# hrubaanna/mysticeti

Hardware: AMD Instinct MI355X
Metric: verified StatementBlock sigs/sec (1/2/4/8 MI355X) vs host-core ed25519-consensus (higher is better)
Workload: dtype u32

## Files before the change

include/mysti_verify.h:

```cpp
#ifndef MYSTI_VERIFY_H
#define MYSTI_VERIFY_H

#include <stddef.h>
#include <stdint.h>

#ifdef __cplusplus
extern "C" {
#endif

typedef struct mv_ctx mv_ctx;
typedef int32_t mv_status;

#define MV_OK 0
#define MV_E_INVALID_ARG (-1)
#define MV_E_HIP (-2)
#define MV_E_NO_DEVICE (-3)
#define MV_E_NO_COMMITTEE (-4)
#define MV_E_ALLOC (-5)
#define MV_E_INDEX_FULL (-6)

#define MV_SIG_OK 0
#define MV_SIG_INVALID 1
#define MV_SIG_MALFORMED_KEY 2

// ... 72 lines not shown

mv_status mv_ed25519_sign(mv_ctx* ctx, const uint8_t* seed, const uint8_t* msg, uint32_t n, uint8_t* pk,
                          uint8_t* sig);

mv_status mv_verify_blocks(mv_ctx* ctx, const uint8_t* buf, const uint64_t* off, const uint64_t* len, uint32_t n,
                           uint8_t* status, uint8_t* msg_digest, uint8_t* block_digest);

mv_status mv_queue_stats(mv_ctx* ctx, uint64_t* calls, uint64_t* passes);

mv_status mv_online_stats(mv_ctx* ctx, uint64_t* requests, uint64_t* launches);

mv_status mv_shard_plan(const uint64_t* weights, uint64_t n, uint32_t parts, uint64_t* cut );

int64_t mv_block_preimage(const uint8_t* bincode, uint64_t len, uint8_t* out, uint64_t cap);

mv_status mv_crc32(mv_ctx* ctx, const uint8_t* buf, const uint64_t* off, const uint64_t* len, uint32_t n,
                   uint32_t* out );

mv_status mv_wal_verify(mv_ctx* ctx, const uint8_t* wal, uint64_t size, uint64_t end_pos, uint32_t map_bits,
                        uint64_t* pos, uint32_t* tag, uint32_t* len, uint8_t* status, uint64_t cap,
                        uint64_t* count);

mv_status mv_wal_replay(mv_ctx* ctx, const uint8_t* wal, uint64_t size, uint64_t end_pos, uint32_t map_bits,
                        uint64_t* pos, uint32_t* tag, uint32_t* len, uint8_t* status, uint64_t cap, uint64_t* count,
                        uint64_t* blk_rows , uint8_t* blk_status ,
                        uint64_t cap_blocks, uint64_t* n_blocks, uint64_t* summary ,
                        uint64_t* last_seen );

uint64_t mv_wal_layout(const uint64_t* payload_len, uint64_t n, uint32_t map_bits, uint64_t start,
                       uint64_t* pos );

int64_t mv_frame_blocks(const uint8_t* buf, uint64_t len, uint64_t* off, uint64_t* blen, uint64_t cap,
                        uint64_t* consumed);

int64_t mv_frame_messages(const uint8_t* buf, uint64_t len, uint32_t* msgs , uint64_t cap_msgs,
                          uint64_t* blk_off, uint64_t* blk_len, uint64_t cap_blocks, uint64_t* n_blocks,
                          uint64_t* consumed);
mv_status mv_verify_frames(mv_ctx* ctx, const uint8_t* buf, const uint64_t* soff, const uint64_t* slen, uint32_t ns,
                           uint64_t* consumed , uint32_t* drop_msg , uint32_t* msgs ,
                           uint64_t cap_msgs, uint64_t* n_msgs, uint64_t* blk_off, uint64_t* blk_len,
                           uint8_t* blk_status , uint64_t cap_blocks, uint64_t* n_blocks);

mv_status mv_index_reserve(mv_ctx* ctx, uint64_t entries);
mv_status mv_index_clear(mv_ctx* ctx);
mv_status mv_index_stats(mv_ctx* ctx, uint64_t* out );
mv_status mv_index_insert(mv_ctx* ctx, const uint64_t* refs , uint64_t n, uint32_t state,
                          uint8_t* prior );
mv_status mv_index_insert_stored(mv_ctx* ctx, const uint64_t* refs , uint64_t n,
                                 uint8_t* prior );
mv_status mv_index_lookup(mv_ctx* ctx, const uint64_t* refs , uint64_t n, uint8_t* state );
mv_status mv_index_wanted(mv_ctx* ctx, uint64_t* refs , uint64_t cap, uint64_t* n);
mv_status mv_accept_blocks(mv_ctx* ctx, const uint8_t* buf, const uint64_t* off, const uint64_t* len,
                           const uint64_t* grp , uint32_t n, uint8_t* blk_status ,
                           uint8_t* blk_state , uint64_t* missing , uint64_t cap_missing,
                           uint64_t* n_missing);
mv_status mv_connect_blocks(mv_ctx* ctx, const uint8_t* buf, const uint64_t* off, const uint64_t* len,
                            const uint64_t* grp , uint32_t n, uint8_t* blk_status ,
                            uint8_t* blk_state , uint64_t* missing , uint64_t cap_missing,
                            uint64_t* n_missing, uint64_t* connected , uint64_t cap_connected,
                            uint64_t* n_connected);
mv_status mv_pending_reserve(mv_ctx* ctx, uint64_t blocks, uint64_t includes);
mv_status mv_pending_stats(mv_ctx* ctx, uint64_t* out );

mv_status mv_dag_reserve(mv_ctx* ctx, uint64_t blocks, uint64_t includes);
mv_status mv_dag_prune(mv_ctx* ctx, uint64_t round);
mv_status mv_dag_stats(mv_ctx* ctx, uint64_t* out );

#define MV_LEADER_UNDECIDED 0
#define MV_LEADER_COMMIT 1
#define MV_LEADER_SKIP 2
#define MV_LEADER_CONFLICT 3
#define MV_LEADER_OVERFLOW 4
#define MV_DECIDE_MAX_LEADER_BLOCKS 8
mv_status mv_decide_leaders(mv_ctx* ctx, const uint64_t* leaders , uint32_t n,
                            uint64_t* out , uint64_t* stakes );

#define MV_COMMIT_KIND_NONE 0
#define MV_COMMIT_KIND_DIRECT 1
#define MV_COMMIT_KIND_INDIRECT 2
#define MV_COMMIT_INCOMPLETE 1
#define MV_COMMIT_BLOCKED 2
mv_status mv_commit_leaders(mv_ctx* ctx, const uint64_t* leaders , uint32_t n,
                            uint64_t* out , uint64_t* info , uint64_t* n_sequence);

mv_status mv_wal_recover(mv_ctx* ctx, const uint8_t* wal, uint64_t size, uint64_t end_pos, uint32_t map_bits,
                         uint64_t* pos, uint32_t* tag, uint32_t* len, uint8_t* status, uint64_t cap, uint64_t* count,
                         uint64_t* blk_rows , uint8_t* blk_status ,
                         uint64_t cap_blocks, uint64_t* n_blocks, uint64_t* summary ,
                         uint64_t* last_seen , uint64_t floor_round, uint64_t* seeded );

#define MV_SEAL_OK 0
#define MV_SEAL_PARSE_ERROR 1
#define MV_SEAL_UNKNOWN_AUTHOR 2
#define MV_SEAL_UNLINKED 3
#define MV_SEAL_LINK 1u
mv_status mv_seal_blocks(mv_ctx* ctx, uint8_t* buf, const uint64_t* off, const uint64_t* len, uint32_t n,
                         const uint8_t* seeds , uint32_t n_auth, uint32_t flags,
                         uint8_t* status , uint8_t* msg_digest ,
                         uint8_t* block_digest );

mv_status mv_dev_ed25519_verify(mv_ctx* ctx, int device, const uint8_t* d_msg, const uint8_t* d_sig,
                                const uint8_t* d_pk, uint32_t n, uint8_t* d_status, void* stream);
mv_status mv_dev_ed25519_verify_batch(mv_ctx* ctx, int device, const uint8_t* d_msg, const uint8_t* d_sig,
                                      const uint8_t* d_pk, const uint32_t* d_key_idx, uint32_t n,
                                      uint8_t* d_status, uint32_t* d_batch_ok, void* stream);
mv_status mv_dev_ed25519_sign(mv_ctx* ctx, int device, const uint8_t* d_seed, const uint8_t* d_msg, uint32_t n,
                              uint8_t* d_pk, uint8_t* d_sig, void* stream);
mv_status mv_dev_verify_blocks(mv_ctx* ctx, int device, const uint8_t* d_buf, uint64_t buf_bytes,
                               const uint64_t* d_off, const uint64_t* d_len, uint32_t n, uint8_t* d_status,
                               uint8_t* d_msg_digest, uint8_t* d_block_digest, void* stream);

mv_status mv_dev_wal_verify(mv_ctx* ctx, int device, const uint8_t* d_wal, uint64_t size, uint64_t end_pos,
                            uint32_t map_bits, uint64_t* d_pos, uint32_t* d_tag, uint32_t* d_len, uint8_t* d_status,
                            uint64_t cap, uint64_t* count, void* stream);
mv_status mv_dev_wal_replay(mv_ctx* ctx, int device, const uint8_t* d_wal, uint64_t size, uint64_t end_pos,
                            uint32_t map_bits, uint64_t* d_pos, uint32_t* d_tag, uint32_t* d_len, uint8_t* d_status,
                            uint64_t cap, uint64_t* count, uint64_t* d_blk_rows, uint8_t* d_blk_status,
                            uint64_t cap_blocks, uint64_t* n_blocks, uint64_t* d_summary, uint64_t* d_last_seen,
                            void* stream);
mv_status mv_dev_verify_frames(mv_ctx* ctx, int device, const uint8_t* d_buf, uint64_t buf_bytes,
                               const uint64_t* d_soff, const uint64_t* d_slen, uint32_t ns, uint64_t* d_consumed,
                               uint32_t* d_drop_msg, uint32_t* d_msgs, uint64_t cap_msgs, uint64_t* n_msgs,
                               uint64_t* d_blk_off, uint64_t* d_blk_len, uint8_t* d_blk_status, uint64_t cap_blocks,
                               uint64_t* n_blocks, void* stream);
mv_status mv_dev_accept_blocks(mv_ctx* ctx, int device, const uint8_t* d_buf, uint64_t buf_bytes,
                               const uint64_t* d_off, const uint64_t* d_len, const uint64_t* d_grp, uint32_t n,
                               uint8_t* d_blk_status, uint8_t* d_blk_state, uint64_t* d_missing, uint64_t cap_missing,
                               uint64_t* n_missing, void* stream);
mv_status mv_dev_index_insert(mv_ctx* ctx, int device, const uint64_t* d_words, uint64_t stride_words, uint64_t n,
                              uint32_t state, void* stream);
mv_status mv_dev_dag_seed_rows(mv_ctx* ctx, int device, const uint8_t* d_wal, uint64_t size,
                               const uint64_t* d_blk_rows , const uint8_t* d_blk_status ,
                               uint64_t n_rows, uint64_t floor_round, uint64_t* seeded , void* stream);
mv_status mv_dev_connect_blocks(mv_ctx* ctx, int device, const uint8_t* d_buf, uint64_t buf_bytes,
                                const uint64_t* d_off, const uint64_t* d_len, const uint64_t* d_grp, uint32_t n,
                                uint8_t* d_blk_status, uint8_t* d_blk_state, uint64_t* d_missing, uint64_t cap_missing,
                                uint64_t* n_missing, uint64_t* d_connected, uint64_t cap_connected,
                                uint64_t* n_connected, void* stream);
mv_status mv_dev_decide_leaders(mv_ctx* ctx, int device, const uint64_t* d_leaders, uint32_t n, uint64_t* d_out,
                                uint64_t* d_stakes , void* stream);
mv_status mv_dev_commit_leaders(mv_ctx* ctx, int device, const uint64_t* d_leaders, uint32_t n, uint64_t* d_out,
                                uint64_t* d_info, uint64_t* n_sequence, void* stream);
mv_status mv_dev_seal_blocks(mv_ctx* ctx, int device, uint8_t* d_buf, uint64_t buf_bytes, const uint64_t* d_off,
                             const uint64_t* d_len, uint32_t n, const uint8_t* d_seeds, uint32_t n_auth,
                             uint32_t flags, uint8_t* d_status, uint8_t* d_msg_digest, uint8_t* d_block_digest,
                             void* stream);
mv_status mv_dev_crc32(mv_ctx* ctx, int device, const uint8_t* d_buf, const uint64_t* d_off, const uint64_t* d_len,
                       uint32_t n, uint32_t* d_out, void* stream);

mv_status mv_batch_stats(mv_ctx* ctx, uint64_t* batches, uint64_t* fallbacks);
mv_status mv_batch_counters(mv_ctx* ctx, uint64_t* out );
mv_status mv_batch_routes(mv_ctx* ctx, uint64_t* out );
mv_status mv_set_batch_groups(mv_ctx* ctx, uint32_t groups);
#define MV_NSTAGES 12
mv_status mv_set_stage_timing(mv_ctx* ctx, int enable);
mv_status mv_stage_times(mv_ctx* ctx, double* ms , uint64_t* calls ,
                         int reset);
mv_status mv_set_option(mv_ctx* ctx, const char* name, int64_t value);
mv_status mv_get_option(mv_ctx* ctx, const char* name, int64_t* value);
mv_status mv_selftest(mv_ctx* ctx, int op, const uint32_t* in, uint32_t n, uint32_t* out);
mv_status mv_selftest_batch_prep(mv_ctx* ctx, const uint8_t* msg, const uint8_t* sig, const uint8_t* pk,
                                 const uint32_t* key_idx, uint32_t n, uint32_t groups, const uint8_t* key,
                                 uint32_t launch_sigs, uint32_t* scal, uint32_t* pts, uint64_t* bsum,
                                 uint8_t* status, uint32_t* info);
mv_status mv_selftest_batch_msm(mv_ctx* ctx, uint32_t n, uint32_t groups, const uint32_t* scal, const uint32_t* pts,
                                const uint64_t* bsum, const uint32_t* key_idx, uint32_t n_keys, uint32_t* win,
                                uint32_t* asum, uint32_t* flags, uint32_t* info);
mv_status mv_selftest_comb_table(mv_ctx* ctx, int key, uint32_t* out);

#ifdef __cplusplus
}
#endif
#endif
```

mysticeti_amd/__init__.py:

```python
from __future__ import annotations

import contextlib
import ctypes
import os
from typing import Iterable, List, Optional, Sequence, Tuple

import numpy as np

_HERE = os.path.dirname(os.path.abspath(__file__))
LIB_PATH = os.environ.get("MV_LIB") or os.path.join(_HERE, "libmysti_verify.so")

MV_OK = 0
SIG_OK, SIG_INVALID, SIG_MALFORMED_KEY = 0, 1, 2
BLOCK_STATUS = [
    "OK", "PARSE_ERROR", "DIGEST_MISMATCH", "EPOCH_MISMATCH", "UNKNOWN_AUTHOR", "GENESIS", "SIG_INVALID",
    "INCLUDE_UNKNOWN_AUTHORITY", "INCLUDE_ROUND", "VOTE_RANGE", "THRESHOLD_CLOCK", "VOTE_RANGE_TOO_LONG",
    "VOTE_RANGE_END_TOO_LARGE",
]
(BLOCK_OK, BLOCK_PARSE_ERROR, BLOCK_DIGEST_MISMATCH, BLOCK_EPOCH_MISMATCH, BLOCK_UNKNOWN_AUTHOR,
 BLOCK_GENESIS, BLOCK_SIG_INVALID, BLOCK_INCLUDE_UNKNOWN_AUTHORITY, BLOCK_INCLUDE_ROUND,
 BLOCK_VOTE_RANGE, BLOCK_THRESHOLD_CLOCK, BLOCK_VOTE_RANGE_TOO_LONG, BLOCK_VOTE_RANGE_END_TOO_LARGE) = range(13)

EXPORTS = [
    "mv_create", "mv_destroy", "mv_last_error", "mv_version", "mv_set_committee", "mv_blake2b256",
    "mv_ed25519_verify", "mv_ed25519_sign", "mv_verify_blocks", "mv_dev_ed25519_verify",
    "mv_dev_ed25519_sign", "mv_selftest", "mv_selftest_batch_prep", "mv_selftest_batch_msm", "mv_selftest_comb_table", "mv_block_preimage", "mv_dev_ed25519_verify_batch", "mv_batch_stats",
    "mv_set_stage_timing", "mv_stage_times", "mv_dev_verify_blocks", "mv_batch_counters", "mv_batch_routes", "mv_set_batch_groups",
    "mv_queue_stats", "mv_shard_plan", "mv_crc32", "mv_wal_verify", "mv_wal_layout", "mv_dev_wal_verify",
    "mv_frame_blocks", "mv_frame_messages", "mv_verify_frames", "mv_dev_verify_frames",
    "mv_index_reserve", "mv_index_clear", "mv_index_stats", "mv_index_insert", "mv_index_lookup", "mv_index_wanted",
    "mv_accept_blocks", "mv_dev_accept_blocks", "mv_dev_index_insert",
    "mv_index_insert_stored", "mv_connect_blocks", "mv_dev_connect_blocks", "mv_pending_reserve", "mv_pending_stats",
    "mv_dag_reserve", "mv_dag_prune", "mv_dag_stats", "mv_decide_leaders", "mv_dev_decide_leaders",
    "mv_commit_leaders", "mv_dev_commit_leaders", "mv_wal_recover", "mv_dev_dag_seed_rows",
    "mv_seal_blocks", "mv_dev_seal_blocks",
    "mv_wal_replay", "mv_dev_wal_replay", "mv_dev_crc32", "mv_host_alloc", "mv_host_free", "mv_online_stats", "mv_set_option", "mv_get_option",
]
SEAL_STATUS = ["OK", "PARSE_ERROR", "UNKNOWN_AUTHOR", "UNLINKED"]
SEAL_OK, SEAL_PARSE_ERROR, SEAL_UNKNOWN_AUTHOR, SEAL_UNLINKED = range(4)
SEAL_LINK = 1
WAL_OK, WAL_CRC_MISMATCH, WAL_NONZERO_CRC_LEN0, WAL_BAD_LENGTH = range(4)
WAL_UNKNOWN_TAG, WAL_BLOCK_DECODE, WAL_UNKNOWN_AUTHORITY = 4, 5, 6
WAL_NONE = 0xFFFFFFFFFFFFFFFF
WAL_ROW_WORDS = 10
MSG_STATUS = ["OK", "DECODE_ERROR", "BLOCK_REJECTED", "TOO_MANY_REQUESTED", "NOT_REACHED", "BAD_SIZE"]
MSG_OK, MSG_DECODE_ERROR, MSG_BLOCK_REJECTED, MSG_TOO_MANY_REQUESTED, MSG_NOT_REACHED, MSG_BAD_SIZE = range(6)
MSG_NONE = 0xFFFFFFFF
REF_ABSENT, REF_WANTED, REF_HAVE, REF_STORED = 0, 1, 2, 3
ACC_STATE = ["REJECTED", "NEW", "KNOWN", "DUP", "DROPPED", "SUSPENDED"]
ACC_REJECTED, ACC_NEW, ACC_KNOWN, ACC_DUP, ACC_DROPPED, ACC_SUSPENDED = range(6)
CONNECT_EARLIER = 0xFFFFFFFFFFFFFFFF
E_INDEX_FULL = -6
E_INVALID_ARG, E_NO_COMMITTEE = -1, -4
LEADER_STATUS = ["UNDECIDED", "COMMIT", "SKIP", "CONFLICT", "OVERFLOW"]
LEADER_UNDECIDED, LEADER_COMMIT, LEADER_SKIP, LEADER_CONFLICT, LEADER_OVERFLOW = range(5)
DECIDE_MAX_LEADER_BLOCKS = 8
COMMIT_KIND_NONE, COMMIT_KIND_DIRECT, COMMIT_KIND_INDIRECT = range(3)
COMMIT_INCOMPLETE, COMMIT_BLOCKED = 1, 2
COMMIT_NO_ANCHOR = 0xFFFFFFFFFFFFFFFF
WAL_MAP_BITS, WAL_MAP_BITS_TEST = 24, 16
STAGES = ["prep", "sort", "bucket", "reduce", "final", "fallback", "parse", "hash", "verify", "verdict", "wal_walk",
          "wal_crc"]
FLAG_NO_BATCH, FLAG_NO_COMB, FLAG_HOST_PARSE, FLAG_NO_ONLINE = 1, 2, 4, 8
BATCH_MIN = 4096
SELFTEST_WIDE_OP = 64
BATCH_MAX_GROUPS = 16
COMB_ROWS, COMB_ENTRIES = 32, 129
BATCH_PREP_UNWRITTEN = 0xA5A5A5A5


class MvError(RuntimeError):

    def __init__(self, msg, code=None):
        super().__init__(msg)
        self.code = code


class _Config(ctypes.Structure):
    _fields_ = [("device_mask", ctypes.c_uint32), ("max_batch", ctypes.c_uint32), ("flags", ctypes.c_uint32),
                ("shards_per_device", ctypes.c_uint32)]


_lib = None


def load_library(path: str = LIB_PATH):
    global _lib
    if _lib is not None:
        return _lib
    if not os.path.exists(path):
        raise MvError(f"{path} missing: build it with `python -m mysticeti_amd.build` (no CPU fallback exists)")
    lib = ctypes.CDLL(path)
    vp, u32, u64 = ctypes.c_void_p, ctypes.c_uint32, ctypes.c_uint64
    lib.mv_create.argtypes = [ctypes.POINTER(_Config), ctypes.POINTER(vp)]
    lib.mv_destroy.argtypes = [vp]
    lib.mv_destroy.restype = None
    lib.mv_last_error.argtypes = [vp]
    lib.mv_last_error.restype = ctypes.c_char_p
    lib.mv_version.restype = ctypes.c_char_p
    lib.mv_set_committee.argtypes = [vp, vp, vp, u32, u64, vp]
    lib.mv_blake2b256.argtypes = [vp, vp, vp, vp, u32, vp]
    lib.mv_ed25519_verify.argtypes = [vp, vp, vp, vp, vp, u32, vp]
    lib.mv_ed25519_sign.argtypes = [vp, vp, vp, u32, vp, vp]
    lib.mv_verify_blocks.argtypes = [vp, vp, vp, vp, u32, vp, vp, vp]
    lib.mv_dev_ed25519_verify.argtypes = [vp, ctypes.c_int, vp, vp, vp, u32, vp, vp]
    lib.mv_dev_ed25519_verify_batch.argtypes = [vp, ctypes.c_int, vp, vp, vp, vp, u32, vp, vp, vp]
    lib.mv_batch_stats.argtypes = [vp, vp, vp]
    lib.mv_batch_counters.argtypes = [vp, vp]
    lib.mv_batch_routes.argtypes = [vp, vp]
    lib.mv_set_batch_groups.argtypes = [vp, u32]
    lib.mv_queue_stats.argtypes = [vp, vp, vp]
    lib.mv_online_stats.argtypes = [vp, vp, vp]
    lib.mv_shard_plan.argtypes = [vp, u64, u32, vp]
    lib.mv_set_stage_timing.argtypes = [vp, ctypes.c_int]
    lib.mv_stage_times.argtypes = [vp, vp, vp, ctypes.c_int]
    lib.mv_dev_verify_blocks.argtypes = [vp, ctypes.c_int, vp, u64, vp, vp, u32, vp, vp, vp, vp]
    lib.mv_dev_ed25519_sign.argtypes = [vp, ctypes.c_int, vp, vp, u32, vp, vp, vp]
    lib.mv_seal_blocks.argtypes = [vp, vp, vp, vp, u32, vp, u32, u32, vp, vp, vp]
    lib.mv_dev_seal_blocks.argtypes = [vp, ctypes.c_int, vp, u64, vp, vp, u32, vp, u32, u32, vp, vp, vp, vp]
    lib.mv_selftest.argtypes = [vp, ctypes.c_int, vp, u32, vp]
    lib.mv_selftest_batch_prep.argtypes = [vp, vp, vp, vp, vp, u32, u32, vp, u32, vp, vp, vp, vp, vp]
    lib.mv_selftest_batch_msm.argtypes = [vp, u32, u32, vp, vp, vp, vp, u32, vp, vp, vp, vp]
    lib.mv_selftest_comb_table.argtypes = [vp, ctypes.c_int, vp]
    lib.mv_block_preimage.argtypes = [vp, u64, vp, u64]
    lib.mv_block_preimage.restype = ctypes.c_int64
    lib.mv_crc32.argtypes = [vp, vp, vp, vp, u32, vp]
    lib.mv_wal_verify.argtypes = [vp, vp, u64, u64, u32, vp, vp, vp, vp, u64, vp]
    lib.mv_wal_layout.argtypes = [vp, u64, u32, u64, vp]
    lib.mv_wal_layout.restype = u64
    lib.mv_frame_blocks.argtypes = [vp, u64, vp, vp, u64, vp]
    lib.mv_frame_blocks.restype = ctypes.c_int64
    lib.mv_frame_messages.argtypes = [vp, u64, vp, u64, vp, vp, u64, vp, vp]
    lib.mv_frame_messages.restype = ctypes.c_int64
    lib.mv_verify_frames.argtypes = [vp, vp, vp, vp, u32, vp, vp, vp, u64, vp, vp, vp, vp, u64, vp]
    lib.mv_dev_verify_frames.argtypes = [vp, ctypes.c_int, vp, u64, vp, vp, u32, vp, vp, vp, u64, vp, vp, vp, vp, u64,
                                         vp, vp]
    lib.mv_dev_wal_verify.argtypes = [vp, ctypes.c_int, vp, u64, u64, u32, vp, vp, vp, vp, u64, vp, vp]
    lib.mv_wal_replay.argtypes = [vp, vp, u64, u64, u32, vp, vp, vp, vp, u64, vp, vp, vp, u64, vp, vp, vp]
    lib.mv_dev_wal_replay.argtypes = [vp, ctypes.c_int, vp, u64, u64, u32, vp, vp, vp, vp, u64, vp, vp, vp, u64, vp, vp,
                                      vp, vp]
    lib.mv_wal_recover.argtypes = [vp, vp, u64, u64, u32, vp, vp, vp, vp, u64, vp, vp, vp, u64, vp, vp, vp, u64, vp]
    lib.mv_dev_dag_seed_rows.argtypes = [vp, ctypes.c_int, vp, u64, vp, vp, u64, u64, vp, vp]
    lib.mv_dev_crc32.argtypes = [vp, ctypes.c_int, vp, vp, vp, u32, vp, vp]
    lib.mv_index_reserve.argtypes = [vp, u64]
    lib.mv_index_clear.argtypes = [vp]
    lib.mv_index_stats.argtypes = [vp, vp]
    lib.mv_index_insert.argtypes = [vp, vp, u64, u32, vp]
    lib.mv_index_lookup.argtypes = [vp, vp, u64, vp]
    lib.mv_index_wanted.argtypes = [vp, vp, u64, vp]
    lib.mv_accept_blocks.argtypes = [vp, vp, vp, vp, vp, u32, vp, vp, vp, u64, vp]
    lib.mv_dev_accept_blocks.argtypes = [vp, ctypes.c_int, vp, u64, vp, vp, vp, u32, vp, vp, vp, u64, vp, vp]
    lib.mv_dev_index_insert.argtypes = [vp, ctypes.c_int, vp, u64, u64, u32, vp]
    lib.mv_index_insert_stored.argtypes = [vp, vp, u64, vp]
    lib.mv_connect_blocks.argtypes = [vp, vp, vp, vp, vp, u32, vp, vp, vp, u64, vp, vp, u64, vp]
    lib.mv_dev_connect_blocks.argtypes = [vp, ctypes.c_int, vp, u64, vp, vp, vp, u32, vp, vp, vp, u64, vp, vp, u64, vp, vp]
    lib.mv_pending_reserve.argtypes = [vp, u64, u64]
    lib.mv_pending_stats.argtypes = [vp, vp]
    lib.mv_dag_reserve.argtypes = [vp, u64, u64]
    lib.mv_dag_prune.argtypes = [vp, u64]
    lib.mv_dag_stats.argtypes = [vp, vp]
    lib.mv_decide_leaders.argtypes = [vp, vp, u32, vp, vp]
    lib.mv_dev_decide_leaders.argtypes = [vp, ctypes.c_int, vp, u32, vp, vp, vp]
    lib.mv_commit_leaders.argtypes = [vp, vp, u32, vp, vp, vp]
    lib.mv_dev_commit_leaders.argtypes = [vp, ctypes.c_int, vp, u32, vp, vp, vp, vp]
    lib.mv_host_alloc.argtypes = [vp, u64, ctypes.POINTER(vp)]
    lib.mv_host_free.argtypes = [vp, vp]
    lib.mv_host_free.restype = None
    lib.mv_set_option.argtypes = [vp, ctypes.c_char_p, ctypes.c_int64]
    lib.mv_get_option.argtypes = [vp, ctypes.c_char_p, ctypes.POINTER(ctypes.c_int64)]
    for name in EXPORTS:
        getattr(lib, name).restype = getattr(lib, name).restype or ctypes.c_int32
    _lib = lib
    return lib


def _p(a: Optional[np.ndarray]):
    return None if a is None else ctypes.c_void_p(a.ctypes.data)


def _u8(a, shape_tail: int) -> np.ndarray:
    a = np.ascontiguousarray(np.asarray(a, dtype=np.uint8))
    return a.reshape(-1, shape_tail)


class Engine:

    def __init__(self, devices: Sequence[int] = (0,), max_batch: int = 0, batch: bool = True, comb: bool = True,
                 host_parse: bool = False, shards_per_device: int = 1, online: bool = True):
        self.lib = load_library()
        mask = 0
        for d in devices:
            mask |= 1 << int(d)
        flags = (0 if batch else FLAG_NO_BATCH) | (0 if comb else FLAG_NO_COMB) | (FLAG_HOST_PARSE if host_parse else 0) \
            | (0 if online else FLAG_NO_ONLINE)
        cfg = _Config(mask, max_batch, flags, shards_per_device)
        h = ctypes.c_void_p()
        rc = self.lib.mv_create(ctypes.byref(cfg), ctypes.byref(h))
        if rc != MV_OK:
            raise MvError(f"mv_create failed ({rc}): no usable gfx950 device")
        self.ctx = h
        self.devices = list(devices)
        self.committee_size = 0

    def close(self):
        if getattr(self, "ctx", None):
            for ptr in getattr(self, "_pinned", {}).values():
                self.lib.mv_host_free(self.ctx, ptr)
            self._pinned = {}
            self.lib.mv_destroy(self.ctx)
            self.ctx = None

    def host_empty(self, shape, dtype=np.uint8) -> np.ndarray:
        nbytes = int(np.prod(shape)) * np.dtype(dtype).itemsize
        ptr = ctypes.c_void_p()
        self._check(self.lib.mv_host_alloc(self.ctx, max(nbytes, 1), ctypes.byref(ptr)), "mv_host_alloc")
# ... 807 lines not shown
```

mysticeti_amd/csrc/batch.hip:

```cpp
#include <hip/hip_runtime.h>
#include <stdint.h>
#include <stdlib.h>

#include <algorithm>

#include "fe25519.h"
#include "ge25519.h"
#include "blake2b_quad.h"
#include "hash_dev.h"
#include "kernels.h"
#include "scalar25519.h"
#include "tables.h"
#include "comb.h"
#include "quad25519.h"
#include "pt_r16.h"

namespace mv {

constexpr int BV_C = 16;
constexpr int BV_NB = 1 << (BV_C - 1);
constexpr int BV_NW = 16;
constexpr int BV_NWR = 8;
constexpr uint32_t BV_NKG = BV_NW * BV_NB;
constexpr int BV_FINE_BITS = 8;
constexpr int BV_NPG = BV_NKG >> BV_FINE_BITS;
constexpr int BV_FAN = 8;
constexpr int BV_MAXG = mvk::BATCH_MAX_GROUPS;
constexpr int P3_QUADS = 9;
constexpr int SC_QUADS = 3;
constexpr int BSUM_WORDS = 12;

MV_DEV int bv_digit(uint32_t word, int half, uint32_t& carry) {
  const uint32_t v = (half ? (word >> 16) : (word & 0xffffu)) + carry;
  carry = v >= (1u << 15) ? 1u : 0u;
  return (int)v - (int)(carry << 16);
}

template <class Fn>
MV_DEV void bv_for_digits(const uint32_t z[4], const uint32_t zk[8], Fn fn) {
  uint32_t carry = 0;
#pragma unroll
  for (int w = 0; w < 7; w++) {
    const int d = bv_digit(z[w >> 1], w & 1, carry);
    if (d) fn(w, d, 0);
  }
  {
    const int d = (int)((z[3] >> 16) + carry);
    if (d) fn(7, d, 0);
  }
  carry = 0;
#pragma unroll
  for (int w = 0; w < 15; w++) {
    const int d = bv_digit(zk[w >> 1], w & 1, carry);
    if (d) fn(w, d, 1);
  }
  {
    const int d = (int)((zk[7] >> 16) + carry);
    if (d) fn(15, d, 1);
  }
}

MV_DEV uint32_t bv_key(int w, int d) { return (uint32_t)w * BV_NB + (uint32_t)(d < 0 ? -d : d) - 1u; }

MV_DEV void precomp_from_affine(precomp& pc, const p3& P) {
  fe d2;
  fe_const(d2, K_D2);
  fe_addn(pc.ypx, P.Y, P.X);
  fe_sub(pc.ymx, P.Y, P.X);
  fe_mul(pc.xy2d, P.T, d2);
}

MV_DEV void pt_store(uint4* pts, size_t idx, const precomp& pc) {
  uint4 q[7];
  precomp_to_quads(q, pc);
  uint4* p = pts + idx * PT_QUADS;
#pragma unroll
  for (int i = 0; i < 7; i++) p[i] = q[i];
  if (PT_QUADS == 8) p[7] = make_uint4(0, 0, 0, 0);
}
MV_DEV void pt_load(precomp& pc, const uint4* pts, uint32_t idx) {
  const uint4* p = pts + (size_t)idx * PT_QUADS;
  uint4 q[7];
#pragma unroll
  for (int i = 0; i < 7; i++) q[i] = p[i];
  quads_to_precomp(pc, q);
}
MV_DEV void p3_store(uint4* a, size_t idx, const p3& P) {
  uint4 q[9];
  p3_to_quads(q, P);
  uint4* p = a + idx * P3_QUADS;
#pragma unroll
  for (int i = 0; i < 9; i++) p[i] = q[i];
}
MV_DEV void p3_load(p3& P, const uint4* a, size_t idx) {
  const uint4* p = a + idx * P3_QUADS;
  uint4 q[9];
#pragma unroll
  for (int i = 0; i < 9; i++) q[i] = p[i];
  quads_to_p3(P, q);
}
MV_DEV void p3_acc(p3& P, const p3& Q) {
  cached c;
  p1p1 t;
  p3_to_cached(c, Q);
  p3_add_cached(t, P, c);
  p1p1_to_p3(P, t);
}
MV_DEV void p3_dbl_n(p3& P, int n) {
  if (n <= 0) return;
  p2 q;
  p1p1 t;
  q.X = P.X; q.Y = P.Y; q.Z = P.Z;
  for (int i = 1; i < n; i++) {
    p2_dbl(t, q);
    p1p1_to_p2(q, t);
  }
  p2_dbl(t, q);
  p1p1_to_p3(P, t);
}

struct BvKey {
  uint32_t w[10];
};

struct CommitteeA {
  const uint4* tab;
  const uint8_t* ok;
  uint32_t stride;
  uint32_t aggregate;
};

#ifndef MV_PREP_OCC
#define MV_PREP_OCC 3
#endif
__global__ void __launch_bounds__(256, MV_PREP_OCC)
    k_bv_prep(const uint8_t* __restrict__ msg, const uint8_t* __restrict__ sig, const uint8_t* __restrict__ pk,
              const uint32_t* __restrict__ key_idx, uint32_t n, BvKey key, CommitteeA ca, uint4* __restrict__ pts,
              uint4* __restrict__ scal, unsigned long long* __restrict__ bsum, uint8_t* __restrict__ status,
              uint32_t blk0, uint32_t group_sigs) {
  __shared__ unsigned long long sbsum[BSUM_WORDS];
  __shared__ uint32_t va[8][256], vs[8][256], vz[4][256];
#ifdef MV_PREP_X2
  __shared__ uint32_t vr[8][256];
#endif
  const uint32_t t = threadIdx.x;
  if (threadIdx.x < BSUM_WORDS) sbsum[threadIdx.x] = 0;
  __syncthreads();
  const uint32_t blk = blockIdx.x + blk0;
  const uint32_t gid = blk * blockDim.x + threadIdx.x;
  const bool live = gid < n;
  const uint32_t idx = live ? gid : n - 1;

  uint32_t aw[8], rw[8], sw[8], mw[8];
  const uint32_t kid = key_idx ? key_idx[idx] : idx;
  load8(aw, pk + 32 * (size_t)kid);
  load8(rw, sig + 64 * (size_t)idx);
  load8(sw, sig + 64 * (size_t)idx + 32);
  load8(mw, msg + 32 * (size_t)idx);
  const bool s_ok = sc_is_canonical(sw);
#pragma unroll
  for (int i = 0; i < 8; i++) {
    va[i][t] = aw[i];
    vs[i][t] = sw[i];
  }
  uint32_t z[4], zk[8];
  {
    uint32_t k[8];
    {
      uint32_t kin[24], h[16];
#pragma unroll
      for (int i = 0; i < 8; i++) {
        kin[i] = rw[i];
        kin[8 + i] = aw[i];
        kin[16 + i] = mw[i];
      }
      sha512_short(h, kin, 96);
      sc_reduce512(k, h);
    }
    uint64_t m[16], h[8];
#pragma unroll
    for (int i = 0; i < 5; i++) m[i] = (uint64_t)key.w[2 * i] | ((uint64_t)key.w[2 * i + 1] << 32);
    m[5] = gid;
#pragma unroll
    for (int i = 6; i < 16; i++) m[i] = 0;
    b2q::lane_init256(h);
    b2q::lane_compress(h, m, 48, true);
    z[0] = (uint32_t)h[0];
    z[1] = (uint32_t)(h[0] >> 32);
    z[2] = (uint32_t)h[1];
    z[3] = (uint32_t)(h[1] >> 32) & 0x7fffffffu;
    uint32_t z8[8], zero[8];
#pragma unroll
    for (int i = 0; i < 8; i++) {
      z8[i] = i < 4 ? z[i] : 0u;
      zero[i] = 0;
    }
    sc_muladd(zk, z8, k, zero);
  }
  uint4* sc = scal + (size_t)idx * SC_QUADS;
#pragma unroll
  for (int i = 0; i < 4; i++) vz[i][t] = z[i];
  if (live) {
    sc[0] = make_uint4(z[0], z[1], z[2], z[3]);
    sc[1] = make_uint4(zk[0], zk[1], zk[2], zk[3]);
    sc[2] = make_uint4(zk[4], zk[5], zk[6], zk[7]);
  }

  bool okA, okR;
  {
    precomp pc;
    if (ca.tab) {
      p3 P;
      decompress1_lean(P, okR, rw);
      precomp_from_affine(pc, P);
      if (live) pt_store(pts, gid, pc);
      okA = ca.ok[kid] != 0;
      if (!ca.aggregate) {
        const uint4* e = ca.tab + (size_t)kid * ca.stride + 8;
        uint4 q[7];
#pragma unroll
        for (int k = 0; k < 7; k++) q[k] = e[k];
        quads_to_precomp(pc, q);
        precomp_cneg(pc, true);
        fe_canon(pc.xy2d, pc.xy2d);
        if (live) pt_store(pts, (size_t)n + gid, pc);
      }
    } else {
#ifdef MV_PREP_X2
    p3 P, Q;
#pragma unroll
    for (int i = 0; i < 8; i++) vr[i][t] = rw[i];
    decompress2_lean(Q, okA, P, okR, [&](int which, uint32_t (&e)[8]) {
      asm volatile("" ::: "memory");
#pragma unroll
      for (int i = 0; i < 8; i++) e[i] = which ? vr[i][t] : va[i][t];
    });
    precomp_from_affine(pc, P);
    if (live) pt_store(pts, gid, pc);
    precomp_from_affine(pc, Q);
    if (live) pt_store(pts, (size_t)n + gid, pc);
#else
    p3 P;
    decompress1_lean(P, okR, rw);
    precomp_from_affine(pc, P);
    if (live) pt_store(pts, gid, pc);
    asm volatile("" ::: "memory");
#pragma unroll
    for (int i = 0; i < 8; i++) aw[i] = va[i][t];
    decompress1_lean(P, okA, aw);
    precomp_from_affine(pc, P);
    if (live) pt_store(pts, (size_t)n + gid, pc);
#endif
    }
  }
  const bool ok = live && okA && okR && s_ok;
  if (live) {
    if (!ok) {
      const uint4 zq = make_uint4(0, 0, 0, 0);
      sc[0] = zq;
      sc[1] = zq;
      sc[2] = zq;
    }
    status[gid] = !okA ? 2 : (ok ? 0 : 1);
  }
  asm volatile("" ::: "memory");
#pragma unroll
  for (int i = 0; i < 4; i++) z[i] = ok ? vz[i][t] : 0u;
#pragma unroll
  for (int i = 0; i < 8; i++) sw[i] = vs[i][t];
  {
    uint64_t acc = 0;
    uint32_t c2 = 0;
#pragma unroll
    for (int c = 0; c < 11; c++) {
#pragma unroll
      for (int i = 0; i < 4; i++)
        if (c - i >= 0 && c - i < 8) mac(acc, c2, z[i], sw[c - i]);
      atomicAdd(&sbsum[c], (unsigned long long)(uint32_t)acc);
      acc = (acc >> 32) | ((uint64_t)c2 << 32);
      c2 = 0;
    }
    atomicAdd(&sbsum[11], (unsigned long long)(uint32_t)acc);
  }
  __syncthreads();
  if (threadIdx.x < BSUM_WORDS)
    atomicAdd(&bsum[(size_t)(blk * 256u / group_sigs) * BSUM_WORDS + threadIdx.x], sbsum[threadIdx.x]);
}

template <int NT = 256>
MV_DEV uint32_t block_excl_scan256(uint32_t v, uint32_t* sm, uint32_t& total) {
  const int t = threadIdx.x;
  sm[t] = v;
  __syncthreads();
  for (int o = 1; o < NT; o <<= 1) {
    uint32_t x = t >= o ? sm[t - o] : 0u;
    __syncthreads();
    sm[t] += x;
    __syncthreads();
  }
  total = sm[NT - 1];
  const uint32_t incl = sm[t];
  __syncthreads();
  return incl - v;
}

constexpr int PART_CHUNK = 1024;

struct BvGroups {
  uint32_t count;
  uint32_t cpg;
};

MV_DEV void load_scalars(uint32_t z[4], uint32_t zk[8], const uint4* scal, uint32_t i) {
  const uint4* sc = scal + (size_t)i * SC_QUADS;
  const uint4 q0 = sc[0], q1 = sc[1], q2 = sc[2];
  z[0] = q0.x; z[1] = q0.y; z[2] = q0.z; z[3] = q0.w;
  zk[0] = q1.x; zk[1] = q1.y; zk[2] = q1.z; zk[3] = q1.w;
  zk[4] = q2.x; zk[5] = q2.y; zk[6] = q2.z; zk[7] = q2.w;
}
__global__ void __launch_bounds__(PART_CHUNK) k_part_count(const uint4* __restrict__ scal, uint32_t n, uint32_t skipA,
                                                           uint32_t* __restrict__ pcount) {
  __shared__ uint32_t hist[BV_NPG];
  for (int i = threadIdx.x; i < BV_NPG; i += PART_CHUNK) hist[i] = 0;
  __syncthreads();
  const uint32_t gid = blockIdx.x * PART_CHUNK + threadIdx.x;
  if (gid < n) {
    uint32_t z[4], zk[8];
    load_scalars(z, zk, scal, gid);
    if (skipA) {
#pragma unroll
      for (int i = 0; i < 8; i++) zk[i] = 0;
    }
    bv_for_digits(z, zk, [&](int w, int d, int) { atomicAdd(&hist[bv_key(w, d) >> BV_FINE_BITS], 1u); });
  }
  __syncthreads();
  for (int i = threadIdx.x; i < BV_NPG; i += PART_CHUNK) pcount[(size_t)blockIdx.x * BV_NPG + i] = hist[i];
}
constexpr int SCAN_SUB = 16;
__global__ void __launch_bounds__(64 * SCAN_SUB) k_part_scan(const uint32_t* __restrict__ pcount, uint32_t nchunk,
                                                             BvGroups G, uint32_t* __restrict__ poff,
                                                             uint32_t* __restrict__ ptot) {
  __shared__ uint32_t gsum[SCAN_SUB][64];
  constexpr uint32_t BPG = BV_NPG / 64;
  const uint32_t pl = threadIdx.x & 63, q = threadIdx.x >> 6;
  const uint32_t g = blockIdx.x / BPG;
  const uint32_t p = (blockIdx.x % BPG) * 64 + pl;
  const uint32_t cg0 = g * G.cpg, cg1 = min(nchunk, cg0 + G.cpg);
  const uint32_t per = (cg1 - cg0 + SCAN_SUB - 1) / SCAN_SUB;
  const uint32_t c0 = min(cg1, cg0 + q * per), c1 = min(cg1, c0 + per);
  uint32_t sum = 0;
  for (uint32_t c = c0; c < c1; c++) sum += pcount[(size_t)c * BV_NPG + p];
  gsum[q][pl] = sum;
  __syncthreads();
  uint32_t run = 0;
  for (uint32_t k = 0; k < q; k++) run += gsum[k][pl];
  for (uint32_t c = c0; c < c1; c++) {
    const uint32_t v = pcount[(size_t)c * BV_NPG + p];
    poff[(size_t)c * BV_NPG + p] = run;
    run += v;
  }
  if (q == SCAN_SUB - 1) ptot[g * BV_NPG + p] = run;
}
__global__ void __launch_bounds__(256) k_part_top(const uint32_t* __restrict__ ptot, uint32_t total,
                                                  uint32_t* __restrict__ pstart) {
  __shared__ uint32_t sm[256];
  const uint32_t per = total / 256;
  const uint32_t* src = ptot + (size_t)per * threadIdx.x;
  uint32_t sum = 0;
  for (uint32_t i = 0; i < per; i++) sum += src[i];
  uint32_t all;
  uint32_t run = block_excl_scan256(sum, sm, all);
  for (uint32_t i = 0; i < per; i++) {
    const uint32_t v = src[i];
    pstart[(size_t)per * threadIdx.x + i] = run;
    run += v;
  }
  if (threadIdx.x == 0) pstart[total] = all;
}
template <class E>
struct PartEntry;
template <>
struct PartEntry<uint32_t> {
  static constexpr bool narrow = true;
  static constexpr uint32_t REF_BITS = 32 - BV_FINE_BITS;
  static MV_DEV uint32_t make(uint32_t gkey, uint32_t ref) { return gkey << REF_BITS | ref; }
  static MV_DEV uint32_t bin(uint32_t e) { return e >> REF_BITS; }
  static MV_DEV uint32_t ref(uint32_t e) { return e & ((1u << REF_BITS) - 1); }
};
template <>
struct PartEntry<unsigned long long> {
  static constexpr bool narrow = false;
  static MV_DEV unsigned long long make(uint32_t gkey, uint32_t ref) { return (unsigned long long)gkey << 32 | ref; }
  static MV_DEV uint32_t bin(unsigned long long e) { return (uint32_t)(e >> 32) & ((1u << BV_FINE_BITS) - 1); }
  static MV_DEV uint32_t ref(unsigned long long e) { return (uint32_t)e; }
};
constexpr uint32_t BV_NARROW_MAX_N = 1u << (PartEntry<uint32_t>::REF_BITS - 2);

constexpr uint32_t BV_PPW = BV_NB >> BV_FINE_BITS;
template <class E>
__global__ void __launch_bounds__(PART_CHUNK) k_part_scatter_lds(const uint4* __restrict__ scal, uint32_t n,
                                                                 const uint32_t* __restrict__ pcount,
                                                                 const uint32_t* __restrict__ poff,
                                                                 const uint32_t* __restrict__ pstart, BvGroups G,
                                                                 uint32_t skipA, uint32_t nall, uint32_t base,
                                                                 E* __restrict__ tmp) {
  using PE = PartEntry<E>;
  __shared__ E buf[2 * PART_CHUNK];
  __shared__ uint8_t bpl[PE::narrow ? 2 * PART_CHUNK : 1];
  static_assert(BV_PPW <= 256, "a slot's partition fits a byte");
  __shared__ uint32_t lofs[BV_PPW + 1], gpos[BV_PPW], rank[BV_PPW];
  const uint32_t gid = blockIdx.x * PART_CHUNK + threadIdx.x;
  const bool live = gid < n;
  const uint32_t g = blockIdx.x / G.cpg;
  int dR[8], dA[16];
#pragma unroll
  for (int w = 0; w < 8; w++) dR[w] = 0;
#pragma unroll
  for (int w = 0; w < 16; w++) dA[w] = 0;
  if (live) {
    uint32_t z[4], zk[8];
    load_scalars(z, zk, scal, gid);
    if (skipA) {
// ... 508 lines not shown
  r4::store(outT, gid, U);
}

__global__ void __launch_bounds__(128) k_bv_final(const uint4* __restrict__ winV, uint32_t nw,
                                                  const uint4* __restrict__ asum,
                                                  const unsigned long long* __restrict__ bsum, uint32_t ngroups,
                                                  const uint4* __restrict__ combB, uint32_t* __restrict__ flags,
                                                  uint32_t rows) {
  __shared__ uint4 sbp[BV_MAXG][P3_QUADS];
  __shared__ uint4 shp[P3_QUADS];
  __shared__ uint32_t sflag[BV_MAXG];
  const uint32_t lane = threadIdx.x & 63;
  if (threadIdx.x >= 64) {
    if (lane < ngroups) {
      uint32_t x[16];
      unsigned long long carry = 0;
#pragma unroll
      for (int c = 0; c < BSUM_WORDS; c++) {
        const unsigned long long v = bsum[(size_t)lane * BSUM_WORDS + c];
        const unsigned long long lo = (v & 0xffffffffull) + (carry & 0xffffffffull);
        x[c] = (uint32_t)lo;
        carry = (v >> 32) + (carry >> 32) + (lo >> 32);
      }
      x[12] = (uint32_t)carry;
      x[13] = (uint32_t)(carry >> 32);
      x[14] = x[15] = 0;
      uint32_t r[8], sd[8];
      sc_reduce512(r, x);
      sc_recode256(sd, r);
      p3 P;
      ct_sum(P, combB, sd, 0, CT_ROWS);
      p3_neg(P, P);
      uint4 q[9];
      p3_to_quads(q, P);
#pragma unroll
      for (int i = 0; i < 9; i++) sbp[lane][i] = q[i];
    }
  }
  const uint32_t g = lane >> 2;
  fe v;
  if (threadIdx.x < 64 && rows && ngroups == 1) {
    const r16::Consts K = r16::consts();
    fe d2;
    fe_const(d2, K_D2);
    fer d2r;
    fer_from_fe(d2r, d2);
    fer pv = r4::load(winV, nw - 1);
#pragma unroll 1
    for (int w = (int)nw - 2; w >= 0; w--) {
      const fer wv = r4::load(winV, w);
#pragma unroll 1
      for (int i = 0; i < BV_C; i++) r4::dbl(pv, K);
      r4::addp(pv, wv, d2r, K);
    }
    if (asum) r4::addp(pv, r4::load(asum, 0), d2r, K);
    r4::store(reinterpret_cast<uint32_t*>(shp), pv);
    __builtin_amdgcn_fence(__ATOMIC_RELEASE, "wavefront");
    __builtin_amdgcn_wave_barrier();
    __builtin_amdgcn_fence(__ATOMIC_ACQUIRE, "wavefront");
    if (g == 0) qp_load(v, shp, 0);
  } else if (threadIdx.x < 64 && g < ngroups) {
    const size_t row0 = (size_t)g * nw;
    qp_load(v, winV, row0 + nw - 1);
    for (int w = (int)nw - 2; w >= 0; w--) {
      fe wv;
      qp_load(wv, winV, row0 + w);
      qp_dbl_n(v, BV_C);
      qp_add(v, wv);
    }
    if (asum) {
      fe av;
      qp_load(av, asum, g);
      qp_add(v, av);
    }
  }
  __syncthreads();
  if (threadIdx.x < 64 && g < ngroups) {
    fe bv;
    qp_load(bv, &sbp[0][0], g);
    qp_add(v, bv);
    qp_dbl_n(v, 3);
    fe Y, Z;
    fe_qget<1>(Y, v);
    fe_qget<2>(Z, v);
    const bool x0 = fe_is_zero(v);
    const bool yz = fe_eq(Y, Z);
    if ((lane & 3) == 0) sflag[g] = x0 && yz ? 1u : 0u;
  }
  __syncthreads();
  if (threadIdx.x == 0) {
    uint32_t all = 1;
    for (uint32_t gg = 0; gg < ngroups; gg++) {
      flags[1 + gg] = sflag[gg];
      all &= sflag[gg];
    }
    flags[0] = all;
  }
}

}

namespace mvk {

namespace {
constexpr size_t align256(size_t x) { return (x + 255) & ~(size_t)255; }
struct BatchLayout {
  size_t pts, scal, pcount, poff, ptot, pstart, tmp, offs, ents, carry, bktT, rV0, rT0, rV1, rT1, bsum, kpart, keyp,
      asum, flag, total;
  BatchLayout(uint32_t n, uint32_t groups) {
    using namespace mv;
    size_t o = 0;
    auto take = [&](size_t bytes) { size_t r = o; o += align256(bytes); return r; };
    pts = take((size_t)2 * n * PT_QUADS * 16);
    scal = take((size_t)n * SC_QUADS * 16);
    const size_t nchunk = (n + PART_CHUNK - 1) / PART_CHUNK;
    pcount = take(nchunk * BV_NPG * 4);
    poff = take(nchunk * BV_NPG * 4);
    ptot = take((size_t)groups * BV_NPG * 4);
    pstart = take(((size_t)groups * BV_NPG + 1) * 4);
    tmp = take((size_t)(BV_NWR + BV_NW) * n * 8);
    offs = take(((size_t)groups * BV_NKG + 1) * 4);
    ents = take((size_t)(BV_NWR + BV_NW) * n * 4);
    carry = take((size_t)groups * BV_NKG / 2 * P3_QUADS * 16);
    bktT = take((size_t)groups * BV_NKG * P3_QUADS * 16);
    const size_t lv = (size_t)groups * (BV_NKG / BV_FAN) * P3_QUADS * 16;
    rV0 = take(lv); rT0 = take(lv); rV1 = take(lv); rT1 = take(lv);
    bsum = take((size_t)BV_MAXG * BSUM_WORDS * 8);
    kpart = take(nchunk * BV_MAXKEYS * 8 * 8);
    keyp = take((size_t)BV_MAXG * BV_MAXKEYS * P3_QUADS * 16);
    asum = take((size_t)BV_MAXG * P3_QUADS * 16);
    flag = take((1 + BV_MAXG) * 4);
    total = o;
  }
};
mv::BvGroups batch_groups(uint32_t n, uint32_t want) {
  const uint32_t nchunk = (n + mv::PART_CHUNK - 1) / mv::PART_CHUNK;
  uint32_t g = want < 1 ? 1 : (want > (uint32_t)mv::BV_MAXG ? (uint32_t)mv::BV_MAXG : want);
  if (g > nchunk) g = nchunk;
  const uint32_t cpg = (nchunk + g - 1) / g;
  return mv::BvGroups{(nchunk + cpg - 1) / cpg, cpg};
}
bool agg_disabled(const Knobs& kn) { return kn.no_key_agg != 0; }

uint32_t reduce_quad_max(const Knobs& kn) { return (uint32_t)kn.reduce_quad; }
}

size_t batch_scratch_bytes(uint32_t n, uint32_t groups) { return BatchLayout(n, groups).total; }

uint32_t batch_group_size(uint32_t n, uint32_t groups) {
  return batch_groups(n, groups).cpg * mv::PART_CHUNK;
}

namespace {
struct PrepStage {
  mv::CommitteeA ca;
  bool agg;
};
hipError_t launch_prep_stage(const Knobs& kn, const uint8_t* msg, const uint8_t* sig, const uint8_t* pk,
                             const uint32_t* key_idx, uint32_t n, const mv::BvGroups& G, const uint32_t key[10],
                             uint4* pts, uint4* scal, unsigned long long* bsum, uint8_t* status, hipStream_t s,
                             const void* comb_a, const uint8_t* key_ok, uint32_t n_keys, const ChunkGate* gate,
                             const hipEvent_t* chain, PrepStage* out) {
  using namespace mv;
  hipError_t e;
  BvKey k;
  for (int i = 0; i < 10; i++) k.w[i] = key[i];
  const bool com = key_idx && key_ok && comb_a;
  const bool agg = com && n_keys > 0 && n_keys <= (uint32_t)BV_MAXKEYS && !agg_disabled(kn);
  const CommitteeA ca{com ? static_cast<const uint4*>(comb_a) : nullptr, key_ok,
                      (uint32_t)(comb_table_bytes(1) / sizeof(uint4)), agg ? 1u : 0u};
  out->ca = ca;
  out->agg = agg;
  e = hipMemsetAsync(bsum, 0, (size_t)BV_MAXG * BSUM_WORDS * 8, s);
  if (e != hipSuccess) return e;
  const uint32_t group_sigs = G.cpg * PART_CHUNK;
  if (gate && gate->n) {
    const uint32_t* end = gate->end;
    if (end[gate->n - 1] != n) return hipErrorInvalidValue;
    for (uint32_t c = 0, lo = 0; c < gate->n; lo = end[c++]) {
      const uint32_t hi = end[c];
      if (hi <= lo || lo % 256 || (hi % 256 && hi != n)) return hipErrorInvalidValue;
      if ((e = hipStreamWaitEvent(s, gate->ready[c], 0)) != hipSuccess) return e;
      hipLaunchKernelGGL(k_bv_prep, dim3((hi - lo + 255) / 256), dim3(256), 0, s, msg, sig, pk, key_idx, n, k, ca,
                         pts, scal, bsum, status, lo / 256, group_sigs);
    }
  } else {
    if (chain && chain[0] && (e = hipStreamWaitEvent(s, chain[0], 0)) != hipSuccess) return e;
    hipLaunchKernelGGL(k_bv_prep, dim3((n + 255) / 256), dim3(256), 0, s, msg, sig, pk, key_idx, n, k, ca, pts, scal,
                       bsum, status, 0u, group_sigs);
    if (chain && (e = hipEventRecord(chain[1], s)) != hipSuccess) return e;
  }
  return hipSuccess;
}
}

hipError_t launch_batch_prep(const Knobs& kn, const uint8_t* msg, const uint8_t* sig, const uint8_t* pk,
                             const uint32_t* key_idx, uint32_t n, uint32_t groups, const uint32_t key[10], void* pts,
                             void* scal, void* bsum, uint8_t* status, hipStream_t s, const void* comb_a,
                             const uint8_t* key_ok, uint32_t n_keys, const ChunkGate* gate, BatchPrepInfo* info) {
  if (n == 0) return hipSuccess;
  const mv::BvGroups G = batch_groups(n, groups);
  PrepStage ps;
  hipError_t e = launch_prep_stage(kn, msg, sig, pk, key_idx, n, G, key, static_cast<uint4*>(pts),
                                   static_cast<uint4*>(scal), static_cast<unsigned long long*>(bsum), status, s, comb_a,
                                   key_ok, n_keys, gate, nullptr, &ps);
  if (e != hipSuccess) return e;
  if (info) *info = BatchPrepInfo{G.count, G.cpg * mv::PART_CHUNK, ps.ca.tab && ps.ca.aggregate ? 0u : 1u};
  return hipGetLastError();
}

namespace {
struct MsmStage {
  const uint4* winV;
  const uint4* asum;
  uint32_t nw;
};
hipError_t launch_msm_stage(const Knobs& kn, const uint32_t* key_idx, uint32_t n, const mv::BvGroups& G, bool agg,
                            uint32_t n_keys, const void* comb_a, const void* comb_b, void* bscratch, hipStream_t s,
                            hipEvent_t* ev, MsmStage* out) {
  using namespace mv;
  auto mark = [&](int i) { if (ev) (void)hipEventRecord(ev[i], s); };
  const BatchLayout L(n, G.count);
  char* base = static_cast<char*>(bscratch);
  const uint4* pts = (const uint4*)(base + L.pts);
  const uint4* scal = (const uint4*)(base + L.scal);
  uint32_t* pcount = (uint32_t*)(base + L.pcount);
  uint32_t* poff = (uint32_t*)(base + L.poff);
  uint32_t* ptot = (uint32_t*)(base + L.ptot);
  uint32_t* pstart = (uint32_t*)(base + L.pstart);
  void* tmp = base + L.tmp;
  const bool sort_narrow = !kn.sort_wide && n <= BV_NARROW_MAX_N;
  uint32_t* offs = (uint32_t*)(base + L.offs);
  uint32_t* ents = (uint32_t*)(base + L.ents);
  uint4* carry = (uint4*)(base + L.carry);
  uint4* bktT = (uint4*)(base + L.bktT);
  uint4* rv[2] = {(uint4*)(base + L.rV0), (uint4*)(base + L.rV1)};
  uint4* rt[2] = {(uint4*)(base + L.rT0), (uint4*)(base + L.rT1)};
  unsigned long long* bsum = (unsigned long long*)(base + L.bsum);
  unsigned long long* kpart = (unsigned long long*)(base + L.kpart);
  uint4* keyp = (uint4*)(base + L.keyp);
  uint4* asum = (uint4*)(base + L.asum);
  uint32_t* flag = (uint32_t*)(base + L.flag);
  const uint32_t nchunk = (n + PART_CHUNK - 1) / PART_CHUNK;
  const uint32_t nparts = G.count * BV_NPG;
  const uint32_t nw = agg ? BV_NWR : BV_NW;
  const uint32_t nk = G.count * BV_NKG;
  {
    mark(1);
    hipLaunchKernelGGL(k_part_count, dim3(nchunk), dim3(PART_CHUNK), 0, s, scal, n, agg ? 1u : 0u, pcount);
    hipLaunchKernelGGL(k_part_scan, dim3(G.count * (BV_NPG / 64)), dim3(64 * SCAN_SUB), 0, s, pcount, nchunk, G, poff,
                       ptot);
    hipLaunchKernelGGL(k_part_top, dim3(1), dim3(256), 0, s, ptot, nparts, pstart);
    if (sort_narrow) {
      hipLaunchKernelGGL(k_part_scatter_lds<uint32_t>, dim3(nchunk), dim3(PART_CHUNK), 0, s, scal, n, pcount, poff,
                         pstart, G, agg ? 1u : 0u, n, 0u, (uint32_t*)tmp);
      hipLaunchKernelGGL(k_fine_sort_lds<uint32_t>, dim3(nparts), dim3(FINE_NT), 0, s, (const uint32_t*)tmp, pstart,
                         G.count, ents, offs);
    } else {
      hipLaunchKernelGGL(k_part_scatter_lds<unsigned long long>, dim3(nchunk), dim3(PART_CHUNK), 0, s, scal, n, pcount,
                         poff, pstart, G, agg ? 1u : 0u, n, 0u, (unsigned long long*)tmp);
      hipLaunchKernelGGL(k_fine_sort_lds<unsigned long long>, dim3(nparts), dim3(FINE_NT), 0, s,
                         (const unsigned long long*)tmp, pstart, G.count, ents, offs);
    }
    mark(2);
    const uint64_t est = (uint64_t)n * (nw + BV_NWR);
    const uint64_t want = kn.bucket_bal > 1 ? est / (uint64_t)kn.bucket_bal
                                            : std::max<uint64_t>(est / 64, std::min<uint64_t>(est / 8, 196608));
    const uint32_t cap = nk / 2;
    const uint32_t nl = (uint32_t)std::min<uint64_t>(cap, std::max<uint64_t>(256, (want + 255) / 256 * 256));
    hipLaunchKernelGGL(k_bv_bucket_bal, dim3(nl / 256), dim3(256), 0, s, pts, offs, ents, nk, nl, carry, bktT);
    hipLaunchKernelGGL(k_bv_bucket_fix, dim3(G.count * nw * BV_NB / 256), dim3(256), 0, s, offs, nk, G.count, nw, nl,
                       carry, bktT);
  }
  if (agg) {
    hipLaunchKernelGGL(k_bv_keyacc, dim3(nchunk), dim3(PART_CHUNK), 0, s, scal, key_idx, n, n_keys, kpart);
    hipLaunchKernelGGL(k_bv_keycol, dim3(G.count * n_keys), dim3(256), 0, s, kpart, nchunk, G.cpg, n_keys,
                       static_cast<const uint4*>(comb_a), keyp);
    hipLaunchKernelGGL(k_bv_keysum, dim3(G.count), dim3(256), 0, s, keyp, n_keys, asum);
  }
  mark(3);
  const uint4* inV = nullptr;
  const uint4* inT = bktT;
  const uint32_t rows = G.count * nw;
  uint32_t cnt = BV_NB;
  int shift = 0;
  int pp = 0;
  while (cnt > 1) {
    const int fan = cnt >= (uint32_t)BV_FAN ? BV_FAN : (int)cnt;
    const uint32_t out = (cnt + fan - 1) / fan;
    const uint32_t lanes = out * rows;
    if (lanes <= (uint32_t)kn.reduce_rows)
      hipLaunchKernelGGL(k_bv_reduce_r, dim3((64 * lanes + 255) / 256), dim3(256), 0, s, inV, inT, cnt, fan, shift,
                         rows, nw, inT == bktT ? 1u : 0u, rv[pp], rt[pp]);
    else if (lanes <= reduce_quad_max(kn))
      hipLaunchKernelGGL(k_bv_reduce_q, dim3((4 * lanes + 255) / 256), dim3(256), 0, s, inV, inT, cnt, fan, shift,
                         rows, nw, inT == bktT ? 1u : 0u, rv[pp], rt[pp]);
    else
      hipLaunchKernelGGL(k_bv_reduce, dim3((lanes + 63) / 64), dim3(64), 0, s, inV, inT, cnt, fan, shift, rows, nw,
                         inT == bktT ? 1u : 0u, rv[pp], rt[pp]);
    inV = rv[pp];
    inT = rt[pp];
    pp ^= 1;
    shift += fan == 8 ? 3 : (fan == 4 ? 2 : 1);
    cnt = out;
  }
  mark(4);
  hipLaunchKernelGGL(k_bv_final, dim3(1), dim3(128), 0, s, inV, nw, agg ? (const uint4*)asum : nullptr, bsum,
                     G.count, static_cast<const uint4*>(comb_b), flag, kn.final_rows ? 1u : 0u);
  mark(5);
  *out = MsmStage{inV, agg ? (const uint4*)asum : nullptr, nw};
  return hipGetLastError();
}
}

hipError_t launch_verify_batch(const Knobs& kn, const uint8_t* msg, const uint8_t* sig, const uint8_t* pk, const uint32_t* key_idx,
                               uint32_t n, uint32_t groups, const uint32_t key[10], const void* btab,
                               void* bscratch, void* vscratch, uint8_t* status, hipStream_t s,
                               uint32_t** flag_out, hipEvent_t* ev, const void* comb_a, const uint8_t* key_ok,
                               uint32_t n_keys, const void* comb_b, const ChunkGate* gate, const hipEvent_t* chain) {
  using namespace mv;
  auto mark = [&](int i) { if (ev) (void)hipEventRecord(ev[i], s); };
  if (n == 0) return hipSuccess;
  const BvGroups G = batch_groups(n, groups);
  const BatchLayout L(n, G.count);
  char* base = static_cast<char*>(bscratch);
  uint4* pts = (uint4*)(base + L.pts);
  uint4* scal = (uint4*)(base + L.scal);
  unsigned long long* bsum = (unsigned long long*)(base + L.bsum);
  uint32_t* flag = (uint32_t*)(base + L.flag);
  if (flag_out) *flag_out = flag;
  hipError_t e;
  mark(0);
  PrepStage ps;
  e = launch_prep_stage(kn, msg, sig, pk, key_idx, n, G, key, pts, scal, bsum, status, s, comb_a, key_ok, n_keys, gate,
                        chain, &ps);
  if (e != hipSuccess) return e;
  const CommitteeA& ca = ps.ca;
  MsmStage ms;
  e = launch_msm_stage(kn, key_idx, n, G, ps.agg, n_keys, comb_a, comb_b, bscratch, s, ev, &ms);
  if (e != hipSuccess) return e;
  e = launch_verify(msg, sig, pk, key_idx, n, btab, vscratch, status, s, flag + 1, G.cpg * PART_CHUNK, pts,
                    ca.tab && ca.aggregate ? comb_a : nullptr);
  mark(6);
  return e;
}

hipError_t launch_batch_msm(const Knobs& kn, uint32_t n, uint32_t groups, const void* h_scal, const void* h_pts,
                            const void* h_bsum, const uint32_t* key_idx, uint32_t n_keys, const void* comb_a,
                            const void* comb_b, void* bscratch, size_t scratch_bytes, hipStream_t s,
                            BatchMsmInfo* info) {
  using namespace mv;
  if (n == 0) return hipSuccess;
  const BvGroups G = batch_groups(n, groups);
  const BatchLayout L(n, G.count);
  const bool agg = key_idx != nullptr;
  if (scratch_bytes < L.total || (agg && (!comb_a || n_keys == 0 || n_keys > (uint32_t)BV_MAXKEYS || agg_disabled(kn))))
    return hipErrorInvalidValue;
  char* base = static_cast<char*>(bscratch);
  hipError_t e;
  if ((e = hipMemcpyAsync(base + L.scal, h_scal, (size_t)n * SC_QUADS * 16, hipMemcpyHostToDevice, s)) != hipSuccess)
    return e;
  if ((e = hipMemcpyAsync(base + L.pts, h_pts, (size_t)(agg ? 1 : 2) * n * PT_QUADS * 16, hipMemcpyHostToDevice, s)) !=
      hipSuccess)
    return e;
  if ((e = hipMemcpyAsync(base + L.bsum, h_bsum, (size_t)BV_MAXG * BSUM_WORDS * 8, hipMemcpyHostToDevice, s)) !=
      hipSuccess)
    return e;
  MsmStage ms;
  e = launch_msm_stage(kn, key_idx, n, G, agg, n_keys, comb_a, comb_b, bscratch, s, nullptr, &ms);
  if (e != hipSuccess) return e;
  *info = BatchMsmInfo{G.count, G.cpg * PART_CHUNK, ms.nw, ms.winV, ms.asum, (const uint32_t*)(base + L.flag)};
  return hipSuccess;
}

}
```

mysticeti_amd/csrc/engine.cpp:

```cpp
#include <hip/hip_runtime.h>
#include <stdio.h>
#include <stdlib.h>
#include <string.h>
#include <dirent.h>
#include <unistd.h>

#include <algorithm>
#include <chrono>
#include <atomic>
#include <condition_variable>
#include <mutex>
#include <string>
#include <thread>
#include <vector>

#include "engine_internal.h"

using namespace mvi;

namespace mvi {

constexpr int kGuardBatches = 64;
constexpr int kSingleRun = 32;
constexpr uint32_t kDenseRejects = 4;
// ... 2 lines not shown
struct Retired {
  int device;
  void* p;
  bool host;
  hipEvent_t guard;
};
std::mutex g_retired_mu;
std::vector<Retired> g_retired;
std::atomic<int> g_retired_n{0};

void free_retired(const std::vector<Retired>& blocks) {
  for (const Retired& r : blocks) (void)(r.host ? hipHostFree(r.p) : hipFree(r.p));
  mvr::g_live -= (int64_t)blocks.size();
}

void reap_retired(int device) {
  std::vector<Retired> mine;
  {
    std::lock_guard<std::mutex> lk(g_retired_mu);
    auto it = std::stable_partition(g_retired.begin(), g_retired.end(),
                                    [device](const Retired& r) { return r.device != device; });
    mine.assign(it, g_retired.end());
    g_retired.erase(it, g_retired.end());
    g_retired_n.store((int)g_retired.size());
  }
  free_retired(mine);
}

void reap_ready(int device) {
  if (g_retired_n.load(std::memory_order_relaxed) == 0) return;
  std::vector<Retired> done;
  {
    std::lock_guard<std::mutex> lk(g_retired_mu);
    auto it = std::stable_partition(g_retired.begin(), g_retired.end(), [device](const Retired& r) {
      if (r.device != device) return true;
      if (!r.guard) return false;
      const hipError_t q = hipEventQuery(r.guard);
      if (q != hipSuccess) (void)hipGetLastError();
      return q != hipSuccess;
    });
    done.assign(it, g_retired.end());
    g_retired.erase(it, g_retired.end());
    g_retired_n.store((int)g_retired.size());
  }
  free_retired(done);
}

}

void mvr::retire(void* p, bool host, hipEvent_t guard) {
  int d = 0;
  (void)hipGetDevice(&d);
  std::lock_guard<std::mutex> lk(g_retired_mu);
  g_retired.push_back(Retired{d, p, host, guard});
  g_retired_n.store((int)g_retired.size());
  g_live++;
}

namespace mvi {

void poll_flags(mv_ctx* ctx, Device& dev) {
  for (int k = 0; k < Device::kFlagRing; k++) {
    const uint32_t ng = dev.batch.flag_groups[k];
    if (!ng) continue;
    if (hipEventQuery(dev.batch.flag_ev[k]) != hipSuccess) {
      (void)hipGetLastError();
      continue;
    }
    dev.batch.flag_groups[k] = 0;
    const uint32_t* f = dev.batch.flags(k);
    if (ng == kSingleMark) {
      if (f[0] >= kDenseRejects) {
        ctx->single_left.store(kSingleRun);
      } else {
        ctx->single_left.store(0);
        ctx->guard_left = kGuardBatches;
      }
      continue;
    }
    ctx->batches++;
    ctx->groups_run += ng;
    uint32_t bad = 0;
    for (uint32_t g = 0; g < ng; g++) bad += f[1 + g] ? 0u : 1u;
    ctx->groups_failed += bad;
    if (!f[0]) {
      ctx->fallbacks++;
      ctx->guard_left = kGuardBatches;
      if (ng >= 2 && 2 * bad >= ng && ctx->groups_fixed == 0) {
        ctx->dense_failures++;
        ctx->single_left.store(kSingleRun);
      }
    }
  }
}

uint32_t pick_groups(mv_ctx* ctx) {
  if (ctx->groups_fixed) return ctx->groups_fixed;
  if (ctx->guard_left.fetch_sub(1) > 0) return ctx->guard_groups;
  ctx->guard_left.store(0);
  return ctx->base_groups;
}

mv_status enqueue_batch(mv_ctx* ctx, Device& dev, const uint8_t* d_msg, const uint8_t* d_sig, const uint8_t* d_pk,
                        const uint32_t* d_key_idx, uint32_t n, uint8_t* d_status, hipStream_t s,
                        uint32_t* flag_dst, const mvk::ChunkGate* gate, bool caller_stream) {
  poll_flags(ctx, dev);
  auto& ring = dev.batch.ring;
  int slot;
  HIPCHK(ctx, ring.claim(&slot));
  if (!dev.batch.h_flags.p) {
    constexpr size_t kFlagBytes = sizeof(uint32_t) * Device::kFlagRing * Device::kFlagWords;
    HIPCHK(ctx, dev.batch.h_flags.ensure(kFlagBytes));
    memset(dev.batch.h_flags.p, 0, kFlagBytes);
  }
  const int fe = dev.batch.flag_next;
  dev.batch.flag_next = (fe + 1) % Device::kFlagRing;
  HIPCHK(ctx, dev.batch.flag_ev[fe].ensure());
  if (dev.batch.flag_groups[fe]) {
    HIPCHK(ctx, hipEventSynchronize(dev.batch.flag_ev[fe]));
    poll_flags(ctx, dev);
  }
  const bool com_a = d_key_idx && dev.committee_loaded && d_pk == dev.tab.committee_pk.as<uint8_t>() &&
                     !(ctx->flags & MV_FLAG_NO_COMB);
  if (ctx->groups_fixed == 0 && ctx->single_left.load() > 0) {
    ctx->single_left--;
    ring.hand_back(slot);
    if (gate && gate->n)
      for (uint32_t c = 0; c < gate->n; c++) HIPCHK(ctx, hipStreamWaitEvent(s, gate->ready[c], 0));
    mv_status st = com_a ? enqueue_committee_verify(ctx, dev, d_msg, d_sig, d_key_idx, n, d_status, s)
                         : enqueue_verify(ctx, dev, d_msg, d_sig, d_pk, d_key_idx, n, d_status, s);
    if (st != MV_OK) return st;
    HIPCHK(ctx, dev.batch.rejects.ensure(sizeof(uint32_t) * Device::kFlagRing));
    uint32_t* cnt = dev.batch.rejects.as<uint32_t>() + fe;
    HIPCHK(ctx, mvk::launch_count_rejects(d_status, n, cnt, s));
    if (flag_dst) HIPCHK(ctx, hipMemsetAsync(flag_dst, 0, 4, s));
    HIPCHK(ctx, hipMemcpyAsync(dev.batch.flags(fe), cnt, sizeof(uint32_t), hipMemcpyDeviceToHost, s));
    HIPCHK(ctx, hipEventRecord(dev.batch.flag_ev[fe], s));
    dev.batch.flag_groups[fe] = kSingleMark;
    ctx->single_batches++;
    return MV_OK;
  }
  HIPCHK(ctx, ring.order_behind(slot, s));
  auto& sl = ring.slot[slot];
  const uint32_t groups = pick_groups(ctx);
  HIPCHK(ctx, sl.scr.b.ensure(mvk::batch_scratch_bytes(n, mvk::BATCH_MAX_GROUPS), sl.done));
  HIPCHK(ctx, sl.scr.v.ensure(mvk::verify_scratch_bytes(n), sl.done));
  uint32_t key[10];
  memcpy(key, ctx->secret, 32);
  const uint64_t call = ctx->calls.fetch_add(1);
  key[8] = (uint32_t)call;
  key[9] = (uint32_t)(call >> 32);
  uint32_t* flag = nullptr;
  mvr::EventSet evs;
  mv_status st = make_events(ctx, mvk::BATCH_STAGES, evs);
  if (st != MV_OK) return st;
  hipEvent_t chain[2] = {};
  const bool chained = ctx->kn.prep_chain && !(gate && gate->n) && (!caller_stream || ctx->kn.prep_chain >= 2);
  if (chained) {
    HIPCHK(ctx, dev.batch.prep_chain.ensure());
    chain[0] = dev.batch.prep_chained ? (hipEvent_t)dev.batch.prep_chain : nullptr;
    chain[1] = dev.batch.prep_chain;
  }
  HIPCHK(ctx, mvk::launch_verify_batch(ctx->kn, d_msg, d_sig, d_pk, d_key_idx, n, groups, key, dev.tab.btab.p, sl.scr.b.p,
                                       sl.scr.v.p, d_status, s, &flag, evs.empty() ? nullptr : evs.data(),
                                       com_a ? dev.tab.combA.p : nullptr, com_a ? dev.tab.keyok.as<uint8_t>() : nullptr,
                                       com_a ? (uint32_t)ctx->committee.size() : 0u, dev.tab.combB.p, gate,
                                       chained ? chain : nullptr));
  if (chained) dev.batch.prep_chained = true;
  keep_events(ctx, dev.id, 0, evs);
  if (flag_dst) HIPCHK(ctx, hipMemcpyAsync(flag_dst, flag, 4, hipMemcpyDeviceToDevice, s));
  const uint32_t ng = (n + mvk::batch_group_size(n, groups) - 1) / mvk::batch_group_size(n, groups);
  HIPCHK(ctx, hipMemcpyAsync(dev.batch.flags(fe), flag, sizeof(uint32_t) * (1 + ng), hipMemcpyDeviceToHost, s));
  HIPCHK(ctx, ring.mark_used(slot, s));
  HIPCHK(ctx, hipEventRecord(dev.batch.flag_ev[fe], s));
  dev.batch.flag_groups[fe] = ng;
  return MV_OK;
}

mv_status enqueue_verify(mv_ctx* ctx, Device& dev, const uint8_t* d_msg, const uint8_t* d_sig, const uint8_t* d_pk,
                         const uint32_t* d_key_idx, uint32_t n, uint8_t* d_status, hipStream_t s) {
  if (n == 0) return MV_OK;
  auto& ring = dev.single.ring;
  int slot;
  HIPCHK(ctx, ring.take(s, &slot));
  auto& sl = ring.slot[slot];
  HIPCHK(ctx, sl.scr.ensure(mvk::verify_scratch_bytes(n), sl.done));
  HIPCHK(ctx, mvk::launch_verify(d_msg, d_sig, d_pk, d_key_idx, n, dev.tab.btab.p, sl.scr.p, d_status, s));
  HIPCHK(ctx, ring.mark_used(slot, s));
  return MV_OK;
}

mv_status enqueue_committee_verify(mv_ctx* ctx, Device& dev, const uint8_t* d_msg, const uint8_t* d_sig,
                                   const uint32_t* d_kidx, uint32_t n, uint8_t* d_status, hipStream_t s,
                                   const mvk::BlockVerdictOut* bv, const mvk::BlockHashIn* hin,
                                   const mvk::BlockIngestIn* ing) {
  if (!(ctx->flags & MV_FLAG_NO_COMB)) {
    HIPCHK(ctx, mvk::launch_verify_comb(ctx->kn, d_msg, d_sig, dev.tab.committee_pk.as<uint8_t>(), d_kidx, n, dev.tab.combB.p,
                                        dev.tab.combA.p, dev.tab.keyok.as<uint8_t>(), d_status, s, bv, hin, ing));
  } else {
    return enqueue_verify(ctx, dev, d_msg, d_sig, dev.tab.committee_pk.as<uint8_t>(), d_kidx, n, d_status, s);
  }
  return MV_OK;
}

bool committee_ready(mv_ctx* ctx) {
  if (!ctx->has_committee) return false;
  for (auto& dev : ctx->devs)
    if (!dev.committee_loaded) return false;
  return true;
}

bool host_pinned(const void* p) {
  if (!p) return false;
  hipPointerAttribute_t a;
  if (hipPointerGetAttributes(&a, p) != hipSuccess) {
    (void)hipGetLastError();
    return false;
  }
  return a.type == hipMemoryTypeHost;
}

bool pinned_range_holds(const void* p, uint64_t bytes) {
  if (!host_pinned(p)) return false;
  void* start = nullptr;
  size_t size = 0;
  hipDeviceptr_t q = const_cast<void*>(p);
  if (hipPointerGetAttribute(&start, HIP_POINTER_ATTRIBUTE_RANGE_START_ADDR, q) != hipSuccess ||
      hipPointerGetAttribute(&size, HIP_POINTER_ATTRIBUTE_RANGE_SIZE, q) != hipSuccess || !start || !size) {
    (void)hipGetLastError();
    return false;
  }
  const uintptr_t a = reinterpret_cast<uintptr_t>(start), b = reinterpret_cast<uintptr_t>(p);
  return b >= a && b - a <= size && bytes <= size - (b - a);
}

mv_status verify_host_streamed(mv_ctx* ctx, Device& dev, const uint8_t* msg, const uint8_t* sig, const uint8_t* pk,
                               const uint32_t* key_idx, uint64_t lo, uint64_t hi, int slot) {
  const int chunk_log2 = (int)std::min<int64_t>(24, std::max<int64_t>(8, ctx->kn.stream_chunk_log2));
  const uint64_t m = hi - lo;
  const std::vector<double> fracs(ctx->kn.stream_fracs, ctx->kn.stream_fracs + ctx->kn.n_stream_fracs);
  std::vector<uint32_t> sizes;
  {
    double tot = 0.0;
    for (double f : fracs) tot += f;
    uint64_t done = 0;
    for (size_t k = 0; k < fracs.size() && done < m; k++) {
      uint64_t want = k + 1 == fracs.size() ? m - done : (((uint64_t)(m * fracs[k] / tot)) + 1023) & ~1023ull;
      if (want < MV_BATCH_MIN) want = MV_BATCH_MIN;
      if (want > m - done) want = m - done;
      if (m - done - want > 0 && m - done - want < MV_BATCH_MIN) want = m - done;
      if (want > ctx->max_batch) want = ctx->max_batch;
      done += want;
      sizes.push_back((uint32_t)want);
    }
    while (done < m) {
      const uint64_t want = std::min<uint64_t>(m - done, ctx->max_batch);
      sizes.push_back((uint32_t)want);
      done += want;
    }
  }
  uint32_t cap = 0;
  for (uint32_t z : sizes) cap = std::max(cap, z);
  uint32_t chunk = 1u << chunk_log2;
  while ((cap + chunk - 1) / chunk > (uint32_t)Device::kMaxChunks / 2) chunk <<= 1;
  auto schedule = [&](int first, uint32_t k) {
    std::vector<uint32_t> cut;
    uint32_t o = 0, c = first ? std::min<uint32_t>(chunk, 1u << 14) : chunk;
    while (o < k) {
      cut.push_back(o);
      o += c;
      if (c < chunk) c *= 2;
    }
    cut.push_back(k);
    return cut;
  };
  const size_t kb = pk ? 32 : 4;
  for (int b = 0; b < Device::kPinBufs; b++) {
    HIPCHK(ctx, dev.pin.pin_free[b].ensure());
    HIPCHK(ctx, dev.pin.chunk_ev[b].ensure(Device::kMaxChunks, hipEventDisableTiming));
    HIPCHK(ctx, dev.pin.pin_msg[b].ensure(32 * (size_t)cap, dev.pin.pin_free[b]));
    HIPCHK(ctx, dev.pin.pin_sig[b].ensure(64 * (size_t)cap, dev.pin.pin_free[b]));
    HIPCHK(ctx, dev.pin.pin_pk[b].ensure(kb * cap, dev.pin.pin_free[b]));
    HIPCHK(ctx, dev.pin.pin_st[b].ensure(cap, dev.pin.pin_free[b]));
  }
  for (int k = 0; k < 2; k++) HIPCHK(ctx, dev.pin.sig_done[slot][k].ensure());
  HIPCHK(ctx, dev.pin.sig_stage[slot].ensure(m));
  uint8_t* hst = dev.pin.sig_stage[slot].as<uint8_t>();
  bool used[2] = {false, false};
  hipStream_t xs = dev.stream;
  uint64_t i = lo;
  for (size_t t = 0; t < sizes.size(); i += sizes[t], t++) {
    const int rot = dev.pin.pin_next++;
    const int b = rot % Device::kPinBufs, ci = rot & 1;
    hipStream_t cs = dev.pin.pstream[ci];
    used[ci] = true;
    const uint32_t k = sizes[t];
    HIPCHK(ctx, hipStreamWaitEvent(xs, dev.pin.pin_free[b], 0));
    const uint8_t* src_pk = pk ? pk + 32 * i : (const uint8_t*)(key_idx + i);
    const std::vector<uint32_t> cut = schedule(t == 0, k);
    std::vector<uint32_t> marks;
    for (uint32_t c = 0; c + 1 < cut.size() && cut[c] < k; c++) {
      const uint32_t o = cut[c];
      const size_t r = std::min(cut[c + 1], k) - o;
      marks.push_back(o + (uint32_t)r);
      HIPCHK(ctx, hipMemcpyAsync(dev.pin.pin_msg[b].as<uint8_t>() + 32 * (size_t)o, msg + 32 * (i + o), 32 * r,
                                 hipMemcpyHostToDevice, xs));
      HIPCHK(ctx, hipMemcpyAsync(dev.pin.pin_sig[b].as<uint8_t>() + 64 * (size_t)o, sig + 64 * (i + o), 64 * r,
                                 hipMemcpyHostToDevice, xs));
      HIPCHK(ctx, hipMemcpyAsync(dev.pin.pin_pk[b].as<uint8_t>() + kb * o, src_pk + kb * o, kb * r,
                                 hipMemcpyHostToDevice, xs));
      HIPCHK(ctx, hipEventRecord(dev.pin.chunk_ev[b][c], xs));
    }
    const mvk::ChunkGate gate{dev.pin.chunk_ev[b].data(), (uint32_t)marks.size(), marks.data()};
    mv_status rc = enqueue_batch(ctx, dev, dev.pin.pin_msg[b].as<uint8_t>(), dev.pin.pin_sig[b].as<uint8_t>(),
                                 pk ? dev.pin.pin_pk[b].as<uint8_t>() : dev.tab.committee_pk.as<uint8_t>(),
                                 pk ? nullptr : dev.pin.pin_pk[b].as<uint32_t>(), k, dev.pin.pin_st[b].as<uint8_t>(), cs,
                                 nullptr, &gate);
    hipError_t e = rc == MV_OK ? hipMemcpyAsync(hst + (i - lo), dev.pin.pin_st[b].p, k, hipMemcpyDeviceToHost, cs)
                               : hipSuccess;
    if (e == hipSuccess && rc == MV_OK) e = hipEventRecord(dev.pin.pin_free[b], cs);
    if (rc != MV_OK || e != hipSuccess) {
      (void)hipStreamSynchronize(xs);
// ... 516 lines not shown
    HIPCHK(ctx, hipSetDevice(dev.id));
    for (uint64_t i = lo; i < hi; i += ctx->max_batch) {
      uint32_t m = (uint32_t)std::min<uint64_t>(ctx->max_batch, hi - i);
      HIPCHK(ctx, dev.hc.msg.ensure(32 * (size_t)m));
      HIPCHK(ctx, dev.hc.sig.ensure(64 * (size_t)m));
      HIPCHK(ctx, dev.hc.status.ensure(m));
      HIPCHK(ctx, hipMemcpyAsync(dev.hc.msg.p, msg + 32 * i, 32 * (size_t)m, hipMemcpyHostToDevice, dev.stream));
      HIPCHK(ctx, hipMemcpyAsync(dev.hc.sig.p, sig + 64 * i, 64 * (size_t)m, hipMemcpyHostToDevice, dev.stream));
      const uint8_t* dpk;
      const uint32_t* dki = nullptr;
      if (pk) {
        HIPCHK(ctx, dev.hc.pk.ensure(32 * (size_t)m));
        HIPCHK(ctx, hipMemcpyAsync(dev.hc.pk.p, pk + 32 * i, 32 * (size_t)m, hipMemcpyHostToDevice, dev.stream));
        dpk = dev.hc.pk.as<uint8_t>();
      } else {
        HIPCHK(ctx, dev.hc.keyidx.ensure(4 * (size_t)m));
        HIPCHK(ctx, hipMemcpyAsync(dev.hc.keyidx.p, key_idx + i, 4 * (size_t)m, hipMemcpyHostToDevice, dev.stream));
        dpk = dev.tab.committee_pk.as<uint8_t>();
        dki = dev.hc.keyidx.as<uint32_t>();
      }
      if (!(ctx->flags & MV_FLAG_NO_BATCH) && m >= MV_BATCH_MIN) {
        mv_status st = enqueue_batch(ctx, dev, dev.hc.msg.as<uint8_t>(), dev.hc.sig.as<uint8_t>(), dpk, dki, m,
                                     dev.hc.status.as<uint8_t>(), dev.stream, nullptr);
        if (st != MV_OK) return st;
      } else if (dki) {
        mv_status st = enqueue_committee_verify(ctx, dev, dev.hc.msg.as<uint8_t>(), dev.hc.sig.as<uint8_t>(), dki, m,
                                                dev.hc.status.as<uint8_t>(), dev.stream);
        if (st != MV_OK) return st;
      } else {
        mv_status st = enqueue_verify(ctx, dev, dev.hc.msg.as<uint8_t>(), dev.hc.sig.as<uint8_t>(), dpk, nullptr, m,
                                      dev.hc.status.as<uint8_t>(), dev.stream);
        if (st != MV_OK) return st;
      }
      HIPCHK(ctx, hipMemcpyAsync(status + i, dev.hc.status.p, m, hipMemcpyDeviceToHost, dev.stream));
      HIPCHK(ctx, hipStreamSynchronize(dev.stream));
      poll_flags(ctx, dev);
    }
    return MV_OK;
  });
}

mv_status mv_ed25519_sign(mv_ctx* ctx, const uint8_t* seed, const uint8_t* msg, uint32_t n, uint8_t* pk,
                          uint8_t* sig) {
  if (!ctx || (n && (!seed || !msg || !pk || !sig))) return set_err(ctx, MV_E_INVALID_ARG, "bad sign args");
  std::lock_guard<std::mutex> lk(ctx->mu);
  return for_each_shard(ctx, n, [&](Device& dev, uint64_t lo, uint64_t hi) -> mv_status {
    HIPCHK(ctx, hipSetDevice(dev.id));
    for (uint64_t i = lo; i < hi; i += ctx->max_batch) {
      uint32_t m = (uint32_t)std::min<uint64_t>(ctx->max_batch, hi - i);
      HIPCHK(ctx, dev.hc.msg.ensure(32 * (size_t)m));
      HIPCHK(ctx, dev.hc.bytes.ensure(32 * (size_t)m));
      HIPCHK(ctx, dev.hc.pk.ensure(32 * (size_t)m));
      HIPCHK(ctx, dev.hc.sig.ensure(64 * (size_t)m));
      HIPCHK(ctx, hipMemcpyAsync(dev.hc.bytes.p, seed + 32 * i, 32 * (size_t)m, hipMemcpyHostToDevice, dev.stream));
      HIPCHK(ctx, hipMemcpyAsync(dev.hc.msg.p, msg + 32 * i, 32 * (size_t)m, hipMemcpyHostToDevice, dev.stream));
      HIPCHK(ctx, mvk::launch_sign(dev.hc.bytes.as<uint8_t>(), dev.hc.msg.as<uint8_t>(), m, dev.tab.btab.p,
                                   dev.hc.pk.as<uint8_t>(), dev.hc.sig.as<uint8_t>(), dev.stream));
      HIPCHK(ctx, hipMemcpyAsync(pk + 32 * i, dev.hc.pk.p, 32 * (size_t)m, hipMemcpyDeviceToHost, dev.stream));
      HIPCHK(ctx, hipMemcpyAsync(sig + 64 * i, dev.hc.sig.p, 64 * (size_t)m, hipMemcpyDeviceToHost, dev.stream));
      HIPCHK(ctx, hipStreamSynchronize(dev.stream));
    }
    return MV_OK;
  });
}

mv_status mv_online_stats(mv_ctx* ctx, uint64_t* requests, uint64_t* launches) {
  if (!ctx) return MV_E_INVALID_ARG;
  uint64_t r = 0, l = 0;
  for (auto& dev : ctx->devs)
    if (dev.online) {
      r += dev.online->requests.load();
      l += dev.online->launches.load();
    }
  if (requests) *requests = r;
  if (launches) *launches = l;
  return MV_OK;
}

mv_status mv_queue_stats(mv_ctx* ctx, uint64_t* calls, uint64_t* passes) {
  if (!ctx) return MV_E_INVALID_ARG;
  if (calls) *calls = ctx->q_calls.load();
  if (passes) *passes = ctx->q_passes.load();
  return MV_OK;
}

mv_status mv_dev_ed25519_verify(mv_ctx* ctx, int device, const uint8_t* d_msg, const uint8_t* d_sig,
                                const uint8_t* d_pk, uint32_t n, uint8_t* d_status, void* stream) {
  if (!ctx || (n && (!d_msg || !d_sig || !d_pk || !d_status))) return set_err(ctx, MV_E_INVALID_ARG, "bad args");
  if ((((uintptr_t)d_msg) | ((uintptr_t)d_sig) | ((uintptr_t)d_pk)) & 15)
    return set_err(ctx, MV_E_INVALID_ARG, "device inputs must be 16-byte aligned");
  std::lock_guard<std::mutex> lk(ctx->mu);
  Device* dev = find_dev(ctx, device);
  if (!dev) return set_err(ctx, MV_E_NO_DEVICE, "device not in context");
  HIPCHK(ctx, hipSetDevice(dev->id));
  reap_idle(ctx, *dev);
  hipStream_t s = stream ? (hipStream_t)stream : dev->stream;
  return enqueue_verify(ctx, *dev, d_msg, d_sig, d_pk, nullptr, n, d_status, s);
}

mv_status mv_dev_ed25519_verify_batch(mv_ctx* ctx, int device, const uint8_t* d_msg, const uint8_t* d_sig,
                                      const uint8_t* d_pk, const uint32_t* d_key_idx, uint32_t n,
                                      uint8_t* d_status, uint32_t* d_batch_ok, void* stream) {
  if (!ctx || (n && (!d_msg || !d_sig || !d_pk || !d_status))) return set_err(ctx, MV_E_INVALID_ARG, "bad args");
  if ((((uintptr_t)d_msg) | ((uintptr_t)d_sig) | ((uintptr_t)d_pk)) & 15)
    return set_err(ctx, MV_E_INVALID_ARG, "device inputs must be 16-byte aligned");
  std::lock_guard<std::mutex> lk(ctx->mu);
  Device* dev = find_dev(ctx, device);
  if (!dev) return set_err(ctx, MV_E_NO_DEVICE, "device not in context");
  if (n == 0) return MV_OK;
  HIPCHK(ctx, hipSetDevice(dev->id));
  reap_idle(ctx, *dev);
  hipStream_t s = stream ? (hipStream_t)stream : dev->stream;
  return enqueue_batch(ctx, *dev, d_msg, d_sig, d_pk, d_key_idx, n, d_status, s, d_batch_ok, nullptr, true);
}

mv_status mv_batch_counters(mv_ctx* ctx, uint64_t* out) {
  if (!ctx || !out) return MV_E_INVALID_ARG;
  mv_status st = mv_batch_stats(ctx, out, out + 1);
  out[2] = ctx->groups_run.load();
  out[3] = ctx->groups_failed.load();
  return st;
}

mv_status mv_batch_routes(mv_ctx* ctx, uint64_t* out) {
  if (!ctx || !out) return MV_E_INVALID_ARG;
  mv_status st = mv_batch_stats(ctx, out, nullptr);
  out[1] = ctx->single_batches.load();
  out[2] = ctx->dense_failures.load();
  return st;
}

mv_status mv_set_batch_groups(mv_ctx* ctx, uint32_t groups) {
  if (!ctx || groups > (uint32_t)mvk::BATCH_MAX_GROUPS) return set_err(ctx, MV_E_INVALID_ARG, "groups > 16");
  std::lock_guard<std::mutex> lk(ctx->mu);
  ctx->groups_fixed = groups;
  ctx->guard_left = 0;
  ctx->single_left = 0;
  return MV_OK;
}

mv_status mv_set_stage_timing(mv_ctx* ctx, int enable) {
  if (!ctx) return MV_E_INVALID_ARG;
  std::lock_guard<std::mutex> lk(ctx->mu);
  ctx->stage_timing = enable != 0;
  return MV_OK;
}

mv_status mv_stage_times(mv_ctx* ctx, double* ms, uint64_t* calls, int reset) {
  if (!ctx) return MV_E_INVALID_ARG;
  std::lock_guard<std::mutex> lk(ctx->tmu);
  for (auto& pe : ctx->pending) {
    HIPCHK(ctx, hipSetDevice(pe.device));
    mvr::EventSet& ev = pe.events;
    HIPCHK(ctx, hipEventSynchronize(ev.back()));
    for (size_t i = 0; i + 1 < ev.size(); i++) {
      float t = 0;
      HIPCHK(ctx, hipEventElapsedTime(&t, ev[i], ev[i + 1]));
      ctx->stage_ms[pe.first_stage + i] += t;
      ctx->stage_calls[pe.first_stage + i]++;
    }
    ev.release();
  }
  ctx->pending.clear();
  for (int i = 0; i < MV_NSTAGES; i++) {
    if (ms) ms[i] = ctx->stage_ms[i];
    if (calls) calls[i] = ctx->stage_calls[i];
  }
  if (reset) {
    for (double& x : ctx->stage_ms) x = 0;
    for (uint64_t& x : ctx->stage_calls) x = 0;
  }
  return MV_OK;
}

mv_status mv_batch_stats(mv_ctx* ctx, uint64_t* batches, uint64_t* fallbacks) {
  if (!ctx) return MV_E_INVALID_ARG;
  {
    std::lock_guard<std::mutex> lk(ctx->mu);
    for (auto& dev : ctx->devs) {
      (void)hipSetDevice(dev.id);
      poll_flags(ctx, dev);
    }
  }
  if (batches) *batches = ctx->batches.load();
  if (fallbacks) *fallbacks = ctx->fallbacks.load();
  return MV_OK;
}

mv_status mv_dev_ed25519_sign(mv_ctx* ctx, int device, const uint8_t* d_seed, const uint8_t* d_msg, uint32_t n,
                              uint8_t* d_pk, uint8_t* d_sig, void* stream) {
  if (!ctx || (n && (!d_seed || !d_msg || !d_pk || !d_sig))) return set_err(ctx, MV_E_INVALID_ARG, "bad args");
  if ((((uintptr_t)d_seed) | ((uintptr_t)d_msg) | ((uintptr_t)d_pk) | ((uintptr_t)d_sig)) & 15)
    return set_err(ctx, MV_E_INVALID_ARG, "device buffers must be 16-byte aligned");
  std::lock_guard<std::mutex> lk(ctx->mu);
  Device* dev = find_dev(ctx, device);
  if (!dev) return set_err(ctx, MV_E_NO_DEVICE, "device not in context");
  HIPCHK(ctx, hipSetDevice(dev->id));
  hipStream_t s = stream ? (hipStream_t)stream : dev->stream;
  HIPCHK(ctx, mvk::launch_sign(d_seed, d_msg, n, dev->tab.btab.p, d_pk, d_sig, s));
  return MV_OK;
}

mv_status mv_selftest(mv_ctx* ctx, int op, const uint32_t* in, uint32_t n, uint32_t* out) {
  if (!ctx || (n && (!in || !out))) return set_err(ctx, MV_E_INVALID_ARG, "bad selftest args");
  std::lock_guard<std::mutex> lk(ctx->mu);
  Device& dev = ctx->devs[0];
  HIPCHK(ctx, hipSetDevice(dev.id));
  const bool wide = op >= mvk::SELFTEST_WIDE_OP;
  const size_t row = wide ? 256 : 64;
  HIPCHK(ctx, dev.hc.bytes.ensure(row * n + 64));
  HIPCHK(ctx, dev.hc.out2.ensure(row * n + 64));
  HIPCHK(ctx, hipMemcpyAsync(dev.hc.bytes.p, in, row * n, hipMemcpyHostToDevice, dev.stream));
  if (wide)
    HIPCHK(ctx, mvk::launch_selftest_wide(op, dev.hc.bytes.as<uint32_t>(), n, dev.hc.out2.as<uint32_t>(), dev.stream));
  else
    HIPCHK(ctx, mvk::launch_selftest(op, dev.hc.bytes.as<uint32_t>(), n, dev.tab.btab.p, dev.hc.out2.as<uint32_t>(), dev.stream));
  HIPCHK(ctx, hipMemcpyAsync(out, dev.hc.out2.p, row * n, hipMemcpyDeviceToHost, dev.stream));
  HIPCHK(ctx, hipStreamSynchronize(dev.stream));
  return MV_OK;
}

mv_status mv_selftest_batch_prep(mv_ctx* ctx, const uint8_t* msg, const uint8_t* sig, const uint8_t* pk,
                                 const uint32_t* key_idx, uint32_t n, uint32_t groups, const uint8_t* key,
                                 uint32_t launch_sigs, uint32_t* scal, uint32_t* pts, uint64_t* bsum,
                                 uint8_t* status, uint32_t* info) {
  if (!ctx || !key || !bsum || !info || (n && (!msg || !sig || !scal || !pts || !status || (!pk == !key_idx))))
    return set_err(ctx, MV_E_INVALID_ARG, "bad batch prep args: exactly one of pk / key_idx");
  if (launch_sigs % 256) return set_err(ctx, MV_E_INVALID_ARG, "launch_sigs must be a multiple of 256");
  std::lock_guard<std::mutex> lk(ctx->mu);
  Device& dev = ctx->devs[0];
  if (key_idx) {
    if (!ctx->has_committee || !dev.committee_loaded)
      return set_err(ctx, MV_E_NO_COMMITTEE, "key_idx given but no committee set");
    for (uint32_t i = 0; i < n; i++)
      if (key_idx[i] >= ctx->committee.size()) return set_err(ctx, MV_E_INVALID_ARG, "key_idx out of range");
  }
  info[0] = info[1] = info[2] = 0;
  memset(bsum, 0, sizeof(uint64_t) * 12 * mvk::BATCH_MAX_GROUPS);
  if (n == 0) return MV_OK;
  HIPCHK(ctx, hipSetDevice(dev.id));
  constexpr size_t kPtRow = 128, kScRow = 48;
  const size_t bsum_bytes = sizeof(uint64_t) * 12 * mvk::BATCH_MAX_GROUPS;
  mvr::DevBuf d_msg, d_sig, d_pk, d_pts, d_scal, d_bsum, d_status;
  mvr::Event ready;
  HIPCHK(ctx, d_msg.ensure(32 * (size_t)n));
  HIPCHK(ctx, d_sig.ensure(64 * (size_t)n));
  HIPCHK(ctx, d_pk.ensure((pk ? 32 : 4) * (size_t)n));
  HIPCHK(ctx, d_pts.ensure(2 * kPtRow * (size_t)n));
  HIPCHK(ctx, d_scal.ensure(kScRow * (size_t)n));
  HIPCHK(ctx, d_bsum.ensure(bsum_bytes));
  HIPCHK(ctx, d_status.ensure(n));
  HIPCHK(ctx, ready.ensure());
  hipStream_t s = dev.stream;
  HIPCHK(ctx, hipMemcpyAsync(d_msg.p, msg, 32 * (size_t)n, hipMemcpyHostToDevice, s));
  HIPCHK(ctx, hipMemcpyAsync(d_sig.p, sig, 64 * (size_t)n, hipMemcpyHostToDevice, s));
  HIPCHK(ctx, hipMemcpyAsync(d_pk.p, pk ? (const void*)pk : key_idx, (pk ? 32 : 4) * (size_t)n, hipMemcpyHostToDevice, s));
  HIPCHK(ctx, hipMemsetAsync(d_pts.p, 0xff, 2 * kPtRow * (size_t)n, s));
  HIPCHK(ctx, hipMemsetAsync(d_scal.p, 0xff, kScRow * (size_t)n, s));
  HIPCHK(ctx, hipMemsetAsync(d_status.p, 0xff, n, s));
  HIPCHK(ctx, hipMemsetAsync(d_bsum.p, 0xff, bsum_bytes, s));
  uint32_t kw[10];
  memcpy(kw, key, 40);
  std::vector<uint32_t> ends;
  std::vector<hipEvent_t> evs;
  if (launch_sigs)
    for (uint64_t o = launch_sigs;; o += launch_sigs) {
      ends.push_back((uint32_t)std::min<uint64_t>(o, n));
      evs.push_back(ready);
      if (o >= n) break;
    }
  HIPCHK(ctx, hipEventRecord(ready, s));
  const mvk::ChunkGate gate{evs.data(), (uint32_t)ends.size(), ends.data()};
  const bool com_a = key_idx && !(ctx->flags & MV_FLAG_NO_COMB);
  mvk::BatchPrepInfo pi{};
  HIPCHK(ctx, mvk::launch_batch_prep(ctx->kn, d_msg.as<uint8_t>(), d_sig.as<uint8_t>(),
                                     pk ? d_pk.as<uint8_t>() : dev.tab.committee_pk.as<uint8_t>(),
                                     pk ? nullptr : d_pk.as<uint32_t>(), n, groups, kw, d_pts.p, d_scal.p, d_bsum.p,
                                     d_status.as<uint8_t>(), s, com_a ? dev.tab.combA.p : nullptr,
                                     com_a ? dev.tab.keyok.as<uint8_t>() : nullptr,
                                     com_a ? (uint32_t)ctx->committee.size() : 0u, launch_sigs ? &gate : nullptr, &pi));
  HIPCHK(ctx, hipMemcpyAsync(scal, d_scal.p, kScRow * (size_t)n, hipMemcpyDeviceToHost, s));
  HIPCHK(ctx, hipMemcpyAsync(pts, d_pts.p, (pi.a_rows ? 2 : 1) * kPtRow * (size_t)n, hipMemcpyDeviceToHost, s));
  HIPCHK(ctx, hipMemcpyAsync(bsum, d_bsum.p, bsum_bytes, hipMemcpyDeviceToHost, s));
  HIPCHK(ctx, hipMemcpyAsync(status, d_status.p, n, hipMemcpyDeviceToHost, s));
  HIPCHK(ctx, hipStreamSynchronize(s));
  info[0] = pi.groups;
  info[1] = pi.group_sigs;
  info[2] = pi.a_rows;
  return MV_OK;
}

mv_status mv_selftest_batch_msm(mv_ctx* ctx, uint32_t n, uint32_t groups, const uint32_t* scal, const uint32_t* pts,
                                const uint64_t* bsum, const uint32_t* key_idx, uint32_t n_keys, uint32_t* win,
                                uint32_t* asum, uint32_t* flags, uint32_t* info) {
  if (!ctx || !bsum || !win || !asum || !flags || !info || (n && (!scal || !pts)))
    return set_err(ctx, MV_E_INVALID_ARG, "bad batch msm args");
  std::lock_guard<std::mutex> lk(ctx->mu);
  Device& dev = ctx->devs[0];
  if (key_idx) {
    if (!ctx->has_committee || !dev.committee_loaded || (ctx->flags & MV_FLAG_NO_COMB))
      return set_err(ctx, MV_E_NO_COMMITTEE, "key_idx given but no committee with comb tables set");
    if (n_keys == 0 || n_keys > ctx->committee.size() || n_keys > 512 || ctx->kn.no_key_agg)
      return set_err(ctx, MV_E_INVALID_ARG, "per-key form: 1..512 keys of the committee, MV_NO_KEY_AGG off");
    for (uint32_t i = 0; i < n; i++)
      if (key_idx[i] >= n_keys) return set_err(ctx, MV_E_INVALID_ARG, "key_idx out of range");
  }
// ... 49 lines not shown
```

mysticeti_amd/csrc/engine_internal.h:

```cpp
#pragma once
#include <hip/hip_runtime.h>

#include <atomic>
#include <condition_variable>
#include <deque>
#include <memory>
#include <mutex>
#include <shared_mutex>
#include <string>
#include <thread>
#include <vector>

#include "../../include/mysti_verify.h"
#include "block_codec.h"
#include "dev_resources.h"
#include "kernels.h"

namespace mvi {

constexpr int kBlockStage0 = mvk::BATCH_STAGES;

constexpr int kBlockStages = 4;
constexpr int kWalStage0 = kBlockStage0 + kBlockStages;
static_assert(kWalStage0 + 2 == MV_NSTAGES, "stage count");

using mvr::DevBuf;
using mvr::HostBuf;

struct OnlineSvc;

struct Device {
  int id = 0;
  int cus = 0;
  bool committee_loaded = false;
  mvr::Stream stream;

  struct Tables {
    DevBuf btab, combB;
    DevBuf committee_pk, stakes, combA, keyok;
  } tab;

  struct HostCall {
    DevBuf msg, sig, pk, keyidx, status, bytes, off, len, out2;
    HostBuf h_in, h_out;
  } hc;

#ifndef MV_SLOTS
#define MV_SLOTS 3
#endif
  static constexpr int kSlots = MV_SLOTS;
  static constexpr int kFlagWords = 1 + mvk::BATCH_MAX_GROUPS;
  static constexpr int kFlagRing = 16;
  struct BatchPath {
    struct Scratch {
      DevBuf b, v;
    };
    mvr::ScratchRing<Scratch, kSlots> ring;
    DevBuf rejects;
    HostBuf h_flags;
    uint32_t flag_groups[kFlagRing] = {};
    mvr::Event flag_ev[kFlagRing];
    int flag_next = 0;
    mvr::Event prep_chain;
    bool prep_chained = false;
    const uint32_t* flags(int e) const { return h_flags.as<uint32_t>() + e * kFlagWords; }
    uint32_t* flags(int e) { return h_flags.as<uint32_t>() + e * kFlagWords; }
  } batch;

  struct SinglePath {
    mvr::ScratchRing<DevBuf, kSlots> ring;
  } single;

#ifndef MV_BLK_SLOTS
#define MV_BLK_SLOTS 3
#endif
  static constexpr int kBlkSlots = MV_BLK_SLOTS;
  struct BlkAux {
    mvr::Event ev[2];
    mvr::Stream stream;
  };
  struct BlockPath {
    mvr::ScratchRing<DevBuf, kBlkSlots> ring;
    BlkAux aux[kBlkSlots];
  } blk;

  static constexpr int kPinBufs = 3;
  static constexpr int kMaxChunks = 64;
  static constexpr int kSigCalls = 4;
  struct PinnedPath {
    DevBuf pin_msg[kPinBufs], pin_sig[kPinBufs], pin_pk[kPinBufs], pin_st[kPinBufs];
    HostBuf sig_stage[kSigCalls];
    mvr::Event sig_done[kSigCalls][2];
    bool sig_busy[kSigCalls] = {};
    mvr::Event pin_free[kPinBufs];
    mvr::EventSet chunk_ev[kPinBufs];
    int pin_next = 0;
    mvr::Stream pstream[2];
  } pin;

  static constexpr int kPassSets = 4;
  struct PassSet {
    HostBuf h_in, h_out;
    DevBuf bytes, out2, scr;
    BlkAux aux;
    mvr::Event done;
    hipStream_t stream = nullptr;
    const void* it = nullptr;
    uint64_t lo = 0;
    uint32_t m = 0;
    bool inflight = false;
  };
  struct PassSets {
    PassSet set[kPassSets];
    mvr::Stream qstream[kPassSets];
  } pass;

  struct Wal {
    DevBuf tab, rec, mcount, mflag, moff, ent, ff, img, pos, tag, len, st;
    DevBuf rctl, rscr, rows, rsum;
  } wal;

  struct Frames {
    DevBuf s, f, o, in, tab;
  } frm;

  struct Index {
    DevBuf tab, ctl;
    DevBuf item, keys, out, wg;
    DevBuf acc, accv, in, tab_in, miss;
    HostBuf h_ctl;
    uint64_t slots = 0;
    uint64_t used = 0;
    bool used_exact = true;
    mvr::Event ahead;
    bool ahead_set = false;
    uint64_t rebuilds = 0;
    uint32_t tag_bits = 64;
    struct Pending {
      DevBuf blk[2], inc[2];
      int cur = 0;
      uint64_t nb = 0, ni = 0, cap_b = 0, cap_i = 0, levels = 0;
      DevBuf cand_slot, cand_dst, lvl, hit, newbase, rows;
      DevBuf row_of;
    } pend;
    struct Dag {
      bool on = false;
      DevBuf rec, inc, map;
      uint64_t nb = 0, ni = 0, cap_b = 0, cap_i = 0, map_slots = 0;
      DevBuf src, newbase, lead, state, lists, sup, res, cmask, cm, marks, span;
    } dag;
  } index;

  struct Seal {
    DevBuf keys, heads, tab, md, bd, in, ol, st, seeds;
    HostBuf h;
  } seal;

  std::shared_ptr<OnlineSvc> online;
};

struct PendingEvents {
  int device;
  int first_stage;
  mvr::EventSet events;
};

}

struct mv_ctx {
  std::mutex mu;
  std::vector<mvi::Device> devs;
  std::string err;
  uint32_t max_batch = 1u << 20;
  uint32_t flags = 0;
  uint32_t secret[8] = {0};
  uint64_t index_secret[2] = {0};
  std::atomic<uint64_t> calls{0};
  std::atomic<uint64_t> batches{0}, fallbacks{0}, groups_run{0}, groups_failed{0};
  uint32_t groups_fixed = 0;
  uint32_t base_groups = 1;
  uint32_t guard_groups = 8;
  std::atomic<int> guard_left{0};
  std::atomic<int> single_left{0};
  std::atomic<uint64_t> single_batches{0}, dense_failures{0};
  bool stage_timing = false;
  std::mutex tmu;
  std::vector<mvi::PendingEvents> pending;
  double stage_ms[MV_NSTAGES] = {0};
  uint64_t stage_calls[MV_NSTAGES] = {0};
  std::atomic<bool> has_committee{false};
  std::condition_variable sig_cv;
  mvh::Committee committee;
  struct BlockReq;
  std::mutex q_mu;
  std::condition_variable q_cv;
  std::deque<BlockReq*> q;
  bool q_packing = false;
  bool q_set_busy[mvi::Device::kPassSets] = {};
  int q_sets = 0;
  std::condition_variable q_linger_cv;
  bool q_lingering = false;
  size_t q_last_calls = 0;
  std::atomic<uint64_t> q_calls{0}, q_passes{0};
  std::shared_mutex com_mu;
  std::atomic<uint64_t> online_rr{0};
  std::vector<size_t> online_devs;
  mvk::Knobs kn;
};

struct mv_ctx::BlockReq {
  const uint8_t* buf;
  const uint64_t *off, *len;
  uint32_t n;
  uint8_t *status, *md, *bd;
  mv_status rc = MV_OK;
  std::string err;
  bool taken = false;
  std::atomic<bool> done{false};
};

namespace mvi {

inline thread_local std::string* t_err = nullptr;

inline void record_err(mv_ctx* ctx, const std::string& msg) {
  if (t_err) *t_err = msg;
  else if (ctx) ctx->err = msg;
}

#define HIPCHK(ctx, expr)                                                                          \
  do {                                                                                             \
    hipError_t e_ = (expr);                                                                        \
    if (e_ != hipSuccess) {                                                                        \
      record_err((ctx), std::string(#expr) + ": " + hipGetErrorString(e_));                        \
      return MV_E_HIP;                                                                             \
    }                                                                                              \
  } while (0)

#define HIPCHK_RC(ctx, rc, expr)                                                  \
  do {                                                                            \
    hipError_t e_ = (expr);                                                       \
    if (e_ != hipSuccess && (rc) == MV_OK) {                                      \
      record_err((ctx), std::string(#expr) + ": " + hipGetErrorString(e_));       \
      (rc) = MV_E_HIP;                                                            \
    }                                                                             \
  } while (0)

inline mv_status set_err(mv_ctx* ctx, mv_status code, const std::string& msg) {
  record_err(ctx, msg);
  return code;
}

template <class Fn>
mv_status for_each_cut(mv_ctx* ctx, const std::vector<uint64_t>& cut, Fn fn) {
  const size_t nd = ctx->devs.size();
  std::vector<mv_status> rc(nd, MV_OK);
  std::vector<std::string> errs(nd);
  std::vector<std::thread> th;
  for (size_t d = 0; d < nd; d++) {
    const uint64_t lo = cut[d], hi = cut[d + 1];
    if (lo == hi) continue;
    th.emplace_back([&, d, lo, hi] {
      t_err = &errs[d];
      rc[d] = fn(ctx->devs[d], lo, hi);
      t_err = nullptr;
    });
  }
  for (auto& t : th) t.join();
  for (size_t d = 0; d < nd; d++)
    if (rc[d] != MV_OK) {
      ctx->err = errs[d];
      return rc[d];
    }
  return MV_OK;
}

template <class Fn>
mv_status for_each_shard(mv_ctx* ctx, uint64_t n, Fn fn) {
  const size_t nd = ctx->devs.size();
  if (nd == 1 || n < 2 * 256) return fn(ctx->devs[0], 0, n);
  std::vector<uint64_t> cut(nd + 1);
  for (size_t d = 0; d <= nd; d++) cut[d] = n * d / nd;
  return for_each_cut(ctx, cut, fn);
}

inline mv_status make_events(mv_ctx* ctx, int count, mvr::EventSet& evs) {
  evs.release();
  if (!ctx->stage_timing) return MV_OK;
  HIPCHK(ctx, evs.ensure(count + 1, hipEventDefault));
  return MV_OK;
}

inline void keep_events(mv_ctx* ctx, int device, int first_stage, mvr::EventSet& evs) {
  if (evs.empty()) return;
  std::lock_guard<std::mutex> lk(ctx->tmu);
  ctx->pending.push_back(PendingEvents{device, first_stage, std::move(evs)});
}

constexpr uint32_t kOnSlots = mvk::ONLINE_SLOTS, kOnMax = mvk::ONLINE_MAX_BLOCKS;
constexpr size_t kOnInCap = mvk::ONLINE_IN_CAP;
constexpr size_t kOnInStride = mvk::ONLINE_IN_STRIDE;
constexpr size_t kOnOutStride = mvk::ONLINE_OUT_STRIDE;

struct OnlineSvc {
  std::mutex mu;
  bool ready = false, launched = false;
  std::atomic<bool> failed{false};
  bool stuck = false;
  struct Resources {
    HostBuf ctl, req, in, out;
    DevBuf dctl, scr;
    mvr::Event exited;
    mvr::Stream stream;
    void abandon() {
      for (HostBuf* b : {&ctl, &req, &in, &out}) b->abandon();
      dctl.abandon();
      scr.abandon();
      exited.abandon();
      stream.abandon();
    }
  } res;
  mvk::OnlineCtl* ctl = nullptr;
  mvk::OnlineReq* req = nullptr;
  uint8_t* in = nullptr;
  uint8_t* out = nullptr;
  void *ctl_d = nullptr, *req_d = nullptr, *in_d = nullptr, *out_d = nullptr;
  std::unique_ptr<std::atomic<uint64_t>[]> freed;
  int max_spinners = 4;
  std::atomic<int> spinners{0}, sleepers{0};
  std::unique_ptr<std::atomic<uint32_t>[]> dwake;
  std::unique_ptr<std::atomic<uint64_t>[]> sleep_q;
  std::unique_ptr<std::atomic<uint32_t>[]> fseq, fwait;
  std::thread reaper;
  std::mutex rmu;
  std::condition_variable rcv;
  bool rstop = false;
  uint64_t next_q = 0;
  uint32_t grid = 0, launch_no = 0;
  std::atomic<uint64_t> requests{0}, launches{0};
  uint64_t idle_us = 10000;
  bool trace = false, debug = false;
  double ticks_per_us = 100.0;
  std::mutex tr_mu;
  double tr_sum[14] = {};
  uint64_t tr_n = 0;
};

inline Device* find_dev(mv_ctx* ctx, int device) {
  for (auto& d : ctx->devs)
    if (d.id == device) return &d;
  return nullptr;
}

void poll_flags(mv_ctx* ctx, Device& dev);
mv_status enqueue_batch(mv_ctx* ctx, Device& dev, const uint8_t* d_msg, const uint8_t* d_sig, const uint8_t* d_pk,
                        const uint32_t* d_key_idx, uint32_t n, uint8_t* d_status, hipStream_t s,
                        uint32_t* flag_dst, const mvk::ChunkGate* gate = nullptr, bool caller_stream = false);
mv_status enqueue_verify(mv_ctx* ctx, Device& dev, const uint8_t* d_msg, const uint8_t* d_sig, const uint8_t* d_pk,
                         const uint32_t* d_key_idx, uint32_t n, uint8_t* d_status, hipStream_t s);
mv_status enqueue_committee_verify(mv_ctx* ctx, Device& dev, const uint8_t* d_msg, const uint8_t* d_sig,
                                   const uint32_t* d_kidx, uint32_t n, uint8_t* d_status, hipStream_t s,
                                   const mvk::BlockVerdictOut* bv = nullptr, const mvk::BlockHashIn* hin = nullptr,
                                   const mvk::BlockIngestIn* ing = nullptr);
bool committee_ready(mv_ctx* ctx);
bool host_pinned(const void* p);
bool pinned_range_holds(const void* p, uint64_t bytes);
void reap_idle(mv_ctx* ctx, Device& dev);

mv_status enqueue_blocks(mv_ctx* ctx, Device& dev, const uint8_t* d_buf, uint64_t buf_bytes, const uint64_t* d_off,
                         const uint64_t* d_len, uint32_t n, uint8_t* d_status, uint8_t* d_md, uint8_t* d_bd,
                         hipStream_t s, DevBuf* own = nullptr, Device::BlkAux* own_aux = nullptr);
std::vector<uint64_t> balanced_cuts(const uint64_t* w, uint64_t n, uint32_t parts);

constexpr size_t ix_al(size_t x) { return (x + 255) & ~(size_t)255; }
using Index = Device::Index;
using Pending = Device::Index::Pending;
using Dag = Device::Index::Dag;
mvk::IndexTable table_of(mv_ctx* ctx, const Index& ix);
mv_status index_dev(mv_ctx* ctx, Device*& dev);
mv_status index_ctl(mv_ctx* ctx, Device& dev, hipStream_t s);
mv_status read_ctl(mv_ctx* ctx, Device& dev, hipStream_t s, const uint64_t** words);
mv_status order_behind_ahead(mv_ctx* ctx, Device& dev, hipStream_t s);
mv_status index_room_for_more(mv_ctx* ctx, Device& dev, uint64_t more, bool can_grow, hipStream_t s);
mv_status insert_rounds(mv_ctx* ctx, Device& dev, const mvk::IndexKeys& ks, uint64_t n, uint32_t state, hipStream_t s);
struct AcceptOut {
  uint64_t n_missing = 0;
  const uint8_t *status = nullptr, *state = nullptr;
  const uint64_t* missing = nullptr;
  mvk::AcceptArrays a{};
  uint64_t ncand = 0, ninc = 0;
};
mv_status accept_run(mv_ctx* ctx, Device& dev, const uint8_t* d_buf, uint64_t buf_bytes, const uint64_t* d_off,
                     const uint64_t* d_len, const uint64_t* d_grp, uint32_t n32, uint64_t cap_missing, bool can_grow,
                     hipStream_t s, AcceptOut& out, bool connect = false);
mv_status stage_blocks(mv_ctx* ctx, Device& dev, const uint8_t* buf, const uint64_t* off, const uint64_t* len,
                       const uint64_t* grp, uint32_t n, uint64_t cap_missing, hipStream_t s, AcceptOut& ao, bool connect);

mvk::PendStore pend_view(const Pending& pd, int k);
mv_status pending_room(mv_ctx* ctx, Device& dev, uint64_t more_b, uint64_t more_i, bool can_grow, hipStream_t s);

mvk::DagStore dag_view(const Dag& dg, const DevBuf& rec, const DevBuf& inc, uint64_t cap_b, uint64_t cap_i);
mvk::DagStore dag_view(const Dag& dg);
mv_status dag_room(mv_ctx* ctx, Device& dev, uint64_t more_b, uint64_t more_i, hipStream_t s, bool can_grow = true);
mv_status dag_seed_run(mv_ctx* ctx, Device& dev, const uint8_t* d_img, uint64_t size, const uint64_t* d_rows,
                       const uint8_t* d_status, uint64_t n, uint64_t floor_round, bool can_grow, hipStream_t s,
                       uint64_t* seeded);

bool online_eligible(mv_ctx* ctx, uint32_t n, uint64_t bytes, uint64_t longest);
mv_status online_verify(mv_ctx* ctx, Device& dev, const uint8_t* buf, const uint64_t* off, const uint64_t* len,
                        uint32_t n, uint8_t* status, uint8_t* md, uint8_t* bd);
bool online_stop(OnlineSvc& o);
void online_release(OnlineSvc& o);

}
```

mysticeti_amd/csrc/fe25519.h:

```cpp
#pragma once
#include <hip/hip_runtime.h>
#include <stdint.h>

#define MV_DEV __device__ __forceinline__

#include "carry32.h"

namespace mv {

constexpr uint32_t M29 = (1u << 29) - 1;
constexpr uint32_t R261 = 1216;

struct fe {
  uint32_t v[9];
};

MV_DEV void fe_normalize(fe& r) {
  uint32_t c;
#pragma unroll
  for (int i = 0; i < 8; i++) {
    c = r.v[i] >> 29;
    r.v[i] &= M29;
    r.v[i + 1] += c;
  }
// ... 139 lines not shown
}

MV_DEV void fe_mul2(fe& r0, const fe& a0, const fe& b0, fe& r1, const fe& a1, const fe& b1) {
  fe_mul(r0, a0, b0);
  fe_mul(r1, a1, b1);
}
MV_DEV void fe_sq2(fe& r0, const fe& a0, fe& r1, const fe& a1) {
  fe_sq(r0, a0);
  fe_sq(r1, a1);
}

MV_DEV void fe_canon(fe& r, const fe& a) {
  fe t = a;
  fe_normalize(t);
#pragma unroll
  for (int it = 0; it < 2; it++) {
    uint32_t q = t.v[8] >> 23;
    t.v[8] &= (1u << 23) - 1;
    t.v[0] += q * 19u;
    uint32_t c;
#pragma unroll
    for (int i = 0; i < 8; i++) {
      c = t.v[i] >> 29;
      t.v[i] &= M29;
      t.v[i + 1] += c;
    }
  }
  uint32_t u[9];
  uint32_t c = 19;
#pragma unroll
  for (int i = 0; i < 9; i++) {
    uint32_t s = t.v[i] + c;
    c = s >> 29;
    u[i] = s & M29;
  }
  const bool ge = (u[8] >> 23) != 0;
  u[8] &= (1u << 23) - 1;
#pragma unroll
  for (int i = 0; i < 9; i++) r.v[i] = ge ? u[i] : t.v[i];
}
MV_DEV bool fe_is_zero(const fe& a) {
  fe c;
  fe_canon(c, a);
  uint32_t o = 0;
#pragma unroll
  for (int i = 0; i < 9; i++) o |= c.v[i];
  return o == 0;
}
MV_DEV bool fe_eq(const fe& a, const fe& b) {
  fe d;
  fe_sub(d, a, b);
  return fe_is_zero(d);
}
MV_DEV bool fe_is_negative(const fe& a) {
  fe c;
  fe_canon(c, a);
  return c.v[0] & 1u;
}
MV_DEV void fe_cmov(fe& r, const fe& a, bool c) {
#pragma unroll
  for (int i = 0; i < 9; i++) r.v[i] = c ? a.v[i] : r.v[i];
}
MV_DEV void fe_from_words_full(fe& r, const uint32_t w[8]) {
#pragma unroll
  for (int i = 0; i < 9; i++) {
    const int b = 29 * i, wi = b >> 5, s = b & 31;
    uint32_t lo = w[wi];
    uint32_t hi = (wi + 1 < 8) ? w[wi + 1] : 0u;
    r.v[i] = __builtin_amdgcn_alignbit(hi, lo, s) & M29;
  }
}
MV_DEV void fe_from_words(fe& r, const uint32_t w[8]) {
  fe_from_words_full(r, w);
  r.v[8] &= (1u << 23) - 1;
}
MV_DEV void fe_to_words(uint32_t w[8], const fe& a) {
  fe c;
  fe_canon(c, a);
#pragma unroll
  for (int j = 0; j < 8; j++) {
    const int b = 32 * j, li = b / 29, s = b % 29;
    uint32_t x = c.v[li] >> s;
    if (li + 1 < 9) x |= c.v[li + 1] << (29 - s);
    if (s > 26 && li + 2 < 9) x |= c.v[li + 2] << (58 - s);
    w[j] = x;
  }
}

MV_DEV void fe_pow22501(fe& t19, fe& t3, const fe& x) {
  fe t0, t1, t2, t5, t7, t13, t15, a;
  fe_sq(t0, x);
  fe_sqn(t1, t0, 2);
  fe_mul(t2, x, t1);
  fe_mul(t3, t0, t2);
  fe_sq(a, t3);
  fe_mul(t5, t2, a);
  fe_sqn(a, t5, 5);
  fe_mul(t7, a, t5);
  fe_sqn(a, t7, 10);
  fe_mul(t1, a, t7);
  fe_sqn(a, t1, 20);
  fe_mul(a, a, t1);
  fe_sqn(a, a, 10);
  fe_mul(t13, a, t7);
  fe_sqn(a, t13, 50);
  fe_mul(t15, a, t13);
  fe_sqn(a, t15, 100);
  fe_mul(a, a, t15);
  fe_sqn(a, a, 50);
  fe_mul(t19, a, t13);
}
MV_DEV void fe_invert(fe& r, const fe& x) {
  fe t19, t3;
  fe_pow22501(t19, t3, x);
  fe_sqn(t19, t19, 5);
  fe_mul(r, t19, t3);
}
MV_DEV void fe_pow_p58(fe& r, const fe& x) {
  fe t19, t3;
  fe_pow22501(t19, t3, x);
  fe_sqn(t19, t19, 2);
  fe_mul(r, t19, x);
}
MV_DEV void fe_sq2n(fe& a, fe& b, int n) {
#pragma unroll 1
  for (int i = 0; i < n; i++) fe_sq2(a, a, b, b);
}
MV_DEV void fe_pow_p58_x2(fe& ra, fe& rb, const fe& xa, const fe& xb) {
  fe a0, b0, a2, b2, a3, b3, a5, b5, a7, b7, a13, b13, a15, b15, ta, tb;
  fe_sq2(a0, xa, b0, xb);
  ta = a0; tb = b0; fe_sq2n(ta, tb, 2);
  fe_mul2(a2, xa, ta, b2, xb, tb);
  fe_mul2(a3, a0, a2, b3, b0, b2);
  fe_sq2(ta, a3, tb, b3);
  fe_mul2(a5, a2, ta, b5, b2, tb);
  ta = a5; tb = b5; fe_sq2n(ta, tb, 5);
  fe_mul2(a7, ta, a5, b7, tb, b5);
  ta = a7; tb = b7; fe_sq2n(ta, tb, 10);
  fe_mul2(a2, ta, a7, b2, tb, b7);
  ta = a2; tb = b2; fe_sq2n(ta, tb, 20);
  fe_mul2(ta, ta, a2, tb, tb, b2);
  fe_sq2n(ta, tb, 10);
  fe_mul2(a13, ta, a7, b13, tb, b7);
  ta = a13; tb = b13; fe_sq2n(ta, tb, 50);
  fe_mul2(a15, ta, a13, b15, tb, b13);
  ta = a15; tb = b15; fe_sq2n(ta, tb, 100);
  fe_mul2(ta, ta, a15, tb, tb, b15);
  fe_sq2n(ta, tb, 50);
  fe_mul2(ta, ta, a13, tb, tb, b13);
  fe_sq2n(ta, tb, 2);
  fe_mul2(ra, ta, xa, rb, tb, xb);
}

MV_DEV void fe_pow_p58_x2_nox(fe& ra, fe& rb, const fe& xa, const fe& xb) {
  fe a0, b0, a2, b2, a3, b3, a5, b5, a7, b7, a13, b13, a15, b15, ta, tb;
  fe_sq2(a0, xa, b0, xb);
  ta = a0; tb = b0; fe_sq2n(ta, tb, 2);
  fe_mul2(a2, xa, ta, b2, xb, tb);
  fe_mul2(a3, a0, a2, b3, b0, b2);
  fe_sq2(ta, a3, tb, b3);
  fe_mul2(a5, a2, ta, b5, b2, tb);
  ta = a5; tb = b5; fe_sq2n(ta, tb, 5);
  fe_mul2(a7, ta, a5, b7, tb, b5);
  ta = a7; tb = b7; fe_sq2n(ta, tb, 10);
  fe_mul2(a2, ta, a7, b2, tb, b7);
  ta = a2; tb = b2; fe_sq2n(ta, tb, 20);
  fe_mul2(ta, ta, a2, tb, tb, b2);
  fe_sq2n(ta, tb, 10);
  fe_mul2(a13, ta, a7, b13, tb, b7);
  ta = a13; tb = b13; fe_sq2n(ta, tb, 50);
  fe_mul2(a15, ta, a13, b15, tb, b13);
  ta = a15; tb = b15; fe_sq2n(ta, tb, 100);
  fe_mul2(ta, ta, a15, tb, tb, b15);
  fe_sq2n(ta, tb, 50);
  fe_mul2(ta, ta, a13, tb, tb, b13);
  fe_sq2n(ta, tb, 2);
  ra = ta;
  rb = tb;
}

}
```

mysticeti_amd/csrc/ge25519.h:

```cpp
#pragma once
#include "fe25519.h"

namespace mv {

struct p3 { fe X, Y, Z, T; };
struct p2 { fe X, Y, Z; };
struct p1p1 { fe X, Y, Z, T; };
struct cached { fe YpX, YmX, Z, T2d; };
struct precomp { fe ypx, ymx, xy2d; };

__constant__ const uint32_t K_D[8] = {0x135978a3, 0x75eb4dca, 0x4141d8ab, 0x00700a4d,
                                      0x7779e898, 0x8cc74079, 0x2b6ffe73, 0x52036cee};
__constant__ const uint32_t K_D2[8] = {0x26b2f159, 0xebd69b94, 0x8283b156, 0x00e0149a,
                                       0xeef3d130, 0x198e80f2, 0x56dffce7, 0x2406d9dc};
__constant__ const uint32_t K_SQRTM1[8] = {0x4a0ea0b0, 0xc4ee1b27, 0xad2fe478, 0x2f431806,
                                           0x3dfbd7a7, 0x2b4d0099, 0x4fc1df0b, 0x2b832480};

MV_DEV void fe_const(fe& r, const uint32_t* c) {
  uint32_t w[8];
#pragma unroll
  for (int i = 0; i < 8; i++) w[i] = c[i];
  fe_from_words_full(r, w);
}

// ... 60 lines not shown
  fe_sub(r.T, ZZ2, TT);
}
template <MulOrder O = MulOrder::chained>
MV_DEV void p3_add_precomp(p1p1& r, const p3& p, const precomp& q) {
  fe PP, MM, TT, Z2, ypx, ymx;
  fe_add(ypx, p.Y, p.X);
  fe_sub(ymx, p.Y, p.X);
  fe_mul<O>(PP, ypx, q.ypx);
  fe_mul<O>(MM, ymx, q.ymx);
  fe_mul<O>(TT, p.T, q.xy2d);
  fe_add(Z2, p.Z, p.Z);
  fe_sub(r.X, PP, MM);
  fe_add(r.Y, PP, MM);
  fe_addn(r.Z, Z2, TT);
  fe_sub(r.T, Z2, TT);
}
MV_DEV void cached_cneg(cached& c, bool neg) {
#pragma unroll
  for (int i = 0; i < 9; i++) {
    uint32_t a = c.YpX.v[i], b = c.YmX.v[i];
    c.YpX.v[i] = neg ? b : a;
    c.YmX.v[i] = neg ? a : b;
  }
  fe n;
  fe_neg(n, c.T2d);
  fe_cmov(c.T2d, n, neg);
}
MV_DEV void precomp_cneg(precomp& c, bool neg) {
#pragma unroll
  for (int i = 0; i < 9; i++) {
    uint32_t a = c.ypx.v[i], b = c.ymx.v[i];
    c.ypx.v[i] = neg ? b : a;
    c.ymx.v[i] = neg ? a : b;
  }
  fe n;
  fe_neg(n, c.xy2d);
  fe_cmov(c.xy2d, n, neg);
}
MV_DEV void p3_neg(p3& r, const p3& p) {
  fe_neg(r.X, p.X);
  r.Y = p.Y;
  r.Z = p.Z;
  fe_neg(r.T, p.T);
}
MV_DEV bool p3_is_identity(const p3& p) { return fe_is_zero(p.X) && fe_eq(p.Y, p.Z); }

MV_DEV bool sqrt_ratio_finish(fe& r, const fe& u, const fe& v, const fe& r0) {
  fe i, check, t, ui;
  fe_const(i, K_SQRTM1);
  fe_sq(t, r0);
  fe_mul(check, v, t);
  fe_add(t, check, u);
  bool flipped = fe_is_zero(t);
  bool correct = fe_eq(check, u);
  fe_mul(ui, u, i);
  fe_add(t, check, ui);
  bool flipped_i = fe_is_zero(t);
  fe ri;
  fe_mul(ri, r0, i);
  r = r0;
  fe_cmov(r, ri, flipped || flipped_i);
  fe nr;
  fe_neg(nr, r);
  fe_cmov(r, nr, fe_is_negative(r));
  return correct || flipped;
}

MV_DEV void decompress_x2(p3& A, bool& okA, const uint32_t ea[8], p3& R, bool& okR, const uint32_t er[8]) {
  fe d, one;
  fe_const(d, K_D);
  fe_set(one, 1);
  fe ya, yr, ua, ur, va, vr, t;
  fe_from_words(ya, ea);
  fe_from_words(yr, er);
  fe_sq(t, ya);
  fe_sub(ua, t, one);
  fe_mul(va, t, d);
  fe_add(va, va, one);
  fe_sq(t, yr);
  fe_sub(ur, t, one);
  fe_mul(vr, t, d);
  fe_add(vr, vr, one);
  fe v3a, v3r, ea7, er7;
  fe_sq(t, va); fe_mul(v3a, t, va);
  fe_sq(t, vr); fe_mul(v3r, t, vr);
  fe_sq(t, v3a); fe_mul(ea7, t, va); fe_mul(ea7, ea7, ua);
  fe_sq(t, v3r); fe_mul(er7, t, vr); fe_mul(er7, er7, ur);
  fe pa, pr;
  fe_pow_p58_x2(pa, pr, ea7, er7);
  fe_mul(pa, pa, v3a); fe_mul(pa, pa, ua);
  fe_mul(pr, pr, v3r); fe_mul(pr, pr, ur);
  fe xa, xr;
  okA = sqrt_ratio_finish(xa, ua, va, pa);
  okR = sqrt_ratio_finish(xr, ur, vr, pr);
  fe n;
  fe_neg(n, xa);
  fe_cmov(xa, n, (ea[7] >> 31) != 0);
  fe_neg(n, xr);
  fe_cmov(xr, n, (er[7] >> 31) != 0);
  A.X = xa; A.Y = ya; fe_set(A.Z, 1); fe_mul(A.T, xa, ya);
  R.X = xr; R.Y = yr; fe_set(R.Z, 1); fe_mul(R.T, xr, yr);
}

MV_DEV void decompress1(p3& A, bool& okA, const uint32_t ea[8]) {
  fe d, one, ya, ua, va, t, v3a, ea7, pa, xa, n;
  fe_const(d, K_D);
  fe_set(one, 1);
  fe_from_words(ya, ea);
  fe_sq(t, ya);
  fe_sub(ua, t, one);
  fe_mul(va, t, d);
  fe_add(va, va, one);
  fe_sq(t, va); fe_mul(v3a, t, va);
  fe_sq(t, v3a); fe_mul(ea7, t, va); fe_mul(ea7, ea7, ua);
  fe_pow_p58(pa, ea7);
  fe_mul(pa, pa, v3a); fe_mul(pa, pa, ua);
  okA = sqrt_ratio_finish(xa, ua, va, pa);
  fe_neg(n, xa);
  fe_cmov(xa, n, (ea[7] >> 31) != 0);
  A.X = xa; A.Y = ya; fe_set(A.Z, 1); fe_mul(A.T, xa, ya);
}

MV_DEV void decompress1_lean(p3& A, bool& okA, const uint32_t ea[8]) {
  fe pa;
  {
    fe d, one, ya, ua, va, t, ea7;
    fe_const(d, K_D);
    fe_set(one, 1);
    fe_from_words(ya, ea);
    fe_sq(t, ya);
    fe_sub(ua, t, one);
    fe_mul(va, t, d);
    fe_add(va, va, one);
    fe_sq(t, va); fe_mul(ea7, t, va);
    fe_sq(t, ea7); fe_mul(ea7, t, va); fe_mul(ea7, ea7, ua);
    fe_pow_p58(pa, ea7);
  }
  fe d, one, ya, ua, va, t, v3a, xa, n;
  fe_const(d, K_D);
  fe_set(one, 1);
  fe_from_words(ya, ea);
  fe_sq(t, ya);
  fe_sub(ua, t, one);
  fe_mul(va, t, d);
  fe_add(va, va, one);
  fe_sq(t, va); fe_mul(v3a, t, va);
  fe_mul(pa, pa, v3a); fe_mul(pa, pa, ua);
  okA = sqrt_ratio_finish(xa, ua, va, pa);
  fe_neg(n, xa);
  fe_cmov(xa, n, (ea[7] >> 31) != 0);
  A.X = xa; A.Y = ya; fe_set(A.Z, 1); fe_mul(A.T, xa, ya);
}

template <class Get>
MV_DEV void decompress2_lean(p3& A, bool& okA, p3& R, bool& okR, Get get) {
  fe pa, pr;
  {
    fe xa, xr;
    {
      fe d, one, y, u, v, t;
      uint32_t ea[8], er[8];
      get(0, ea);
      get(1, er);
      fe_const(d, K_D);
      fe_set(one, 1);
      fe_from_words(y, ea);
      fe_sq(t, y);
      fe_sub(u, t, one);
      fe_mul(v, t, d);
      fe_add(v, v, one);
      fe_sq(t, v); fe_mul(xa, t, v);
      fe_sq(t, xa); fe_mul(xa, t, v); fe_mul(xa, xa, u);
      fe_from_words(y, er);
      fe_sq(t, y);
      fe_sub(u, t, one);
      fe_mul(v, t, d);
      fe_add(v, v, one);
      fe_sq(t, v); fe_mul(xr, t, v);
      fe_sq(t, xr); fe_mul(xr, t, v); fe_mul(xr, xr, u);
    }
    fe_pow_p58_x2_nox(pa, pr, xa, xr);
  }
  auto finish = [](p3& P, bool& ok, const uint32_t e[8], fe& p) {
    fe d, one, y, u, v, t, v3, x, n;
    fe_const(d, K_D);
    fe_set(one, 1);
    fe_from_words(y, e);
    fe_sq(t, y);
    fe_sub(u, t, one);
    fe_mul(v, t, d);
    fe_add(v, v, one);
    fe_sq(t, v); fe_mul(v3, t, v);
    fe_sq(t, v3); fe_mul(t, t, v); fe_mul(t, t, u);
    fe_mul(p, p, t);
    fe_mul(p, p, v3); fe_mul(p, p, u);
    ok = sqrt_ratio_finish(x, u, v, p);
    fe_neg(n, x);
    fe_cmov(x, n, (e[7] >> 31) != 0);
    P.X = x; P.Y = y; fe_set(P.Z, 1); fe_mul(P.T, x, y);
  };
  uint32_t e[8];
  get(0, e);
  finish(A, okA, e, pa);
  get(1, e);
  finish(R, okR, e, pr);
}

}
```

mysticeti_amd/csrc/kernels.h:

```cpp
#pragma once
#include <hip/hip_runtime.h>
#include <stddef.h>
#include <stdint.h>

namespace mvk {
struct Knobs {
  int64_t blk_pipe = 1;
  int64_t comb_split_bytes = 2048;
  int64_t hash_in_comb = 1;
  int64_t ingest_in_comb = 1;
  int64_t verdict_fused = 1;
  int64_t blk_chunk_bytes = 256ll << 20;
  int64_t pack_threads = 0;
  int64_t blk_trace = 0;
  int64_t blk_zerocopy = 1ll << 20;
  int64_t pass_spin = 0;
  int64_t pass_sets = 2;
  int64_t q_linger_us = 50;
  int64_t q_spin_us = 0;
  int64_t online = 1;
  int64_t online_long = 1;
  int64_t online_prio = 1;
  int64_t online_wgs = 0;
  int64_t online_idle_us = 10000;
  int64_t online_trace = 0;
  int64_t online_debug = 0;
  int64_t online_inject = 0;
  int64_t online_spinners = 0;
  int64_t stream_chunk_log2 = 17;
  int64_t guard_groups = 8;
  int64_t base_groups = 1;
  double stream_fracs[8] = {0.7, 0.3};
  int n_stream_fracs = 2;
  int64_t no_key_agg = 0;
  int64_t reduce_quad = 16384;
  int64_t b2_lane = 1;
  int64_t comb_quad = -1;
  int64_t reduce_rows = 1024;
  int64_t final_rows = 1;
  int64_t bucket_bal = 1;
  int64_t sort_wide = 0;
  int64_t prep_chain = 1;
  int64_t blk_walk = 1;
  int64_t index_tag_bits = 64;
};

size_t verify_scratch_bytes(uint32_t n);
size_t btable_bytes();
hipError_t launch_btable_init(void* d_btab, hipStream_t s);
hipError_t launch_verify(const uint8_t* msg, const uint8_t* sig, const uint8_t* pk, const uint32_t* key_idx, uint32_t n,
                         const void* btab, void* scratch, uint8_t* status, hipStream_t s, const uint32_t* skip = nullptr,
                         uint32_t skip_group = 0, const void* prep_pts = nullptr, const void* prep_comb = nullptr);
hipError_t launch_count_rejects(const uint8_t* status, uint32_t n, uint32_t* count, hipStream_t s);
hipError_t launch_sign(const uint8_t* seed, const uint8_t* msg, uint32_t n, const void* btab, uint8_t* pk,
                       uint8_t* sig, hipStream_t s);
hipError_t launch_blake2b(const Knobs& kn, const uint8_t* buf, const uint64_t* off, const uint64_t* len, uint32_t n, uint8_t* out,
                          hipStream_t s);
hipError_t launch_block_hash(const Knobs& kn, const uint8_t* buf, const uint64_t* off, const uint64_t* len, uint32_t n,
                             uint8_t* msg_out, uint8_t* dig_out, hipStream_t s);
hipError_t launch_blake2b_quad(const Knobs& kn, const uint8_t* buf, const uint64_t* off, const uint64_t* len, uint32_t n, uint8_t* out,
                               hipStream_t s);
hipError_t launch_block_hash_quad(const Knobs& kn, const uint8_t* buf, const uint64_t* off, const uint64_t* len, uint32_t n,
                                  uint8_t* msg_out, uint8_t* dig_out, hipStream_t s);
hipError_t launch_blake2b_lane(const uint8_t* buf, const uint64_t* off, const uint64_t* len, uint32_t n, uint8_t* out,
                               hipStream_t s);
hipError_t launch_block_hash_lane(const uint8_t* buf, const uint64_t* off, const uint64_t* len, uint32_t n,
                                  uint8_t* msg_out, uint8_t* dig_out, hipStream_t s);
hipError_t launch_selftest(int op, const uint32_t* in, uint32_t n, const void* btab, uint32_t* out, hipStream_t s);
constexpr int SELFTEST_WIDE_OP = 64;
constexpr int SELFTEST_SCALAR_OP = 112;
hipError_t launch_selftest_wide(int op, const uint32_t* in, uint32_t n, uint32_t* out, hipStream_t s);
struct ChunkGate {
  const hipEvent_t* ready;
  uint32_t n;
  const uint32_t* end;
};
constexpr int BATCH_STAGES = 6;
constexpr int BATCH_MAX_GROUPS = 16;
size_t batch_scratch_bytes(uint32_t n, uint32_t groups);
uint32_t batch_group_size(uint32_t n, uint32_t groups);
hipError_t launch_verify_batch(const Knobs& kn, const uint8_t* msg, const uint8_t* sig, const uint8_t* pk, const uint32_t* key_idx,
                               uint32_t n, uint32_t groups, const uint32_t key[10], const void* btab,
                               void* bscratch, void* vscratch, uint8_t* status, hipStream_t s,
                               uint32_t** flag_out, hipEvent_t* ev = nullptr, const void* comb_a = nullptr,
                               const uint8_t* key_ok = nullptr, uint32_t n_keys = 0, const void* comb_b = nullptr,
                               const struct ChunkGate* gate = nullptr, const hipEvent_t* chain = nullptr);
struct BatchPrepInfo {
  uint32_t groups, group_sigs, a_rows;
};
hipError_t launch_batch_prep(const Knobs& kn, const uint8_t* msg, const uint8_t* sig, const uint8_t* pk,
                             const uint32_t* key_idx, uint32_t n, uint32_t groups, const uint32_t key[10], void* pts,
                             void* scal, void* bsum, uint8_t* status, hipStream_t s, const void* comb_a,
                             const uint8_t* key_ok, uint32_t n_keys, const struct ChunkGate* gate,
                             BatchPrepInfo* info);
struct BatchMsmInfo {
  uint32_t groups, group_sigs, nw;
  const uint4* win;
  const uint4* asum;
  const uint32_t* flag;
};
hipError_t launch_batch_msm(const Knobs& kn, uint32_t n, uint32_t groups, const void* h_scal, const void* h_pts,
                            const void* h_bsum, const uint32_t* key_idx, uint32_t n_keys, const void* comb_a,
                            const void* comb_b, void* bscratch, size_t scratch_bytes, hipStream_t s,
                            BatchMsmInfo* info);
size_t comb_table_bytes(uint32_t nbases);
hipError_t launch_comb_init(const uint8_t* enc, uint32_t nb, int negate, void* tab, uint8_t* ok, hipStream_t s);
struct BlockVerdictOut {
  const uint32_t* facts;
  const uint8_t* claimed;
  uint8_t* msg_digest;
  uint8_t* digest;
  uint8_t* status;
};
struct BlockHashIn {
  const uint8_t* stage;
  const uint64_t* pre_off;
  const uint64_t* pre_len;
  uint8_t* msg_digest;
  uint8_t* digest;
};
struct BlockIngestIn {
  const uint8_t* buf;
  const uint64_t* off;
  const uint64_t* len;
  const uint64_t* stakes;
  uint32_t n_auth;
  uint64_t epoch, quorum_thr;
  uint8_t* stage;
  uint64_t* pre_off;
  uint64_t* pre_len;
  uint8_t* sig;
  uint32_t* key_idx;
  uint32_t* facts;
  uint8_t* claimed;
};
#ifndef MV_ONLINE_SLOTS
#define MV_ONLINE_SLOTS 128
#endif
constexpr uint32_t ONLINE_SLOTS = MV_ONLINE_SLOTS;
constexpr uint32_t ONLINE_MAX_BLOCKS = 64;
constexpr uint32_t ONLINE_JOBS = 16 * ONLINE_SLOTS;
constexpr uint32_t ONLINE_MAX_WGS = 256;
constexpr uint32_t ONLINE_WG_LEFT = 0x80000000u;
constexpr uint64_t ONLINE_EXIT_STOP = 1, ONLINE_EXIT_IDLE = 2, ONLINE_EXIT_MAX = 3;
constexpr size_t ONLINE_IN_CAP = 128u << 10;
constexpr size_t online_al(size_t x) { return (x + 255) & ~(size_t)255; }
constexpr size_t ONLINE_IN_STRIDE = online_al(16 * ONLINE_MAX_BLOCKS + ONLINE_IN_CAP + 64);
constexpr size_t ONLINE_OUT_STRIDE = online_al(65 * ONLINE_MAX_BLOCKS);
constexpr size_t ONLINE_O_OUT = ONLINE_IN_STRIDE;
constexpr size_t ONLINE_O_STAGE = ONLINE_O_OUT + ONLINE_OUT_STRIDE;
constexpr size_t ONLINE_O_POFF = ONLINE_O_STAGE + online_al(ONLINE_IN_CAP + 4096);
constexpr size_t ONLINE_O_PLEN = ONLINE_O_POFF + online_al(8 * ONLINE_MAX_BLOCKS);
constexpr size_t ONLINE_O_SIG = ONLINE_O_PLEN + online_al(8 * ONLINE_MAX_BLOCKS);
constexpr size_t ONLINE_O_KIDX = ONLINE_O_SIG + online_al(64 * ONLINE_MAX_BLOCKS);
constexpr size_t ONLINE_O_FACTS = ONLINE_O_KIDX + online_al(4 * ONLINE_MAX_BLOCKS);
constexpr size_t ONLINE_O_CLAIMED = ONLINE_O_FACTS + online_al(4 * ONLINE_MAX_BLOCKS);
constexpr size_t ONLINE_O_SST = ONLINE_O_CLAIMED + online_al(32 * ONLINE_MAX_BLOCKS);
constexpr size_t ONLINE_SCR_STRIDE = ONLINE_O_SST + online_al(ONLINE_MAX_BLOCKS);
constexpr uint32_t INGEST_WINDOW_BYTES = 10240;
struct OnlineReq {
  uint64_t seq;
  uint32_t n;
  uint32_t copy_bytes;
};
struct OnlineCtl {
  uint64_t tail;
  uint64_t stop;
  uint64_t done[ONLINE_SLOTS];
  uint64_t trace[ONLINE_SLOTS][14];
  uint32_t wg[ONLINE_MAX_WGS];
  uint64_t exit_why, exit_ready, exit_head, exit_tail;
};
struct OnlineDev {
  unsigned long long ready;
  unsigned long long jobs_head;
  unsigned long long jobs_tail;
  uint32_t quit, epoch;
  uint32_t n[ONLINE_SLOTS];
  uint32_t jobs_done[ONLINE_SLOTS];
  unsigned long long moved[ONLINE_SLOTS];
  unsigned long long jobs[ONLINE_JOBS];
  uint64_t sink[2 * 1024];
};
struct OnlineArgs {
  OnlineCtl* ctl;
  const OnlineReq* reqs;
  OnlineDev* dev;
  const uint8_t* in_host;
  uint8_t* out_host;
  uint8_t* scr;
  const void* combB;
  const void* combA;
  const uint8_t* key_ok;
  const uint8_t* pk;
  const uint64_t* stakes;
  uint64_t epoch, quorum_thr;
  uint32_t n_auth;
  uint32_t launch;
  uint64_t idle_ticks, max_ticks;
};
hipError_t launch_online(const OnlineArgs& a, uint32_t grid, hipStream_t s);
hipError_t launch_verify_comb(const Knobs& kn, const uint8_t* msg, const uint8_t* sig, const uint8_t* pk, const uint32_t* key_idx,
                              uint32_t n, const void* combB, const void* combA, const uint8_t* key_ok,
                              uint8_t* status, hipStream_t s, const BlockVerdictOut* bv = nullptr,
                              const BlockHashIn* hin = nullptr, const BlockIngestIn* ing = nullptr);
bool comb_short_chain(const Knobs& kn, uint32_t n);
hipError_t launch_hash_comb_pre(const uint8_t* stage, const uint64_t* poff, const uint64_t* plen, uint32_t n,
                                uint8_t* md, uint8_t* bd, const uint8_t* sig, const void* combB, void* rbuf,
                                void* sbuf, uint8_t* qflags, hipStream_t s);
hipError_t launch_comb_post(const uint8_t* msg, const uint8_t* sig, const uint8_t* pk, const uint32_t* key_idx,
                            uint32_t n, const void* combA, const uint8_t* key_ok, const void* rbuf,
                            const void* sbuf, const uint8_t* qflags, uint8_t* status, hipStream_t s,
                            const BlockVerdictOut* bv = nullptr);
hipError_t launch_block_parse(const uint8_t* buf, const uint64_t* off, const uint64_t* len, uint32_t n,
                              const uint64_t* stakes, uint32_t n_auth, uint64_t epoch, uint64_t quorum_thr,
                              uint8_t* stage, uint64_t* pre_off, uint64_t* pre_len, uint8_t* sig, uint32_t* key_idx,
                              uint32_t* facts, uint8_t* claimed, hipStream_t s);
hipError_t launch_block_walk(const uint8_t* buf, const uint64_t* off, const uint64_t* len, uint32_t n,
                             const uint64_t* stakes, uint32_t n_auth, uint64_t epoch, uint64_t quorum_thr,
                             uint8_t* sig, uint32_t* key_idx, uint32_t* facts, uint8_t* claimed, uint8_t* md,
                             uint8_t* bd, hipStream_t s);
hipError_t launch_block_digest_gate(const uint8_t* claimed, const uint8_t* digest, const uint32_t* facts, uint32_t n,
                                    uint8_t* sig, hipStream_t s);
hipError_t launch_block_verdict(const uint32_t* facts, const uint8_t* claimed, uint8_t* msg_digest, uint8_t* digest,
                                const uint8_t* sig_status, uint32_t n, uint8_t* status, hipStream_t s);
size_t wal_table_words();
void wal_build_tables(uint32_t* out);
hipError_t launch_crc32(const uint8_t* buf, const uint64_t* off, const uint64_t* len, uint32_t n,
                        const uint32_t* tables, uint32_t* out, int cus, hipStream_t s);
constexpr uint8_t WAL_MAP_EMPTY = 0, WAL_MAP_NEXT = 1, WAL_MAP_END = 2, WAL_MAP_BAD = 3;
// ... 278 lines not shown
```

rust/mysti-verify-sys/src/lib.rs:

```rust
#![allow(non_camel_case_types)]
use std::os::raw::{c_char, c_void};

#[repr(C)]
pub struct mv_ctx {
    _p: [u8; 0],
}

#[repr(C)]
#[derive(Default, Clone, Copy)]
pub struct mv_config {
    pub device_mask: u32,
    pub max_batch: u32,
    pub flags: u32,
    pub shards_per_device: u32,
}

pub const MV_OK: i32 = 0;
pub const MV_E_INVALID_ARG: i32 = -1;
pub const MV_E_HIP: i32 = -2;
pub const MV_E_NO_DEVICE: i32 = -3;
pub const MV_E_NO_COMMITTEE: i32 = -4;
pub const MV_E_ALLOC: i32 = -5;
pub const MV_E_INDEX_FULL: i32 = -6;

pub const MV_REF_ABSENT: u8 = 0;
pub const MV_REF_WANTED: u8 = 1;
pub const MV_REF_HAVE: u8 = 2;
pub const MV_REF_STORED: u8 = 3;

pub const MV_ACC_REJECTED: u8 = 0;
pub const MV_ACC_NEW: u8 = 1;
pub const MV_ACC_KNOWN: u8 = 2;
pub const MV_ACC_DUP: u8 = 3;
pub const MV_ACC_DROPPED: u8 = 4;
pub const MV_ACC_SUSPENDED: u8 = 5;

pub const MV_LEADER_UNDECIDED: u64 = 0;
pub const MV_LEADER_COMMIT: u64 = 1;
pub const MV_LEADER_SKIP: u64 = 2;
pub const MV_LEADER_CONFLICT: u64 = 3;
pub const MV_LEADER_OVERFLOW: u64 = 4;
pub const MV_DECIDE_MAX_LEADER_BLOCKS: u64 = 8;
pub const MV_COMMIT_KIND_NONE: u64 = 0;
pub const MV_COMMIT_KIND_DIRECT: u64 = 1;
pub const MV_COMMIT_KIND_INDIRECT: u64 = 2;
pub const MV_COMMIT_INCOMPLETE: u64 = 1;
pub const MV_COMMIT_BLOCKED: u64 = 2;

pub const MV_SIG_OK: u8 = 0;
pub const MV_SIG_INVALID: u8 = 1;
pub const MV_SIG_MALFORMED_KEY: u8 = 2;

pub const MV_BLOCK_OK: u8 = 0;
pub const MV_BLOCK_PARSE_ERROR: u8 = 1;
pub const MV_BLOCK_DIGEST_MISMATCH: u8 = 2;
pub const MV_BLOCK_EPOCH_MISMATCH: u8 = 3;
pub const MV_BLOCK_UNKNOWN_AUTHOR: u8 = 4;
pub const MV_BLOCK_GENESIS: u8 = 5;
pub const MV_BLOCK_SIG_INVALID: u8 = 6;
pub const MV_BLOCK_INCLUDE_UNKNOWN_AUTHORITY: u8 = 7;
pub const MV_BLOCK_INCLUDE_ROUND: u8 = 8;
pub const MV_BLOCK_VOTE_RANGE: u8 = 9;
pub const MV_BLOCK_THRESHOLD_CLOCK: u8 = 10;
pub const MV_BLOCK_VOTE_RANGE_TOO_LONG: u8 = 11;
pub const MV_BLOCK_VOTE_RANGE_END_TOO_LARGE: u8 = 12;

pub const MV_SEAL_OK: u8 = 0;
pub const MV_SEAL_PARSE_ERROR: u8 = 1;
pub const MV_SEAL_UNKNOWN_AUTHOR: u8 = 2;
pub const MV_SEAL_UNLINKED: u8 = 3;
pub const MV_SEAL_LINK: u32 = 1;

pub const MV_WAL_OK: u8 = 0;
pub const MV_WAL_CRC_MISMATCH: u8 = 1;
pub const MV_WAL_NONZERO_CRC_LEN0: u8 = 2;
pub const MV_WAL_BAD_LENGTH: u8 = 3;
pub const MV_WAL_UNKNOWN_TAG: u8 = 4;
pub const MV_WAL_BLOCK_DECODE: u8 = 5;
pub const MV_WAL_UNKNOWN_AUTHORITY: u8 = 6;

pub const MV_MSG_OK: u32 = 0;
pub const MV_MSG_DECODE_ERROR: u32 = 1;
pub const MV_MSG_BLOCK_REJECTED: u32 = 2;
pub const MV_MSG_TOO_MANY_REQUESTED: u32 = 3;
pub const MV_MSG_NOT_REACHED: u32 = 4;
pub const MV_MSG_BAD_SIZE: u32 = 5;

pub const MV_FLAG_NO_BATCH: u32 = 1;
pub const MV_FLAG_NO_COMB: u32 = 2;
pub const MV_FLAG_HOST_PARSE: u32 = 4;
pub const MV_FLAG_NO_ONLINE: u32 = 8;
pub const MV_BATCH_MIN: u32 = 4096;
pub const MV_NSTAGES: usize = 12;

extern "C" {
    pub fn mv_create(cfg: *const mv_config, out: *mut *mut mv_ctx) -> i32;
    pub fn mv_destroy(ctx: *mut mv_ctx);
    pub fn mv_last_error(ctx: *const mv_ctx) -> *const c_char;
    pub fn mv_version() -> *const c_char;
    pub fn mv_set_committee(ctx: *mut mv_ctx, pks: *const u8, stakes: *const u64, n: u32, epoch: u64,
                            key_ok: *mut u8) -> i32;
    pub fn mv_blake2b256(ctx: *mut mv_ctx, buf: *const u8, off: *const u64, len: *const u64, n: u32,
                         out: *mut u8) -> i32;
    pub fn mv_ed25519_verify(ctx: *mut mv_ctx, msg: *const u8, sig: *const u8, pk: *const u8,
                             key_idx: *const u32, n: u32, status: *mut u8) -> i32;
    pub fn mv_host_alloc(ctx: *mut mv_ctx, bytes: u64, out: *mut *mut c_void) -> i32;
    pub fn mv_host_free(ctx: *mut mv_ctx, p: *mut c_void);
    pub fn mv_ed25519_sign(ctx: *mut mv_ctx, seed: *const u8, msg: *const u8, n: u32, pk: *mut u8,
                           sig: *mut u8) -> i32;
    pub fn mv_verify_blocks(ctx: *mut mv_ctx, buf: *const u8, off: *const u64, len: *const u64, n: u32,
                            status: *mut u8, msg_digest: *mut u8, block_digest: *mut u8) -> i32;
    pub fn mv_block_preimage(bincode: *const u8, len: u64, out: *mut u8, cap: u64) -> i64;
    pub fn mv_queue_stats(ctx: *mut mv_ctx, calls: *mut u64, passes: *mut u64) -> i32;
    pub fn mv_online_stats(ctx: *mut mv_ctx, requests: *mut u64, launches: *mut u64) -> i32;
    pub fn mv_shard_plan(weights: *const u64, n: u64, parts: u32, cut: *mut u64) -> i32;
    pub fn mv_crc32(ctx: *mut mv_ctx, buf: *const u8, off: *const u64, len: *const u64, n: u32,
                    out: *mut u32) -> i32;
    pub fn mv_wal_verify(ctx: *mut mv_ctx, wal: *const u8, size: u64, end_pos: u64, map_bits: u32,
                         pos: *mut u64, tag: *mut u32, len: *mut u32, status: *mut u8, cap: u64,
                         count: *mut u64) -> i32;
    pub fn mv_wal_replay(ctx: *mut mv_ctx, wal: *const u8, size: u64, end_pos: u64, map_bits: u32,
                         pos: *mut u64, tag: *mut u32, len: *mut u32, status: *mut u8, cap: u64,
                         count: *mut u64, blk_rows: *mut u64, blk_status: *mut u8, cap_blocks: u64,
                         n_blocks: *mut u64, summary: *mut u64, last_seen: *mut u64) -> i32;
    pub fn mv_wal_recover(ctx: *mut mv_ctx, wal: *const u8, size: u64, end_pos: u64, map_bits: u32,
                          pos: *mut u64, tag: *mut u32, len: *mut u32, status: *mut u8, cap: u64,
                          count: *mut u64, blk_rows: *mut u64, blk_status: *mut u8, cap_blocks: u64,
                          n_blocks: *mut u64, summary: *mut u64, last_seen: *mut u64, floor_round: u64,
                          seeded: *mut u64) -> i32;
    pub fn mv_wal_layout(payload_len: *const u64, n: u64, map_bits: u32, start: u64, pos: *mut u64) -> u64;
    pub fn mv_frame_blocks(buf: *const u8, len: u64, off: *mut u64, blen: *mut u64, cap: u64,
                           consumed: *mut u64) -> i64;
    pub fn mv_frame_messages(buf: *const u8, len: u64, msgs: *mut u32, cap_msgs: u64, blk_off: *mut u64,
                             blk_len: *mut u64, cap_blocks: u64, n_blocks: *mut u64,
                             consumed: *mut u64) -> i64;
    pub fn mv_verify_frames(ctx: *mut mv_ctx, buf: *const u8, soff: *const u64, slen: *const u64, ns: u32,
                            consumed: *mut u64, drop_msg: *mut u32, msgs: *mut u32, cap_msgs: u64,
                            n_msgs: *mut u64, blk_off: *mut u64, blk_len: *mut u64, blk_status: *mut u8,
                            cap_blocks: u64, n_blocks: *mut u64) -> i32;
    pub fn mv_index_reserve(ctx: *mut mv_ctx, entries: u64) -> i32;
    pub fn mv_index_clear(ctx: *mut mv_ctx) -> i32;
    pub fn mv_index_stats(ctx: *mut mv_ctx, out: *mut u64) -> i32;
    pub fn mv_index_insert(ctx: *mut mv_ctx, refs: *const u64, n: u64, state: u32, prior: *mut u8) -> i32;
    pub fn mv_index_insert_stored(ctx: *mut mv_ctx, refs: *const u64, n: u64, prior: *mut u8) -> i32;
    pub fn mv_index_lookup(ctx: *mut mv_ctx, refs: *const u64, n: u64, state: *mut u8) -> i32;
    pub fn mv_index_wanted(ctx: *mut mv_ctx, refs: *mut u64, cap: u64, n: *mut u64) -> i32;
    pub fn mv_accept_blocks(ctx: *mut mv_ctx, buf: *const u8, off: *const u64, len: *const u64,
                            grp: *const u64, n: u32, blk_status: *mut u8, blk_state: *mut u8,
                            missing: *mut u64, cap_missing: u64, n_missing: *mut u64) -> i32;
    pub fn mv_dev_accept_blocks(ctx: *mut mv_ctx, device: i32, d_buf: *const u8, buf_bytes: u64,
                                d_off: *const u64, d_len: *const u64, d_grp: *const u64, n: u32,
                                d_blk_status: *mut u8, d_blk_state: *mut u8, d_missing: *mut u64,
                                cap_missing: u64, n_missing: *mut u64, stream: *mut c_void) -> i32;
    pub fn mv_connect_blocks(ctx: *mut mv_ctx, buf: *const u8, off: *const u64, len: *const u64,
                             grp: *const u64, n: u32, blk_status: *mut u8, blk_state: *mut u8,
                             missing: *mut u64, cap_missing: u64, n_missing: *mut u64,
                             connected: *mut u64, cap_connected: u64, n_connected: *mut u64) -> i32;
    pub fn mv_dev_connect_blocks(ctx: *mut mv_ctx, device: i32, d_buf: *const u8, buf_bytes: u64,
                                 d_off: *const u64, d_len: *const u64, d_grp: *const u64, n: u32,
                                 d_blk_status: *mut u8, d_blk_state: *mut u8, d_missing: *mut u64,
                                 cap_missing: u64, n_missing: *mut u64, d_connected: *mut u64,
                                 cap_connected: u64, n_connected: *mut u64, stream: *mut c_void) -> i32;
    pub fn mv_pending_reserve(ctx: *mut mv_ctx, blocks: u64, includes: u64) -> i32;
    pub fn mv_pending_stats(ctx: *mut mv_ctx, out: *mut u64) -> i32;
    pub fn mv_dag_reserve(ctx: *mut mv_ctx, blocks: u64, includes: u64) -> i32;
    pub fn mv_dag_prune(ctx: *mut mv_ctx, round: u64) -> i32;
    pub fn mv_dag_stats(ctx: *mut mv_ctx, out: *mut u64) -> i32;
    pub fn mv_decide_leaders(ctx: *mut mv_ctx, leaders: *const u64, n: u32, out: *mut u64, stakes: *mut u64) -> i32;
    pub fn mv_dev_decide_leaders(ctx: *mut mv_ctx, device: i32, d_leaders: *const u64, n: u32, d_out: *mut u64,
                                 d_stakes: *mut u64, stream: *mut c_void) -> i32;
    pub fn mv_commit_leaders(ctx: *mut mv_ctx, leaders: *const u64, n: u32, out: *mut u64, info: *mut u64,
                             n_sequence: *mut u64) -> i32;
    pub fn mv_dev_commit_leaders(ctx: *mut mv_ctx, device: i32, d_leaders: *const u64, n: u32, d_out: *mut u64,
                                 d_info: *mut u64, n_sequence: *mut u64, stream: *mut c_void) -> i32;
    pub fn mv_dev_index_insert(ctx: *mut mv_ctx, device: i32, d_words: *const u64, stride_words: u64, n: u64,
                               state: u32, stream: *mut c_void) -> i32;
    pub fn mv_dev_dag_seed_rows(ctx: *mut mv_ctx, device: i32, d_wal: *const u8, size: u64, d_blk_rows: *const u64,
                                d_blk_status: *const u8, n_rows: u64, floor_round: u64, seeded: *mut u64,
                                stream: *mut c_void) -> i32;
    pub fn mv_seal_blocks(ctx: *mut mv_ctx, buf: *mut u8, off: *const u64, len: *const u64, n: u32,
                          seeds: *const u8, n_auth: u32, flags: u32, status: *mut u8, msg_digest: *mut u8,
                          block_digest: *mut u8) -> i32;
    pub fn mv_dev_seal_blocks(ctx: *mut mv_ctx, device: i32, d_buf: *mut u8, buf_bytes: u64, d_off: *const u64,
                              d_len: *const u64, n: u32, d_seeds: *const u8, n_auth: u32, flags: u32,
                              d_status: *mut u8, d_msg_digest: *mut u8, d_block_digest: *mut u8,
                              stream: *mut c_void) -> i32;
    pub fn mv_dev_verify_frames(ctx: *mut mv_ctx, device: i32, d_buf: *const u8, buf_bytes: u64,
                                d_soff: *const u64, d_slen: *const u64, ns: u32, d_consumed: *mut u64,
                                d_drop_msg: *mut u32, d_msgs: *mut u32, cap_msgs: u64, n_msgs: *mut u64,
                                d_blk_off: *mut u64, d_blk_len: *mut u64, d_blk_status: *mut u8,
                                cap_blocks: u64, n_blocks: *mut u64, stream: *mut c_void) -> i32;
    pub fn mv_dev_ed25519_verify(ctx: *mut mv_ctx, device: i32, d_msg: *const u8, d_sig: *const u8,
                                 d_pk: *const u8, n: u32, d_status: *mut u8, stream: *mut c_void) -> i32;
    pub fn mv_dev_ed25519_verify_batch(ctx: *mut mv_ctx, device: i32, d_msg: *const u8, d_sig: *const u8,
                                       d_pk: *const u8, d_key_idx: *const u32, n: u32, d_status: *mut u8,
                                       d_batch_ok: *mut u32, stream: *mut c_void) -> i32;
    pub fn mv_dev_ed25519_sign(ctx: *mut mv_ctx, device: i32, d_seed: *const u8, d_msg: *const u8, n: u32,
                               d_pk: *mut u8, d_sig: *mut u8, stream: *mut c_void) -> i32;
    pub fn mv_dev_verify_blocks(ctx: *mut mv_ctx, device: i32, d_buf: *const u8, buf_bytes: u64,
                                d_off: *const u64, d_len: *const u64, n: u32, d_status: *mut u8,
                                d_msg_digest: *mut u8, d_block_digest: *mut u8, stream: *mut c_void) -> i32;
    pub fn mv_dev_wal_verify(ctx: *mut mv_ctx, device: i32, d_wal: *const u8, size: u64, end_pos: u64,
                             map_bits: u32, d_pos: *mut u64, d_tag: *mut u32, d_len: *mut u32,
                             d_status: *mut u8, cap: u64, count: *mut u64, stream: *mut c_void) -> i32;
    pub fn mv_dev_wal_replay(ctx: *mut mv_ctx, device: i32, d_wal: *const u8, size: u64, end_pos: u64,
                             map_bits: u32, d_pos: *mut u64, d_tag: *mut u32, d_len: *mut u32,
                             d_status: *mut u8, cap: u64, count: *mut u64, d_blk_rows: *mut u64,
                             d_blk_status: *mut u8, cap_blocks: u64, n_blocks: *mut u64,
                             d_summary: *mut u64, d_last_seen: *mut u64, stream: *mut c_void) -> i32;
    pub fn mv_dev_crc32(ctx: *mut mv_ctx, device: i32, d_buf: *const u8, d_off: *const u64, d_len: *const u64,
                        n: u32, d_out: *mut u32, stream: *mut c_void) -> i32;
    pub fn mv_batch_stats(ctx: *mut mv_ctx, batches: *mut u64, fallbacks: *mut u64) -> i32;
    pub fn mv_batch_counters(ctx: *mut mv_ctx, out: *mut u64) -> i32;
    pub fn mv_batch_routes(ctx: *mut mv_ctx, out: *mut u64) -> i32;
    pub fn mv_set_batch_groups(ctx: *mut mv_ctx, groups: u32) -> i32;
    pub fn mv_set_stage_timing(ctx: *mut mv_ctx, enable: i32) -> i32;
    pub fn mv_stage_times(ctx: *mut mv_ctx, ms: *mut f64, calls: *mut u64, reset: i32) -> i32;
    pub fn mv_selftest(ctx: *mut mv_ctx, op: i32, input: *const u32, n: u32, out: *mut u32) -> i32;
    pub fn mv_selftest_batch_prep(ctx: *mut mv_ctx, msg: *const u8, sig: *const u8, pk: *const u8,
                                  key_idx: *const u32, n: u32, groups: u32, key: *const u8, launch_sigs: u32,
                                  scal: *mut u32, pts: *mut u32, bsum: *mut u64, status: *mut u8,
                                  info: *mut u32) -> i32;
    pub fn mv_selftest_batch_msm(ctx: *mut mv_ctx, n: u32, groups: u32, scal: *const u32, pts: *const u32,
                                 bsum: *const u64, key_idx: *const u32, n_keys: u32, win: *mut u32,
                                 asum: *mut u32, flags: *mut u32, info: *mut u32) -> i32;
    pub fn mv_selftest_comb_table(ctx: *mut mv_ctx, key: i32, out: *mut u32) -> i32;
    pub fn mv_set_option(ctx: *mut mv_ctx, name: *const c_char, value: i64) -> i32;
    pub fn mv_get_option(ctx: *mut mv_ctx, name: *const c_char, value: *mut i64) -> i32;
}
```

Before: 348.1 million.

## Split batch prep into scalar kernel and point-decompression kernel, sort before prep

```diff
diff --git a/include/mysti_verify.h b/include/mysti_verify.h
--- a/include/mysti_verify.h
+++ b/include/mysti_verify.h
@@ -248,7 +248,7 @@
 mv_status mv_batch_counters(mv_ctx* ctx, uint64_t* out );
 mv_status mv_batch_routes(mv_ctx* ctx, uint64_t* out );
 mv_status mv_set_batch_groups(mv_ctx* ctx, uint32_t groups);
-#define MV_NSTAGES 12
+#define MV_NSTAGES 13
 mv_status mv_set_stage_timing(mv_ctx* ctx, int enable);
 mv_status mv_stage_times(mv_ctx* ctx, double* ms , uint64_t* calls ,
                          int reset);
diff --git a/mysticeti_amd/__init__.py b/mysticeti_amd/__init__.py
--- a/mysticeti_amd/__init__.py
+++ b/mysticeti_amd/__init__.py
@@ -60,7 +60,7 @@
 COMMIT_NO_ANCHOR = 0xFFFFFFFFFFFFFFFF
 WAL_MAP_BITS, WAL_MAP_BITS_TEST = 24, 16
 STAGES = ["prep", "sort", "bucket", "reduce", "final", "fallback", "parse", "hash", "verify", "verdict", "wal_walk",
-          "wal_crc"]
+          "wal_crc", "scal"]
 FLAG_NO_BATCH, FLAG_NO_COMB, FLAG_HOST_PARSE, FLAG_NO_ONLINE = 1, 2, 4, 8
 BATCH_MIN = 4096
 SELFTEST_WIDE_OP = 64
diff --git a/mysticeti_amd/csrc/batch.hip b/mysticeti_amd/csrc/batch.hip
--- a/mysticeti_amd/csrc/batch.hip
+++ b/mysticeti_amd/csrc/batch.hip
@@ -130,50 +130,23 @@
   uint32_t aggregate;
 };
 
-#ifndef MV_PREP_OCC
-#define MV_PREP_OCC 3
-#endif
-__global__ void __launch_bounds__(256, MV_PREP_OCC)
-    k_bv_prep(const uint8_t* __restrict__ msg, const uint8_t* __restrict__ sig, const uint8_t* __restrict__ pk,
-              const uint32_t* __restrict__ key_idx, uint32_t n, BvKey key, CommitteeA ca, uint4* __restrict__ pts,
-              uint4* __restrict__ scal, unsigned long long* __restrict__ bsum, uint8_t* __restrict__ status,
-              uint32_t blk0, uint32_t group_sigs) {
-  __shared__ unsigned long long sbsum[BSUM_WORDS];
-  __shared__ uint32_t va[8][256], vs[8][256], vz[4][256];
-#ifdef MV_PREP_X2
-  __shared__ uint32_t vr[8][256];
-#endif
-  const uint32_t t = threadIdx.x;
-  if (threadIdx.x < BSUM_WORDS) sbsum[threadIdx.x] = 0;
-  __syncthreads();
-  const uint32_t blk = blockIdx.x + blk0;
-  const uint32_t gid = blk * blockDim.x + threadIdx.x;
-  const bool live = gid < n;
-  const uint32_t idx = live ? gid : n - 1;
-
-  uint32_t aw[8], rw[8], sw[8], mw[8];
-  const uint32_t kid = key_idx ? key_idx[idx] : idx;
-  load8(aw, pk + 32 * (size_t)kid);
-  load8(rw, sig + 64 * (size_t)idx);
-  load8(sw, sig + 64 * (size_t)idx + 32);
-  load8(mw, msg + 32 * (size_t)idx);
+__global__ void __launch_bounds__(256, 2)
+    k_bv_scal(const uint8_t* __restrict__ msg, const uint8_t* __restrict__ sig, const uint8_t* __restrict__ pk,
+              const uint32_t* __restrict__ key_idx, uint32_t n, BvKey key, uint4* __restrict__ scal, uint32_t blk0) {
+  const uint32_t gid = (blockIdx.x + blk0) * blockDim.x + threadIdx.x;
+  if (gid >= n) return;
+  uint32_t sw[8];
+  load8(sw, sig + 64 * (size_t)gid + 32);
   const bool s_ok = sc_is_canonical(sw);
-#pragma unroll
-  for (int i = 0; i < 8; i++) {
-    va[i][t] = aw[i];
-    vs[i][t] = sw[i];
-  }
   uint32_t z[4], zk[8];
   {
     uint32_t k[8];
     {
       uint32_t kin[24], h[16];
-#pragma unroll
-      for (int i = 0; i < 8; i++) {
-        kin[i] = rw[i];
-        kin[8 + i] = aw[i];
-        kin[16 + i] = mw[i];
-      }
+      const uint32_t kid = key_idx ? key_idx[gid] : gid;
+      load8(kin, sig + 64 * (size_t)gid);
+      load8(kin + 8, pk + 32 * (size_t)kid);
+      load8(kin + 16, msg + 32 * (size_t)gid);
       sha512_short(h, kin, 96);
       sc_reduce512(k, h);
     }
@@ -197,23 +170,41 @@
     }
     sc_muladd(zk, z8, k, zero);
   }
-  uint4* sc = scal + (size_t)idx * SC_QUADS;
-#pragma unroll
-  for (int i = 0; i < 4; i++) vz[i][t] = z[i];
-  if (live) {
-    sc[0] = make_uint4(z[0], z[1], z[2], z[3]);
-    sc[1] = make_uint4(zk[0], zk[1], zk[2], zk[3]);
-    sc[2] = make_uint4(zk[4], zk[5], zk[6], zk[7]);
-  }
+  uint4* sc = scal + (size_t)gid * SC_QUADS;
+  const uint4 zq = make_uint4(0, 0, 0, 0);
+  sc[0] = s_ok ? make_uint4(z[0], z[1], z[2], z[3]) : zq;
+  sc[1] = s_ok ? make_uint4(zk[0], zk[1], zk[2], zk[3]) : zq;
+  sc[2] = s_ok ? make_uint4(zk[4], zk[5], zk[6], zk[7]) : zq;
+}
+
+#ifndef MV_PREP_OCC
+#define MV_PREP_OCC 3
+#endif
+__global__ void __launch_bounds__(256, MV_PREP_OCC)
+    k_bv_prep(const uint8_t* __restrict__ sig, const uint8_t* __restrict__ pk, const uint32_t* __restrict__ key_idx,
+              uint32_t n, CommitteeA ca, uint4* __restrict__ pts, uint4* __restrict__ scal,
+              unsigned long long* __restrict__ bsum, uint8_t* __restrict__ status, uint32_t blk0,
+              uint32_t group_sigs) {
+  __shared__ unsigned long long sbsum[BSUM_WORDS];
+  if (threadIdx.x < BSUM_WORDS) sbsum[threadIdx.x] = 0;
+  __syncthreads();
+  const uint32_t blk = blockIdx.x + blk0;
+  const uint32_t gid = blk * blockDim.x + threadIdx.x;
+  const bool live = gid < n;
+  const uint32_t idx = live ? gid : n - 1;
+  const uint32_t kid = key_idx ? key_idx[idx] : idx;
+  const bool a_rows = !(ca.tab && ca.aggregate);
 
   bool okA, okR;
   {
+    uint32_t ew[8];
     precomp pc;
+    p3 P;
+    load8(ew, sig + 64 * (size_t)idx);
+    decompress1_lean(P, okR, ew);
+    precomp_from_affine(pc, P);
+    if (live) pt_store(pts, gid, pc);
     if (ca.tab) {
-      p3 P;
-      decompress1_lean(P, okR, rw);
-      precomp_from_affine(pc, P);
-      if (live) pt_store(pts, gid, pc);
       okA = ca.ok[kid] != 0;
       if (!ca.aggregate) {
         const uint4* e = ca.tab + (size_t)kid * ca.stride + 8;
@@ -226,34 +217,26 @@
         if (live) pt_store(pts, (size_t)n + gid, pc);
       }
     } else {
-#ifdef MV_PREP_X2
-    p3 P, Q;
-#pragma unroll
-    for (int i = 0; i < 8; i++) vr[i][t] = rw[i];
-    decompress2_lean(Q, okA, P, okR, [&](int which, uint32_t (&e)[8]) {
       asm volatile("" ::: "memory");
-#pragma unroll
-      for (int i = 0; i < 8; i++) e[i] = which ? vr[i][t] : va[i][t];
-    });
-    precomp_from_affine(pc, P);
-    if (live) pt_store(pts, gid, pc);
-    precomp_from_affine(pc, Q);
-    if (live) pt_store(pts, (size_t)n + gid, pc);
-#else
-    p3 P;
-    decompress1_lean(P, okR, rw);
-    precomp_from_affine(pc, P);
-    if (live) pt_store(pts, gid, pc);
-    asm volatile("" ::: "memory");
-#pragma unroll
-    for (int i = 0; i < 8; i++) aw[i] = va[i][t];
-    decompress1_lean(P, okA, aw);
-    precomp_from_affine(pc, P);
-    if (live) pt_store(pts, (size_t)n + gid, pc);
-#endif
-    }
-  }
-  const bool ok = live && okA && okR && s_ok;
+      load8(ew, pk + 32 * (size_t)kid);
+      decompress1_lean(P, okA, ew);
+      precomp_from_affine(pc, P);
+      if (live) pt_store(pts, (size_t)n + gid, pc);
+    }
+    if (live && !(okA && okR)) {
+      fe_set(pc.ypx, 1);
+      fe_set(pc.ymx, 1);
+      fe_set(pc.xy2d, 0);
+      pt_store(pts, gid, pc);
+      if (a_rows) pt_store(pts, (size_t)n + gid, pc);
+    }
+  }
+  asm volatile("" ::: "memory");
+  uint32_t sw[8], z[4];
+  load8(sw, sig + 64 * (size_t)idx + 32);
+  uint4* sc = scal + (size_t)idx * SC_QUADS;
+  const uint4 z4 = sc[0];
+  const bool ok = live && okA && okR && sc_is_canonical(sw);
   if (live) {
     if (!ok) {
       const uint4 zq = make_uint4(0, 0, 0, 0);
@@ -263,11 +246,10 @@
     }
     status[gid] = !okA ? 2 : (ok ? 0 : 1);
   }
-  asm volatile("" ::: "memory");
-#pragma unroll
-  for (int i = 0; i < 4; i++) z[i] = ok ? vz[i][t] : 0u;
-#pragma unroll
-  for (int i = 0; i < 8; i++) sw[i] = vs[i][t];
+  z[0] = ok ? z4.x : 0u;
+  z[1] = ok ? z4.y : 0u;
+  z[2] = ok ? z4.z : 0u;
+  z[3] = ok ? z4.w : 0u;
   {
     uint64_t acc = 0;
     uint32_t c2 = 0;
@@ -1082,6 +1064,51 @@
 }
 
 namespace {
+struct StageMarks {
+  hipEvent_t* ev;
+  hipStream_t s;
+  void begin(int k) const { if (ev) (void)hipEventRecord(ev[2 * k], s); }
+  void end(int k) const { if (ev) (void)hipEventRecord(ev[2 * k + 1], s); }
+};
+constexpr int ST_PREP = 0, ST_SORT = 1, ST_BUCKET = 2, ST_REDUCE = 3, ST_FINAL = 4, ST_FALLBACK = 5,
+              ST_SCAL = BATCH_STAGES;
+
+hipError_t launch_sort_stage(const Knobs& kn, uint32_t n, const mv::BvGroups& G, bool agg, void* bscratch,
+                             hipStream_t s, const StageMarks& mk) {
+  using namespace mv;
+  const BatchLayout L(n, G.count);
+  char* base = static_cast<char*>(bscratch);
+  const uint4* scal = (const uint4*)(base + L.scal);
+  uint32_t* pcount = (uint32_t*)(base + L.pcount);
+  uint32_t* poff = (uint32_t*)(base + L.poff);
+  uint32_t* ptot = (uint32_t*)(base + L.ptot);
+  uint32_t* pstart = (uint32_t*)(base + L.pstart);
+  void* tmp = base + L.tmp;
+  uint32_t* offs = (uint32_t*)(base + L.offs);
+  uint32_t* ents = (uint32_t*)(base + L.ents);
+  const bool sort_narrow = !kn.sort_wide && n <= BV_NARROW_MAX_N;
+  const uint32_t nchunk = (n + PART_CHUNK - 1) / PART_CHUNK;
+  const uint32_t nparts = G.count * BV_NPG;
+  mk.begin(ST_SORT);
+  hipLaunchKernelGGL(k_part_count, dim3(nchunk), dim3(PART_CHUNK), 0, s, scal, n, agg ? 1u : 0u, pcount);
+  hipLaunchKernelGGL(k_part_scan, dim3(G.count * (BV_NPG / 64)), dim3(64 * SCAN_SUB), 0, s, pcount, nchunk, G, poff,
+                     ptot);
+  hipLaunchKernelGGL(k_part_top, dim3(1), dim3(256), 0, s, ptot, nparts, pstart);
+  if (sort_narrow) {
+    hipLaunchKernelGGL(k_part_scatter_lds<uint32_t>, dim3(nchunk), dim3(PART_CHUNK), 0, s, scal, n, pcount, poff,
+                       pstart, G, agg ? 1u : 0u, n, 0u, (uint32_t*)tmp);
+    hipLaunchKernelGGL(k_fine_sort_lds<uint32_t>, dim3(nparts), dim3(FINE_NT), 0, s, (const uint32_t*)tmp, pstart,
+                       G.count, ents, offs);
+  } else {
+    hipLaunchKernelGGL(k_part_scatter_lds<unsigned long long>, dim3(nchunk), dim3(PART_CHUNK), 0, s, scal, n, pcount,
+                       poff, pstart, G, agg ? 1u : 0u, n, 0u, (unsigned long long*)tmp);
+    hipLaunchKernelGGL(k_fine_sort_lds<unsigned long long>, dim3(nparts), dim3(FINE_NT), 0, s,
+                       (const unsigned long long*)tmp, pstart, G.count, ents, offs);
+  }
+  mk.end(ST_SORT);
+  return hipGetLastError();
+}
+
 struct PrepStage {
   mv::CommitteeA ca;
   bool agg;
@@ -1090,7 +1117,7 @@
                              const uint32_t* key_idx, uint32_t n, const mv::BvGroups& G, const uint32_t key[10],
                              uint4* pts, uint4* scal, unsigned long long* bsum, uint8_t* status, hipStream_t s,
                              const void* comb_a, const uint8_t* key_ok, uint32_t n_keys, const ChunkGate* gate,
-                             const hipEvent_t* chain, PrepStage* out) {
+                             const hipEvent_t* chain, void* sort_scratch, const StageMarks& mk, PrepStage* out) {
   using namespace mv;
   hipError_t e;
   BvKey k;
@@ -1107,20 +1134,33 @@
   if (gate && gate->n) {
     const uint32_t* end = gate->end;
     if (end[gate->n - 1] != n) return hipErrorInvalidValue;
+    mk.begin(ST_SCAL);
+    mk.end(ST_SCAL);
+    mk.begin(ST_PREP);
     for (uint32_t c = 0, lo = 0; c < gate->n; lo = end[c++]) {
       const uint32_t hi = end[c];
       if (hi <= lo || lo % 256 || (hi % 256 && hi != n)) return hipErrorInvalidValue;
       if ((e = hipStreamWaitEvent(s, gate->ready[c], 0)) != hipSuccess) return e;
-      hipLaunchKernelGGL(k_bv_prep, dim3((hi - lo + 255) / 256), dim3(256), 0, s, msg, sig, pk, key_idx, n, k, ca,
-                         pts, scal, bsum, status, lo / 256, group_sigs);
-    }
+      hipLaunchKernelGGL(k_bv_scal, dim3((hi - lo + 255) / 256), dim3(256), 0, s, msg, sig, pk, key_idx, n, k, scal,
+                         lo / 256);
+      hipLaunchKernelGGL(k_bv_prep, dim3((hi - lo + 255) / 256), dim3(256), 0, s, sig, pk, key_idx, n, ca, pts, scal,
+                         bsum, status, lo / 256, group_sigs);
+    }
+    mk.end(ST_PREP);
+    if (sort_scratch && (e = launch_sort_stage(kn, n, G, agg, sort_scratch, s, mk)) != hipSuccess) return e;
   } else {
+    mk.begin(ST_SCAL);
+    hipLaunchKernelGGL(k_bv_scal, dim3((n + 255) / 256), dim3(256), 0, s, msg, sig, pk, key_idx, n, k, scal, 0u);
+    mk.end(ST_SCAL);
+    if (sort_scratch && (e = launch_sort_stage(kn, n, G, agg, sort_scratch, s, mk)) != hipSuccess) return e;
     if (chain && chain[0] && (e = hipStreamWaitEvent(s, chain[0], 0)) != hipSuccess) return e;
-    hipLaunchKernelGGL(k_bv_prep, dim3((n + 255) / 256), dim3(256), 0, s, msg, sig, pk, key_idx, n, k, ca, pts, scal,
-                       bsum, status, 0u, group_sigs);
+    mk.begin(ST_PREP);
+    hipLaunchKernelGGL(k_bv_prep, dim3((n + 255) / 256), dim3(256), 0, s, sig, pk, key_idx, n, ca, pts, scal, bsum,
+                       status, 0u, group_sigs);
+    mk.end(ST_PREP);
     if (chain && (e = hipEventRecord(chain[1], s)) != hipSuccess) return e;
   }
-  return hipSuccess;
+  return hipGetLastError();
 }
 }
 
@@ -1133,7 +1173,7 @@
   PrepStage ps;
   hipError_t e = launch_prep_stage(kn, msg, sig, pk, key_idx, n, G, key, static_cast<uint4*>(pts),
                                    static_cast<uint4*>(scal), static_cast<unsigned long long*>(bsum), status, s, comb_a,
-                                   key_ok, n_keys, gate, nullptr, &ps);
+                                   key_ok, n_keys, gate, nullptr, nullptr, StageMarks{nullptr, s}, &ps);
   if (e != hipSuccess) return e;
   if (info) *info = BatchPrepInfo{G.count, G.cpg * mv::PART_CHUNK, ps.ca.tab && ps.ca.aggregate ? 0u : 1u};
   return hipGetLastError();
@@ -1147,19 +1187,14 @@
 };
 hipError_t launch_msm_stage(const Knobs& kn, const uint32_t* key_idx, uint32_t n, const mv::BvGroups& G, bool agg,
                             uint32_t n_keys, const void* comb_a, const void* comb_b, void* bscratch, hipStream_t s,
-                            hipEvent_t* ev, MsmStage* out) {
+                            bool sorted, const StageMarks& mk, MsmStage* out) {
   using namespace mv;
-  auto mark = [&](int i) { if (ev) (void)hipEventRecord(ev[i], s); };
+  hipError_t e;
+  if (!sorted && (e = launch_sort_stage(kn, n, G, agg, bscratch, s, mk)) != hipSuccess) return e;
   const BatchLayout L(n, G.count);
   char* base = static_cast<char*>(bscratch);
   const uint4* pts = (const uint4*)(base + L.pts);
   const uint4* scal = (const uint4*)(base + L.scal);
-  uint32_t* pcount = (uint32_t*)(base + L.pcount);
-  uint32_t* poff = (uint32_t*)(base + L.poff);
-  uint32_t* ptot = (uint32_t*)(base + L.ptot);
-  uint32_t* pstart = (uint32_t*)(base + L.pstart);
-  void* tmp = base + L.tmp;
-  const bool sort_narrow = !kn.sort_wide && n <= BV_NARROW_MAX_N;
   uint32_t* offs = (uint32_t*)(base + L.offs);
   uint32_t* ents = (uint32_t*)(base + L.ents);
   uint4* carry = (uint4*)(base + L.carry);
@@ -1172,27 +1207,10 @@
   uint4* asum = (uint4*)(base + L.asum);
   uint32_t* flag = (uint32_t*)(base + L.flag);
   const uint32_t nchunk = (n + PART_CHUNK - 1) / PART_CHUNK;
-  const uint32_t nparts = G.count * BV_NPG;
   const uint32_t nw = agg ? BV_NWR : BV_NW;
   const uint32_t nk = G.count * BV_NKG;
+  mk.begin(ST_BUCKET);
   {
-    mark(1);
-    hipLaunchKernelGGL(k_part_count, dim3(nchunk), dim3(PART_CHUNK), 0, s, scal, n, agg ? 1u : 0u, pcount);
-    hipLaunchKernelGGL(k_part_scan, dim3(G.count * (BV_NPG / 64)), dim3(64 * SCAN_SUB), 0, s, pcount, nchunk, G, poff,
-                       ptot);
-    hipLaunchKernelGGL(k_part_top, dim3(1), dim3(256), 0, s, ptot, nparts, pstart);
-    if (sort_narrow) {
-      hipLaunchKernelGGL(k_part_scatter_lds<uint32_t>, dim3(nchunk), dim3(PART_CHUNK), 0, s, scal, n, pcount, poff,
-                         pstart, G, agg ? 1u : 0u, n, 0u, (uint32_t*)tmp);
-      hipLaunchKernelGGL(k_fine_sort_lds<uint32_t>, dim3(nparts), dim3(FINE_NT), 0, s, (const uint32_t*)tmp, pstart,
-                         G.count, ents, offs);
-    } else {
-      hipLaunchKernelGGL(k_part_scatter_lds<unsigned long long>, dim3(nchunk), dim3(PART_CHUNK), 0, s, scal, n, pcount,
-                         poff, pstart, G, agg ? 1u : 0u, n, 0u, (unsigned long long*)tmp);
-      hipLaunchKernelGGL(k_fine_sort_lds<unsigned long long>, dim3(nparts), dim3(FINE_NT), 0, s,
-                         (const unsigned long long*)tmp, pstart, G.count, ents, offs);
-    }
-    mark(2);
     const uint64_t est = (uint64_t)n * (nw + BV_NWR);
     const uint64_t want = kn.bucket_bal > 1 ? est / (uint64_t)kn.bucket_bal
                                             : std::max<uint64_t>(est / 64, std::min<uint64_t>(est / 8, 196608));
@@ -1208,7 +1226,8 @@
                        static_cast<const uint4*>(comb_a), keyp);
     hipLaunchKernelGGL(k_bv_keysum, dim3(G.count), dim3(256), 0, s, keyp, n_keys, asum);
   }
-  mark(3);
+  mk.end(ST_BUCKET);
+  mk.begin(ST_REDUCE);
   const uint4* inV = nullptr;
   const uint4* inT = bktT;
   const uint32_t rows = G.count * nw;
@@ -1234,10 +1253,11 @@
     shift += fan == 8 ? 3 : (fan == 4 ? 2 : 1);
     cnt = out;
   }
-  mark(4);
+  mk.end(ST_REDUCE);
+  mk.begin(ST_FINAL);
   hipLaunchKernelGGL(k_bv_final, dim3(1), dim3(128), 0, s, inV, nw, agg ? (const uint4*)asum : nullptr, bsum,
                      G.count, static_cast<const uint4*>(comb_b), flag, kn.final_rows ? 1u : 0u);
-  mark(5);
+  mk.end(ST_FINAL);
   *out = MsmStage{inV, agg ? (const uint4*)asum : nullptr, nw};
   return hipGetLastError();
 }
@@ -1249,7 +1269,7 @@
                                uint32_t** flag_out, hipEvent_t* ev, const void* comb_a, const uint8_t* key_ok,
                                uint32_t n_keys, const void* comb_b, const ChunkGate* gate, const hipEvent_t* chain) {
   using namespace mv;
-  auto mark = [&](int i) { if (ev) (void)hipEventRecord(ev[i], s); };
+  const StageMarks mk{ev, s};
   if (n == 0) return hipSuccess;
   const BvGroups G = batch_groups(n, groups);
   const BatchLayout L(n, G.count);
@@ -1260,18 +1280,18 @@
   uint32_t* flag = (uint32_t*)(base + L.flag);
   if (flag_out) *flag_out = flag;
   hipError_t e;
-  mark(0);
   PrepStage ps;
   e = launch_prep_stage(kn, msg, sig, pk, key_idx, n, G, key, pts, scal, bsum, status, s, comb_a, key_ok, n_keys, gate,
-                        chain, &ps);
+                        chain, bscratch, mk, &ps);
   if (e != hipSuccess) return e;
   const CommitteeA& ca = ps.ca;
   MsmStage ms;
-  e = launch_msm_stage(kn, key_idx, n, G, ps.agg, n_keys, comb_a, comb_b, bscratch, s, ev, &ms);
+  e = launch_msm_stage(kn, key_idx, n, G, ps.agg, n_keys, comb_a, comb_b, bscratch, s, true, mk, &ms);
   if (e != hipSuccess) return e;
+  mk.begin(ST_FALLBACK);
   e = launch_verify(msg, sig, pk, key_idx, n, btab, vscratch, status, s, flag + 1, G.cpg * PART_CHUNK, pts,
                     ca.tab && ca.aggregate ? comb_a : nullptr);
-  mark(6);
+  mk.end(ST_FALLBACK);
   return e;
 }
 
@@ -1297,7 +1317,8 @@
       hipSuccess)
     return e;
   MsmStage ms;
-  e = launch_msm_stage(kn, key_idx, n, G, agg, n_keys, comb_a, comb_b, bscratch, s, nullptr, &ms);
+  e = launch_msm_stage(kn, key_idx, n, G, agg, n_keys, comb_a, comb_b, bscratch, s, false,
+                       StageMarks{nullptr, s}, &ms);
   if (e != hipSuccess) return e;
   *info = BatchMsmInfo{G.count, G.cpg * PART_CHUNK, ms.nw, ms.winV, ms.asum, (const uint32_t*)(base + L.flag)};
   return hipSuccess;
diff --git a/mysticeti_amd/csrc/engine.cpp b/mysticeti_amd/csrc/engine.cpp
--- a/mysticeti_amd/csrc/engine.cpp
+++ b/mysticeti_amd/csrc/engine.cpp
@@ -178,7 +178,7 @@
   key[9] = (uint32_t)(call >> 32);
   uint32_t* flag = nullptr;
   mvr::EventSet evs;
-  mv_status st = make_events(ctx, mvk::BATCH_STAGES, evs);
+  mv_status st = make_events(ctx, mvk::BATCH_EVENTS - 1, evs);
   if (st != MV_OK) return st;
   hipEvent_t chain[2] = {};
   const bool chained = ctx->kn.prep_chain && !(gate && gate->n) && (!caller_stream || ctx->kn.prep_chain >= 2);
@@ -193,7 +193,12 @@
                                        com_a ? (uint32_t)ctx->committee.size() : 0u, dev.tab.combB.p, gate,
                                        chained ? chain : nullptr));
   if (chained) dev.batch.prep_chained = true;
-  keep_events(ctx, dev.id, 0, evs);
+  {
+    std::vector<int> stages(mvk::BATCH_STAGES + 1);
+    for (int k = 0; k < mvk::BATCH_STAGES; k++) stages[k] = k;
+    stages[mvk::BATCH_STAGES] = kScalStage;
+    keep_event_pairs(ctx, dev.id, std::move(stages), evs);
+  }
   if (flag_dst) HIPCHK(ctx, hipMemcpyAsync(flag_dst, flag, 4, hipMemcpyDeviceToDevice, s));
   const uint32_t ng = (n + mvk::batch_group_size(n, groups) - 1) / mvk::batch_group_size(n, groups);
   HIPCHK(ctx, hipMemcpyAsync(dev.batch.flags(fe), flag, sizeof(uint32_t) * (1 + ng), hipMemcpyDeviceToHost, s));
@@ -1016,6 +1021,17 @@
   for (auto& pe : ctx->pending) {
     HIPCHK(ctx, hipSetDevice(pe.device));
     mvr::EventSet& ev = pe.events;
+    if (!pe.pair_stage.empty()) {
+      for (size_t k = 0; k < pe.pair_stage.size(); k++) {
+        float t = 0;
+        HIPCHK(ctx, hipEventSynchronize(ev[2 * k + 1]));
+        HIPCHK(ctx, hipEventElapsedTime(&t, ev[2 * k], ev[2 * k + 1]));
+        ctx->stage_ms[pe.pair_stage[k]] += t;
+        ctx->stage_calls[pe.pair_stage[k]]++;
+      }
+      ev.release();
+      continue;
+    }
     HIPCHK(ctx, hipEventSynchronize(ev.back()));
     for (size_t i = 0; i + 1 < ev.size(); i++) {
       float t = 0;
diff --git a/mysticeti_amd/csrc/engine_internal.h b/mysticeti_amd/csrc/engine_internal.h
--- a/mysticeti_amd/csrc/engine_internal.h
+++ b/mysticeti_amd/csrc/engine_internal.h
@@ -22,7 +22,8 @@
 
 constexpr int kBlockStages = 4;
 constexpr int kWalStage0 = kBlockStage0 + kBlockStages;
-static_assert(kWalStage0 + 2 == MV_NSTAGES, "stage count");
+constexpr int kScalStage = kWalStage0 + 2;
+static_assert(kScalStage + 1 == MV_NSTAGES, "stage count");
 
 using mvr::DevBuf;
 using mvr::HostBuf;
@@ -163,6 +164,7 @@
   int device;
   int first_stage;
   mvr::EventSet events;
+  std::vector<int> pair_stage;
 };
 
 }
@@ -294,7 +296,12 @@
 inline void keep_events(mv_ctx* ctx, int device, int first_stage, mvr::EventSet& evs) {
   if (evs.empty()) return;
   std::lock_guard<std::mutex> lk(ctx->tmu);
-  ctx->pending.push_back(PendingEvents{device, first_stage, std::move(evs)});
+  ctx->pending.push_back(PendingEvents{device, first_stage, std::move(evs), {}});
+}
+inline void keep_event_pairs(mv_ctx* ctx, int device, std::vector<int> stages, mvr::EventSet& evs) {
+  if (evs.empty()) return;
+  std::lock_guard<std::mutex> lk(ctx->tmu);
+  ctx->pending.push_back(PendingEvents{device, 0, std::move(evs), std::move(stages)});
 }
 
 constexpr uint32_t kOnSlots = mvk::ONLINE_SLOTS, kOnMax = mvk::ONLINE_MAX_BLOCKS;
diff --git a/mysticeti_amd/csrc/fe25519.h b/mysticeti_amd/csrc/fe25519.h
--- a/mysticeti_amd/csrc/fe25519.h
+++ b/mysticeti_amd/csrc/fe25519.h
@@ -315,31 +315,4 @@
   fe_mul2(ra, ta, xa, rb, tb, xb);
 }
 
-MV_DEV void fe_pow_p58_x2_nox(fe& ra, fe& rb, const fe& xa, const fe& xb) {
-  fe a0, b0, a2, b2, a3, b3, a5, b5, a7, b7, a13, b13, a15, b15, ta, tb;
-  fe_sq2(a0, xa, b0, xb);
-  ta = a0; tb = b0; fe_sq2n(ta, tb, 2);
-  fe_mul2(a2, xa, ta, b2, xb, tb);
-  fe_mul2(a3, a0, a2, b3, b0, b2);
-  fe_sq2(ta, a3, tb, b3);
-  fe_mul2(a5, a2, ta, b5, b2, tb);
-  ta = a5; tb = b5; fe_sq2n(ta, tb, 5);
-  fe_mul2(a7, ta, a5, b7, tb, b5);
-  ta = a7; tb = b7; fe_sq2n(ta, tb, 10);
-  fe_mul2(a2, ta, a7, b2, tb, b7);
-  ta = a2; tb = b2; fe_sq2n(ta, tb, 20);
-  fe_mul2(ta, ta, a2, tb, tb, b2);
-  fe_sq2n(ta, tb, 10);
-  fe_mul2(a13, ta, a7, b13, tb, b7);
-  ta = a13; tb = b13; fe_sq2n(ta, tb, 50);
-  fe_mul2(a15, ta, a13, b15, tb, b13);
-  ta = a15; tb = b15; fe_sq2n(ta, tb, 100);
-  fe_mul2(ta, ta, a15, tb, tb, b15);
-  fe_sq2n(ta, tb, 50);
-  fe_mul2(ta, ta, a13, tb, tb, b13);
-  fe_sq2n(ta, tb, 2);
-  ra = ta;
-  rb = tb;
-}
-
-}
+}
diff --git a/mysticeti_amd/csrc/ge25519.h b/mysticeti_amd/csrc/ge25519.h
--- a/mysticeti_amd/csrc/ge25519.h
+++ b/mysticeti_amd/csrc/ge25519.h
@@ -236,58 +236,4 @@
   A.X = xa; A.Y = ya; fe_set(A.Z, 1); fe_mul(A.T, xa, ya);
 }
 
-template <class Get>
-MV_DEV void decompress2_lean(p3& A, bool& okA, p3& R, bool& okR, Get get) {
-  fe pa, pr;
-  {
-    fe xa, xr;
-    {
-      fe d, one, y, u, v, t;
-      uint32_t ea[8], er[8];
-      get(0, ea);
-      get(1, er);
-      fe_const(d, K_D);
-      fe_set(one, 1);
-      fe_from_words(y, ea);
-      fe_sq(t, y);
-      fe_sub(u, t, one);
-      fe_mul(v, t, d);
-      fe_add(v, v, one);
-      fe_sq(t, v); fe_mul(xa, t, v);
-      fe_sq(t, xa); fe_mul(xa, t, v); fe_mul(xa, xa, u);
-      fe_from_words(y, er);
-      fe_sq(t, y);
-      fe_sub(u, t, one);
-      fe_mul(v, t, d);
-      fe_add(v, v, one);
-      fe_sq(t, v); fe_mul(xr, t, v);
-      fe_sq(t, xr); fe_mul(xr, t, v); fe_mul(xr, xr, u);
-    }
-    fe_pow_p58_x2_nox(pa, pr, xa, xr);
-  }
-  auto finish = [](p3& P, bool& ok, const uint32_t e[8], fe& p) {
-    fe d, one, y, u, v, t, v3, x, n;
-    fe_const(d, K_D);
-    fe_set(one, 1);
-    fe_from_words(y, e);
-    fe_sq(t, y);
-    fe_sub(u, t, one);
-    fe_mul(v, t, d);
-    fe_add(v, v, one);
-    fe_sq(t, v); fe_mul(v3, t, v);
-    fe_sq(t, v3); fe_mul(t, t, v); fe_mul(t, t, u);
-    fe_mul(p, p, t);
-    fe_mul(p, p, v3); fe_mul(p, p, u);
-    ok = sqrt_ratio_finish(x, u, v, p);
-    fe_neg(n, x);
-    fe_cmov(x, n, (e[7] >> 31) != 0);
-    P.X = x; P.Y = y; fe_set(P.Z, 1); fe_mul(P.T, x, y);
-  };
-  uint32_t e[8];
-  get(0, e);
-  finish(A, okA, e, pa);
-  get(1, e);
-  finish(R, okR, e, pr);
-}
-
-}
+}
diff --git a/mysticeti_amd/csrc/kernels.h b/mysticeti_amd/csrc/kernels.h
--- a/mysticeti_amd/csrc/kernels.h
+++ b/mysticeti_amd/csrc/kernels.h
@@ -76,6 +76,7 @@
   const uint32_t* end;
 };
 constexpr int BATCH_STAGES = 6;
+constexpr int BATCH_EVENTS = 2 * (BATCH_STAGES + 1);
 constexpr int BATCH_MAX_GROUPS = 16;
 size_t batch_scratch_bytes(uint32_t n, uint32_t groups);
 uint32_t batch_group_size(uint32_t n, uint32_t groups);
diff --git a/rust/mysti-verify-sys/src/lib.rs b/rust/mysti-verify-sys/src/lib.rs
--- a/rust/mysti-verify-sys/src/lib.rs
+++ b/rust/mysti-verify-sys/src/lib.rs
@@ -91,7 +91,7 @@
 pub const MV_FLAG_HOST_PARSE: u32 = 4;
 pub const MV_FLAG_NO_ONLINE: u32 = 8;
 pub const MV_BATCH_MIN: u32 = 4096;
-pub const MV_NSTAGES: usize = 12;
+pub const MV_NSTAGES: usize = 13;
 
 extern "C" {
     pub fn mv_create(cfg: *const mv_config, out: *mut *mut mv_ctx) -> i32;
```

Result: no change. 350.7 million (median of 6 runs) (+0.8%).
